# sc15i2gp/daily-ray-trace

Hardware: NVIDIA B200
Metric: camera_paths_per_sec (higher is better)
Workload: dtype f32

## Files before the change

### daily-ray-trace_b200/csrc/drt_capi.cu

```cuda
#include <cuda_runtime.h>
#include <math.h>
#include <stdarg.h>
#include <stdio.h>
#include <stdlib.h>
#include <string.h>
#include <vector>
#include "drt_context.cuh"

static thread_local char g_err[512];

int drt_fail(int code, const char *fmt, ...)
{
    va_list ap;
    va_start(ap, fmt);
    vsnprintf(g_err, sizeof(g_err), fmt, ap);
    va_end(ap);
    return code;
}

extern "C" const char *drt_cuda_last_error(void) { return g_err; }

extern "C" int drt_cuda_device_count(void)
{
    int n = 0;
// ... 170 lines not shown
    if(nmirror + ncond + ndiel == mm->num_lobes && (nmirror != 0) + (ncond != 0) + (ndiel != 0) == 1)
    {
        if(basis_out) *basis_out = nmirror ? 0 : ndiel ? 1 : 2;
        return (nmirror || (base_n && own_n)) ? DRT_CLASS_SPECULAR : DRT_CLASS_GENERAL;
    }
    return DRT_CLASS_GENERAL;
}

static int scene_kernel_mode(const drt_scene *scene)
{
    int nlights = 0;
    for(int i = 0; i < scene->num_surfaces; i += 1) nlights += scene->materials[scene->surfaces[i].material].is_emissive ? 1 : 0;
    bool all_fast = nlights == 1 && !scene->materials[scene->escape_material].is_emissive, classed = all_fast;
    for(int i = 0; i < scene->num_surfaces; i += 1)
    {
        const int m = scene->surfaces[i].material;
        if(scene->materials[m].is_black_body || scene->surfaces[i].type == DRT_GEO_POINT || scene->surfaces[i].type == DRT_GEO_NONE) continue;
        const int cls = classify_material(scene, m, nullptr, nullptr, nullptr);
        if(cls != DRT_CLASS_PLASTIC) all_fast = false;
        if(cls == DRT_CLASS_GENERAL) classed = false;
    }
    if(getenv("DRT_NO_CLASSED")) classed = all_fast;
    return all_fast ? 1 : classed ? 2 : 0;
}

template <typename R>
static void fill_geom(GeomT<R> *g, const drt_scene *s, const drt_camera *c);

extern "C" int drt_cuda_plan_scene(const drt_scene *scene, const drt_camera *camera, int32_t *kernel_mode_out, int32_t *material_class, float *specular_constants)
{
    if(!scene || !camera || !kernel_mode_out) return fail(DRT_CUDA_E_ARG, "NULL argument");
    int rc = drt_cuda_validate_scene(scene);
    if(rc != DRT_CUDA_OK) return rc;
    *kernel_mode_out = scene_kernel_mode(scene);
    if(material_class || specular_constants)
    {
        GeomT<float> *g = new GeomT<float>();
        fill_geom(g, scene, camera);
        for(int m = 0; m < scene->num_materials; m += 1)
        {
            if(material_class) material_class[m] = g->mclass[m];
            if(specular_constants) memcpy(specular_constants + (size_t)m * 6, g->spec_c[m], 6 * sizeof(float));
        }
        delete g;
    }
    return DRT_CUDA_OK;
}

template <typename R>
static void fill_geom(GeomT<R> *g, const drt_scene *s, const drt_camera *c)
{
    memset(g, 0, sizeof(*g));
    g->nsurf = s->num_surfaces; g->nmat = s->num_materials; g->n = s->num_wavelengths;
    g->base_mat = s->base_material; g->escape_mat = s->escape_material;
    uint32_t i0 = (uint32_t)((DRT_TRANS_WL - s->min_wl) / s->wl_interval);
    double w0 = s->min_wl + i0 * s->wl_interval, w1 = s->min_wl + (i0 + 1) * s->wl_interval;
    g->trans_num = (R)(DRT_TRANS_WL - w0);
    g->trans_den = (R)(w1 - w0);
    int nl = 0;
    for(int i = 0; i < s->num_surfaces; i += 1)
    {
        const drt_surface *f = &s->surfaces[i];
        g->type[i] = f->type; g->mat[i] = f->material;
        g->px[i] = (R)f->position[0]; g->py[i] = (R)f->position[1]; g->pz[i] = (R)f->position[2];
        g->rad[i] = (R)f->radius;
        g->nx[i] = (R)f->normal[0]; g->ny[i] = (R)f->normal[1]; g->nz[i] = (R)f->normal[2];
        g->ux[i] = (R)f->u[0]; g->uy[i] = (R)f->u[1]; g->uz[i] = (R)f->u[2];
        g->vx[i] = (R)f->v[0]; g->vy[i] = (R)f->v[1]; g->vz[i] = (R)f->v[2];
        double pdf = 1.0;
        if(f->type == DRT_GEO_PLANE)
        {
            double ul = sqrt(f->u[0] * f->u[0] + f->u[1] * f->u[1] + f->u[2] * f->u[2]);
            double vl = sqrt(f->v[0] * f->v[0] + f->v[1] * f->v[1] + f->v[2] * f->v[2]);
            g->ulen[i] = (R)ul; g->vlen[i] = (R)vl;
            g->unx[i] = (R)(f->u[0] / ul); g->uny[i] = (R)(f->u[1] / ul); g->unz[i] = (R)(f->u[2] / ul);
            g->vnx[i] = (R)(f->v[0] / vl); g->vny[i] = (R)(f->v[1] / vl); g->vnz[i] = (R)(f->v[2] / vl);
            double cx = f->u[1] * f->v[2] - f->u[2] * f->v[1], cy = f->u[2] * f->v[0] - f->u[0] * f->v[2], cz = f->u[0] * f->v[1] - f->u[1] * f->v[0];
            pdf = sqrt(cx * cx + cy * cy + cz * cz);
        }
        else if(f->type == DRT_GEO_SPHERE) pdf = (double)(4.0 * 3.1415926535897932385L * f->radius * f->radius);
        g->light_pdf[i] = (R)pdf;
        if(s->materials[f->material].is_emissive) g->light_surf[nl++] = i;
    }
    g->nlights = nl;
    auto plane_axis = [&](const drt_surface *f) -> int {
        auto single = [](const double *v) -> int {
            int axis = -1;
            for(int k = 0; k < 3; k += 1) if(v[k] != 0.0) { if(axis >= 0) return -1; axis = k; }
            return axis;
        };
        int a = single(f->normal), b = single(f->u), c = single(f->v);
        if(a < 0 || b < 0 || c < 0 || a == b || a == c || b == c) return -1;
        if(f->normal[a] != 1.0 && f->normal[a] != -1.0) return -1;
        return a;
    };
    int slot = 0;
    for(int pass = 0; pass < 9; pass += 1)
        for(int i = 0; i < s->num_surfaces; i += 1)
        {
            const drt_surface *f = &s->surfaces[i];
            const int group = pass / 2;
            if(pass < 8)
            {
                if(f->type != DRT_GEO_PLANE || plane_axis(f) != (group < 3 ? group : -1)) continue;
                if(surface_is_boundary(s, i) != ((pass & 1) == 0)) continue;
                if((pass & 1) == 0) g->nax_b[group] += 1;
            }
            else if(f->type != DRT_GEO_SPHERE) continue;
            g->sid[slot] = i;
            g->N4[slot] = R4<R>{ g->nx[i], g->ny[i], g->nz[i], (R)0 };
            g->P4[slot] = R4<R>{ g->px[i], g->py[i], g->pz[i], g->rad[i] };
            g->U4[slot] = R4<R>{ g->unx[i], g->uny[i], g->unz[i], g->ulen[i] };
            g->V4[slot] = R4<R>{ g->vnx[i], g->vny[i], g->vnz[i], g->vlen[i] };
            if(group < 3)
            {
                const int a = group, b = (a == 0) ? 1 : 0, c = (a == 2) ? 1 : 2;
                double lo[2], hi[2];
                const int bc[2] = { b, c };
                for(int k = 0; k < 2; k += 1)
                {
                    double p0 = f->position[bc[k]], p1 = p0 + f->u[bc[k]] + f->v[bc[k]];
                    lo[k] = p0 < p1 ? p0 : p1; hi[k] = p0 < p1 ? p1 : p0;
                }
                g->AX4[slot] = R4<R>{ (R)f->position[a], (R)(0.5 * (lo[0] + hi[0])), (R)(0.5 * (hi[0] - lo[0])), (R)(0.5 * (lo[1] + hi[1])) };
                g->AXH[slot] = R2<R>{ (R)(0.5 * (hi[1] - lo[1])), (R)i };
                g->nax[a] += 1;
            }
            slot += 1;
            if(pass < 8) g->nplanes += 1; else g->nspheres += 1;
        }
    for(int m = 0; m < s->num_materials; m += 1)
    {
        const drt_material *mm = &s->materials[m];
        g->mflags[m] = (mm->is_black_body ? 1 : 0) | (mm->is_emissive ? 2 : 0);
        g->nlobes[m] = mm->num_lobes; g->dirf[m] = mm->dir_func;
        for(int k = 0; k < mm->num_lobes && k < DRT_MAX_LOBES; k += 1) g->lobes[m][k] = (unsigned char)mm->lobes[k];
        g->shin[m] = (R)mm->shininess; g->rough[m] = (R)mm->roughness;
        int mask = 0;
        for(int k = 0; k < mm->num_lobes && k < DRT_MAX_LOBES; k += 1)
            switch(mm->lobes[k])
            {
                case DRT_LOBE_BP_DIFFUSE: mask |= 1 << BK_DIFFUSE; break;
                case DRT_LOBE_BP_GLOSSY: mask |= 1 << BK_GLOSSY; break;
                case DRT_LOBE_MIRROR: mask |= 1 << BK_MIRROR; break;
                case DRT_LOBE_FS_CONDUCTOR: mask |= 1 << BK_COND_ON; break;
                case DRT_LOBE_FS_DIELECTRIC_REFLECTANCE: mask |= 1 << BK_DIEL_R; break;
                case DRT_LOBE_FS_DIELECTRIC_TRANSMITTANCE: mask |= (1 << BK_DIEL_R) | (1 << BK_CONST); break;
                case DRT_LOBE_CT_CONDUCTOR: mask |= 1 << BK_COND_MN; break;
                default: break;
            }
        g->bmask[m] = mask;
        g->mclass[m] = classify_material(s, m, nullptr, nullptr, nullptr);
        if(g->mclass[m] == DRT_CLASS_SPECULAR)
            for(int match = 0; match < 3; match += 1)
            {
                const bool refl = match == 1, trans = match == 2;
                double cur_c = 0.0, cur_x = 0.0, acc_c = 0.0, acc_x = 0.0;
                for(int k = 0; k < mm->num_lobes; k += 1)
                {
                    bool wrote = false; double val = 0.0, val_c = 0.0;
                    switch(mm->lobes[k])
                    {
                        case DRT_LOBE_MIRROR: wrote = true; val = refl ? 1.0 : 0.0; break;
                        case DRT_LOBE_FS_CONDUCTOR: case DRT_LOBE_FS_DIELECTRIC_REFLECTANCE: wrote = refl; val = 1.0; break;
                        case DRT_LOBE_FS_DIELECTRIC_TRANSMITTANCE: wrote = trans; val = -1.0; val_c = 1.0; break;
                        default: break;
                    }
                    if(wrote) { cur_x = val; cur_c = val_c; }
                    acc_c += cur_c; acc_x += cur_x;
                }
                g->spec_c[m][match][0] = (float)acc_c; g->spec_c[m][match][1] = (float)acc_x;
            }
        int nct = 0;
        for(int k = 0; k < mm->num_lobes && k < DRT_MAX_LOBES; k += 1) nct += mm->lobes[k] == DRT_LOBE_CT_CONDUCTOR;
        g->ct_mult[m] = (float)nct;
        int words = __builtin_popcount((unsigned)mask) + ((mask >> BK_COND_MN) & 1);
        if(!mm->is_black_body && words > g->eval_words) g->eval_words = words;
        if(mm->spd_mask & (1 << DRT_SPD_REFRACT))
        {
            g->n630[m] = (R)value_at_wl(s, mm->spd[DRT_SPD_REFRACT], DRT_TRANS_WL);
            g->refr_a[m] = (R)mm->spd[DRT_SPD_REFRACT][i0];
            g->refr_b[m] = (R)mm->spd[DRT_SPD_REFRACT][i0 + 1];
        }
    }
    for(int k = 0; k < 3; k += 1)
    {
        g->fwd[k] = (R)c->forward[k]; g->right[k] = (R)c->right[k]; g->up[k] = (R)c->up[k];
        g->ap_pos[k] = (R)c->aperture_position[k]; g->film_bl[k] = (R)c->film_bottom_left[k];
    }
    g->ap_radius = (R)c->aperture_radius; g->focal_depth = (R)c->focal_depth;
    g->pixel_w = (R)c->pixel_width; g->pixel_h = (R)c->pixel_height;
    for(int k = 0; k < 9; k += 1) g->lens_rot[k] = (R)c->lens_rotation[k];
}

extern "C" int drt_cuda_validate_scene(const drt_scene *scene)
{
    if(!scene) return fail(DRT_CUDA_E_ARG, "NULL argument");
    int n = scene->num_wavelengths;
    if(n < 2 || n > DRT_MAX_WAVELENGTHS) return fail(DRT_CUDA_E_ARG, "%d wavelengths (need 2..%d)", n, DRT_MAX_WAVELENGTHS);
    if(scene->num_surfaces < 0 || scene->num_surfaces > DRT_MAX_SURFACES || scene->num_materials < 1 || scene->num_materials > DRT_MAX_MATERIALS)
        return fail(DRT_CUDA_E_ARG, "%d surfaces / %d materials out of range", scene->num_surfaces, scene->num_materials);
    if(scene->base_material < 0 || scene->escape_material < 0) return fail(DRT_CUDA_E_UNSUPPORTED, "scene needs a base_material and an escape_material");
    if(scene->base_material >= scene->num_materials || scene->escape_material >= scene->num_materials)
        return fail(DRT_CUDA_E_ARG, "base_material %d / escape_material %d out of range (%d materials)", scene->base_material, scene->escape_material, scene->num_materials);
    if(!(scene->wl_interval > 0.0)) return fail(DRT_CUDA_E_ARG, "wl_interval must be positive");
    uint32_t i0 = (uint32_t)((DRT_TRANS_WL - scene->min_wl) / scene->wl_interval);
    if(DRT_TRANS_WL < scene->min_wl || (int)i0 + 1 >= n) return fail(DRT_CUDA_E_UNSUPPORTED, "630 nm (trans_wl, daily_ray_trace.c:381) lies outside the wavelength grid");
    for(int i = 0; i < scene->num_surfaces; i += 1)
    {
        if(scene->surfaces[i].material < 0 || scene->surfaces[i].material >= scene->num_materials) return fail(DRT_CUDA_E_ARG, "surface %d: bad material index", i);
        if(scene->surfaces[i].type < DRT_GEO_NONE || scene->surfaces[i].type > DRT_GEO_PLANE) return fail(DRT_CUDA_E_ARG, "surface %d: bad type %d", i, scene->surfaces[i].type);
    }
    for(int m = 0; m < scene->num_materials; m += 1)
    {
        const drt_material *mm = &scene->materials[m];
        if(mm->num_lobes < 0 || mm->num_lobes > DRT_MAX_LOBES) return fail(DRT_CUDA_E_ARG, "material %d: %d lobes (0..%d)", m, mm->num_lobes, DRT_MAX_LOBES);
        if(mm->dir_func < DRT_DIR_NONE || mm->dir_func >= DRT_DIR_COUNT) return fail(DRT_CUDA_E_ARG, "material %d: bad dir_func %d", m, mm->dir_func);
        for(int k = 0; k < mm->num_lobes; k += 1)
            if(mm->lobes[k] < -1 || mm->lobes[k] >= DRT_LOBE_COUNT) return fail(DRT_CUDA_E_ARG, "material %d: bad lobe id %d", m, mm->lobes[k]);
    }
    for(int i = 0; i < scene->num_surfaces; i += 1)
    {
        const drt_material *mm = &scene->materials[scene->surfaces[i].material];
        if(scene->surfaces[i].type != DRT_GEO_POINT && scene->surfaces[i].type != DRT_GEO_NONE && !mm->is_black_body && mm->dir_func == DRT_DIR_NONE)
            return fail(DRT_CUDA_E_ARG, "surface %d: its material has no dir_func", i);
    }
    return DRT_CUDA_OK;
}

extern "C" int drt_cuda_upload_scene(drt_cuda_context *ctx, const drt_scene *scene, const drt_camera *camera, const drt_tables *tables)
{
    if(!ctx || !scene || !camera || !tables) return fail(DRT_CUDA_E_ARG, "NULL argument");
    int vrc = drt_cuda_validate_scene(scene);
    if(vrc != DRT_CUDA_OK) return vrc;
    CU(cudaSetDevice(ctx->device));
    const int n = scene->num_wavelengths;
    const uint32_t i0 = (uint32_t)((DRT_TRANS_WL - scene->min_wl) / scene->wl_interval);
    (void)i0;

    GeomT<float> *g32 = new GeomT<float>();
    GeomT<double> *g64 = new GeomT<double>();
    fill_geom(g32, scene, camera);
    fill_geom(g64, scene, camera);

    ctx->hit_bound = scene_hit_bound(scene, camera, &ctx->hit_u0, &ctx->hit_u1, &ctx->hit_v0, &ctx->hit_v1);

    SpdIndex index;
    memset(&index, 0, sizeof(index));
    int half_slots = (n + 15) / 16;
    half_slots = half_slots <= 2 ? 2 : half_slots <= 3 ? 3 : half_slots <= 5 ? 5 : 8;
    index.n = n; index.nslots = half_slots; index.npad = ((n + 31) / 32) * 32;
    if(index.npad < half_slots * 16) index.npad = half_slots * 16;
    std::vector<float> pool((size_t)index.npad, 0.f);
    int rows = 1;
    for(int m = 0; m < scene->num_materials; m += 1)
        for(int k = 0; k < DRT_SPD_COUNT; k += 1)
        {
            if(!(scene->materials[m].spd_mask & (1 << k))) continue;
            index.row[m][k] = (rows++) * index.npad;
            size_t at = pool.size();
            pool.resize(at + (size_t)index.npad, 0.f);
            for(int i = 0; i < n; i += 1) pool[at + (size_t)i] = (float)scene->materials[m].spd[k][i];
        }
    index.nrows = rows;
    if(g32->nlights == 1)
    {
        const double *emission = scene->materials[scene->surfaces[g32->light_surf[0]].material].spd[DRT_SPD_EMISSION];
        const bool have_e = (scene->materials[scene->surfaces[g32->light_surf[0]].material].spd_mask & (1 << DRT_SPD_EMISSION)) != 0;
        for(int m = 0; m < scene->num_materials; m += 1)
        {
            const drt_material *mm = &scene->materials[m];
            if(mm->is_black_body || mm->num_lobes != 2 || g32->bmask[m] != ((1 << BK_DIFFUSE) | (1 << BK_GLOSSY))) continue;
            size_t at = (pool.size() + 3) & ~(size_t)3;
            pool.resize(at + (size_t)half_slots * 64, 0.f);
            index.plastic[m] = (int)at;
            auto val = [&](int k, int slot, int lane) -> float {
                int wl = lane + slot * 16;
                return (wl < n && (mm->spd_mask & (1 << k))) ? (float)mm->spd[k][wl] : 0.f;
            };
            auto emi = [&](int slot, int lane) -> float {
                int wl = lane + slot * 16;
                return (wl < n && have_e) ? (float)emission[wl] : 0.f;
            };
            const int np = half_slots / 2;
            for(int lane = 0; lane < 16; lane += 1)
            {
                for(int pr = 0; pr < np; pr += 1)
                    for(int j = 0; j < 2; j += 1)
                    {
                        int slot = 2 * pr + j;
                        float d = val(DRT_SPD_DIFFUSE, slot, lane), gl = val(DRT_SPD_GLOSSY, slot, lane), e = emi(slot, lane);
                        float *c0 = &pool[at + ((size_t)(2 * pr) * 16 + lane) * 4], *c1 = &pool[at + ((size_t)(2 * pr + 1) * 16 + lane) * 4];
                        c0[j] = d; c0[2 + j] = gl; c1[j] = d * e; c1[2 + j] = gl * e;
                    }
                if(half_slots & 1)
                {
                    int slot = half_slots - 1;
                    float d = val(DRT_SPD_DIFFUSE, slot, lane), gl = val(DRT_SPD_GLOSSY, slot, lane), e = emi(slot, lane);
                    float *c = &pool[at + ((size_t)(half_slots - 1) * 16 + lane) * 4];
                    c[0] = d; c[1] = gl; c[2] = d * e; c[3] = gl * e;
                }
            }
        }
        for(int m = 0; m < scene->num_materials; m += 1)
        {
            const drt_material *mm = &scene->materials[m];
            int nd = 0, ng = 0;
            if(mm->is_black_body || classify_material(scene, m, &nd, &ng, nullptr) != DRT_CLASS_PLASTIC) continue;
            auto val = [&](int k, int mult, int slot, int lane) -> float {
                int wl = lane + slot * 16;
                return (wl < n && (mm->spd_mask & (1 << k))) ? (float)((double)mult * mm->spd[k][wl]) : 0.f;
            };
            const int nchunks = (half_slots + 1) / 2;
            size_t at2 = (pool.size() + 3) & ~(size_t)3;
            pool.resize(at2 + (size_t)nchunks * 64, 0.f);
            index.plastic2[m] = (int)at2;
            for(int lane = 0; lane < 16; lane += 1)
                for(int ch = 0; ch < nchunks; ch += 1)
                {
                    float *c = &pool[at2 + ((size_t)ch * 16 + lane) * 4];
                    if(2 * ch + 1 < half_slots)
                    {
                        c[0] = val(DRT_SPD_DIFFUSE, nd, 2 * ch, lane); c[1] = val(DRT_SPD_DIFFUSE, nd, 2 * ch + 1, lane);
                        c[2] = val(DRT_SPD_GLOSSY, ng, 2 * ch, lane);  c[3] = val(DRT_SPD_GLOSSY, ng, 2 * ch + 1, lane);
                    }
                    else { c[0] = val(DRT_SPD_DIFFUSE, nd, 2 * ch, lane); c[1] = val(DRT_SPD_GLOSSY, ng, 2 * ch, lane); }
                }
        }
        const int nchunks = (half_slots + 1) / 2;
        size_t ate = (pool.size() + 3) & ~(size_t)3;
        pool.resize(ate + (size_t)nchunks * 32, 0.f);
        index.light_pairs = (int)ate;
        for(int lane = 0; lane < 16; lane += 1)
            for(int ch = 0; ch < nchunks; ch += 1)
            {
                float *c = &pool[ate + ((size_t)ch * 16 + lane) * 2];
                int w0 = lane + (2 * ch) * 16, w1 = lane + (2 * ch + 1) * 16;
                c[0] = (w0 < n && have_e) ? (float)emission[w0] : 0.f;
                c[1] = (2 * ch + 1 < half_slots && w1 < n && have_e) ? (float)emission[w1] : 0.f;
            }
    }

    if(scene->materials[scene->base_material].spd_mask & (1 << DRT_SPD_REFRACT))
    {
        const drt_material *bm = &scene->materials[scene->base_material];
        const bool base_k = (bm->spd_mask & (1 << DRT_SPD_EXTINCT)) != 0;
        for(int m = 0; m < scene->num_materials; m += 1)
        {
            const drt_material *mm = &scene->materials[m];
            if(m == scene->base_material || mm->is_black_body || !(mm->spd_mask & (1 << DRT_SPD_REFRACT))) continue;
            const bool own_k = (mm->spd_mask & (1 << DRT_SPD_EXTINCT)) != 0;
            for(int side = 0; side < 2; side += 1)
                for(int k = 0; k < 3; k += 1)
                {
                    size_t at = pool.size();
                    pool.resize(at + (size_t)index.npad, 0.f);
                    index.fres[m][side][k] = (int)at;
                    for(int i = 0; i < n; i += 1)
                    {
                        const double ir = side ? mm->spd[DRT_SPD_REFRACT][i] : bm->spd[DRT_SPD_REFRACT][i];
                        const double tr = side ? bm->spd[DRT_SPD_REFRACT][i] : mm->spd[DRT_SPD_REFRACT][i];
                        const double te = side ? (base_k ? bm->spd[DRT_SPD_EXTINCT][i] : 0.0) : (own_k ? mm->spd[DRT_SPD_EXTINCT][i] : 0.0);
                        const double eta = tr / ir, kap = te / ir;
                        pool[at + (size_t)i] = (float)(k == 0 ? ir / tr : k == 1 ? eta * eta - kap * kap : 4.0 * eta * eta * kap * kap);
                    }
                }
        }
    }

    std::vector<unsigned char> rgbt(drt_rgb_tables_bytes());
    drt_fill_rgb_tables(rgbt.data(), tables);

    ctx->have_scene = false;
    cudaError_t e = cudaSuccess;
    if(e == cudaSuccess && !ctx->d_geom32) e = cudaMalloc(&ctx->d_geom32, sizeof(GeomT<float>));
    if(e == cudaSuccess && !ctx->d_geom64) e = cudaMalloc(&ctx->d_geom64, sizeof(GeomT<double>));
    if(e == cudaSuccess && !ctx->d_index) e = cudaMalloc(&ctx->d_index, sizeof(SpdIndex));
    if(e == cudaSuccess && !ctx->d_rgb_tables) e = cudaMalloc(&ctx->d_rgb_tables, rgbt.size());
    if(e == cudaSuccess && ctx->pool_capacity < pool.size() * 4)
    {
        cudaFree(ctx->d_pool); ctx->d_pool = nullptr; ctx->pool_capacity = 0;
        e = cudaMalloc(&ctx->d_pool, pool.size() * 4);
        if(e == cudaSuccess) ctx->pool_capacity = pool.size() * 4;
    }
    if(e == cudaSuccess) e = cudaMemcpy(ctx->d_geom32, g32, sizeof(GeomT<float>), cudaMemcpyHostToDevice);
    if(e == cudaSuccess) e = cudaMemcpy(ctx->d_geom64, g64, sizeof(GeomT<double>), cudaMemcpyHostToDevice);
    if(e == cudaSuccess) e = cudaMemcpy(ctx->d_index, &index, sizeof(index), cudaMemcpyHostToDevice);
    if(e == cudaSuccess) e = cudaMemcpy(ctx->d_pool, pool.data(), pool.size() * 4, cudaMemcpyHostToDevice);
    if(e == cudaSuccess) e = cudaMemcpy(ctx->d_rgb_tables, rgbt.data(), rgbt.size(), cudaMemcpyHostToDevice);
    int nlights = g32->nlights;
    int mode = scene_kernel_mode(scene);
    bool all_fast = mode == 1, classed = mode != 0;
    if(pool.size() > 65535) all_fast = classed = false;
    int eval_words = g32->eval_words > 0 ? g32->eval_words : 1;
    delete g32; delete g64;
    if(e != cudaSuccess) return fail(DRT_CUDA_E_CUDA, "scene upload: %s", cudaGetErrorString(e));
    ctx->n = n; ctx->nslots = index.nslots; ctx->nlights = nlights; ctx->eval_words = eval_words; ctx->all_fast = all_fast; ctx->classed = classed && !all_fast; ctx->pool_words = (uint32_t)pool.size();
    ctx->upload_bytes = sizeof(GeomT<float>) + sizeof(GeomT<double>) + sizeof(SpdIndex) + pool.size() * 4 + rgbt.size();
    ctx->have_scene = true;
    return DRT_CUDA_OK;
}

extern "C" int drt_cuda_scene_upload_bytes(const drt_cuda_context *ctx, size_t *bytes)
{
    if(!ctx || !bytes) return fail(DRT_CUDA_E_ARG, "NULL argument");
    *bytes = ctx->upload_bytes;
    return DRT_CUDA_OK;
}

extern "C" int drt_cuda_set_geometry_precision(drt_cuda_context *ctx, int precision)
{
    if(!ctx || (precision != DRT_GEOMETRY_F32 && precision != DRT_GEOMETRY_F64)) return fail(DRT_CUDA_E_ARG, "bad precision");
    ctx->f64_geometry = precision == DRT_GEOMETRY_F64;
    return DRT_CUDA_OK;
}

extern "C" int drt_cuda_film_sizes(const drt_cuda_context *ctx, uint32_t width, uint32_t height, size_t *spectral, size_t *filter)
{
    if(!ctx || !ctx->have_scene) return fail(DRT_CUDA_E_STATE, "upload a scene first");
    if(spectral) *spectral = (size_t)width * height * (size_t)ctx->n * 4;
    if(filter) *filter = (size_t)width * height * 4;
    return DRT_CUDA_OK;
}

static int kernel_mode(const drt_cuda_context *ctx) { return ctx->f64_geometry ? 0 : ctx->all_fast ? 1 : ctx->classed ? 2 : 0; }

static void record_layout(const drt_cuda_context *ctx, uint32_t max_depth, uint32_t smem_depth, RenderLaunch &L)
{
    L.eval_words = (uint32_t)ctx->eval_words;
    const bool compact = kernel_mode(ctx) != 0;
    L.bounce_words = (2 + (uint32_t)ctx->nlights * (L.eval_words + 1) + L.eval_words + 3u) & ~3u;
    if(L.bounce_words < 8) L.bounce_words = 8;
    L.head_words = 4;
    if(smem_depth > max_depth) smem_depth = max_depth;
    if(compact) { L.bounce_words = 4; L.head_words = (2 + (smem_depth + 1) / 2 + 3u) & ~3u; }
    L.smem_depth = smem_depth;
    L.path_words = L.head_words + smem_depth * L.bounce_words;
    L.path_stride = ((L.path_words / 4) & 1u) ? L.path_words : L.path_words + 4;
    const uint32_t over = max_depth - smem_depth;
    L.deep_hdr_off = over * L.bounce_words;
    L.deep_stride = over ? ((L.deep_hdr_off + (compact ? (over + 1) / 2 : 0u) + 4u + 3u) & ~3u) : 0u;
}

static bool launch_shape(const drt_cuda_context *ctx, uint32_t max_depth, bool whole, RenderLaunch &L, int *warps_out, int *ctas_out, size_t *smem_out)
{
    const int mode = kernel_mode(ctx);
    const int full_warps = drt_render_cta_warps(ctx->f64_geometry, mode), want_ctas = drt_render_min_ctas(ctx->f64_geometry, mode);
    auto bytes = [&](uint32_t depth, int warps) { record_layout(ctx, max_depth, depth, L); return drt_render_smem_bytes(L, ctx->f64_geometry, warps, ctx->nslots); };
    int warps = full_warps;
    uint32_t depth = max_depth;
    const size_t per_cta = (size_t)(227 * 1024) / (size_t)want_ctas - 1024;
    if(!whole && max_depth > 1 && bytes(max_depth, warps) > per_cta)
    {
        uint32_t lo = 1, hi = max_depth;
        while(lo < hi) { uint32_t mid = (lo + hi + 1) / 2; if(bytes(mid, warps) <= per_cta) lo = mid; else hi = mid - 1; }
        depth = lo;
    }
    size_t smem = bytes(depth, warps);
    while(smem > ctx->smem_optin && warps > 1) { warps /= 2; smem = bytes(depth, warps); }
    *warps_out = warps; *smem_out = smem;
    if(smem > ctx->smem_optin) return false;
    int ctas_per_sm = (int)((size_t)(227 * 1024) / (smem + 1024));
    int by_threads = (want_ctas * full_warps) / warps;
    if(ctas_per_sm > by_threads) ctas_per_sm = by_threads;
    if(ctas_per_sm < 1) ctas_per_sm = 1;
    *ctas_out = ctas_per_sm;
    return true;
}

extern "C" int drt_cuda_render_kernel_info(drt_cuda_context *ctx, const drt_render_params *params, char *name, size_t name_len, int *warps_per_cta, int *ctas_per_sm)
{
    if(!ctx || !params || params->sample_end <= params->sample_begin) return fail(DRT_CUDA_E_ARG, "bad argument");
    const uint32_t max_depth = params->max_depth;
    if(!ctx->have_scene) return fail(DRT_CUDA_E_STATE, "upload a scene first");
    RenderLaunch L;
    memset(&L, 0, sizeof(L));
    L.pool_words = ctx->pool_words;
    int warps = 0, ctas = 0;
    size_t smem = 0;
    if(!launch_shape(ctx, max_depth, false, L, &warps, &ctas, &smem)) return fail(DRT_CUDA_E_UNSUPPORTED, "one bounce record of this scene does not fit in shared memory");
    if(name && name_len)
        snprintf(name, name_len, "drt::render_kernel<%s,%d,%d,%s,%s>", ctx->f64_geometry ? "double" : "float", ctx->nslots,
                 kernel_mode(ctx), (params->sample_end - params->sample_begin >= 32) ? "true" : "false", L.deep_stride ? "true" : "false");
    if(warps_per_cta) *warps_per_cta = warps;
    if(ctas_per_sm) *ctas_per_sm = ctas;
    return DRT_CUDA_OK;
}

static int launch(drt_cuda_context *ctx, const drt_render_params *p, uint32_t x0, uint32_t y0, uint32_t x1, uint32_t y1,
                  FilmPtrs film, float *dump, int accumulate, cudaStream_t stream, float *record_dump = nullptr, uint32_t *path_words_out = nullptr,
                  const drt_film *scatter = nullptr, int scatter_count = 0, int scatter_rank = 0, uint64_t scatter_slice = 0, bool keep_stats = false,
                  uint64_t band_begin = 0, uint64_t band_end = 0, const drt_adaptive *adaptive = nullptr)
{
    if(!ctx->have_scene) return fail(DRT_CUDA_E_STATE, "upload a scene first");
    if(p->width == 0 || p->height == 0 || x1 > p->width || y1 > p->height || x0 >= x1 || y0 >= y1) return fail(DRT_CUDA_E_ARG, "bad image rectangle");
    if(p->sample_end < p->sample_begin) return fail(DRT_CUDA_E_ARG, "bad sample range [%u,%u)", p->sample_begin, p->sample_end);
    CU(cudaSetDevice(ctx->device));
    if(p->sample_end == p->sample_begin)
    {
        if(path_words_out) *path_words_out = 0;
        if(!keep_stats)
        {
            ctx->d_stats = ctx->d_stats_ring + (ctx->stats_calls++ % DRT_RING);
            CU(cudaMemsetAsync(ctx->d_stats, 0, sizeof(DeviceStats), stream));
        }
        ctx->last_launches = 0;
        if(film.sum && !accumulate && scatter_count == 0)
        {
            const size_t n = (size_t)ctx->n, w = p->width;
            if(x0 != 0 || x1 != p->width) return fail(DRT_CUDA_E_ARG, "empty sample range on a partial-width rectangle");
            const size_t at = (size_t)y0 * w, cnt = (size_t)(y1 - y0) * w;
            CU(cudaMemsetAsync(film.sum + at * n, 0, cnt * n * 4, stream)); CU(cudaMemsetAsync(film.mean + at * n, 0, cnt * n * 4, stream));
            CU(cudaMemsetAsync(film.m2 + at * n, 0, cnt * n * 4, stream));  CU(cudaMemsetAsync(film.filter + at, 0, cnt * 4, stream));
        }
        return DRT_CUDA_OK;
    }
    RenderLaunch L;
    memset(&L, 0, sizeof(L));
    L.geom = ctx->f64_geometry ? ctx->d_geom64 : ctx->d_geom32;
    L.spd_index = ctx->d_index; L.pool = ctx->d_pool; L.pool_words = ctx->pool_words;
    L.film = film; L.path_dump = dump; L.record_dump = record_dump;
    L.width = p->width; L.height = p->height; L.x0 = x0; L.y0 = y0; L.x1 = x1; L.y1 = y1;
    L.sample_begin = p->sample_begin; L.sample_end = p->sample_end; L.max_depth = p->max_depth;
    L.pixel_scheme = p->pixel_scheme; L.seed = p->seed; L.accumulate = accumulate; L.nlights = ctx->nlights;
    uint32_t spp = p->sample_end - p->sample_begin;
    L.pixels_per_task = spp >= 32 ? 1 : 32 / spp;
    for(int i = 0; i < scatter_count; i += 1) L.scatter[i] = FilmPtrs{ scatter[i].sum, scatter[i].filter, scatter[i].mean, scatter[i].m2 };
    L.scatter_count = (uint32_t)scatter_count; L.scatter_rank = (uint32_t)scatter_rank; L.scatter_slice = (uint32_t)scatter_slice;
    uint32_t rect[4];
    hit_rect(ctx->hit_bound && p->max_depth > 0, ctx->hit_u0, ctx->hit_u1, ctx->hit_v0, ctx->hit_v1, p->width, p->height, rect);
    L.hit_x0 = rect[0]; L.hit_y0 = rect[1]; L.hit_x1 = rect[2]; L.hit_y1 = rect[3];
    if(adaptive)
    {
        L.adaptive = 1; L.rel_error = adaptive->rel_error; L.min_samples = adaptive->min_samples;
        L.luminance_w = reinterpret_cast<const float *>(static_cast<const unsigned char *>(ctx->d_rgb_tables) + drt_rgb_tables_yw_offset());
    }
    const bool whole = record_dump != nullptr || (path_words_out != nullptr && !dump && !film.sum);
    int warps, ctas_per_sm;
    size_t smem;
    if(!launch_shape(ctx, p->max_depth, whole, L, &warps, &ctas_per_sm, &smem))
        return fail(DRT_CUDA_E_UNSUPPORTED, "%s: max_cast_depth %u with %d lights needs %zu bytes of shared memory per warp (limit %zu)",
                    whole ? "record dump" : "render", p->max_depth, ctx->nlights, smem, ctx->smem_optin);
    if(path_words_out) { *path_words_out = L.path_words; if(!record_dump && !dump && !film.sum) return DRT_CUDA_OK; }
    uint64_t npix = (uint64_t)(x1 - x0) * (y1 - y0);
    const bool band = band_end > band_begin;
    if(band)
    {
        if(L.pixels_per_task != 1 || scatter_count < 1 || band_end > scatter_slice || x0 != 0 || y0 != 0 || x1 != p->width || y1 != p->height)
            return fail(DRT_CUDA_E_ARG, "a band needs a scattered whole-frame render with at least 32 samples per pixel");
        L.band_chunk = (uint32_t)(band_end - band_begin); L.band_period = (uint32_t)scatter_slice; L.band_base = (uint32_t)band_begin;
    }
    uint64_t ntasks = band ? (uint64_t)L.band_chunk * scatter_count : (npix + L.pixels_per_task - 1) / L.pixels_per_task;
    if(scatter_count > 1)
        L.task_rotate = band ? (uint32_t)(((uint64_t)scatter_rank * L.band_chunk) % ntasks)
                             : (uint32_t)((((uint64_t)scatter_rank * scatter_slice) / L.pixels_per_task) % ntasks);
    uint64_t grid = (uint64_t)ctx->num_sms * ctas_per_sm;
    uint64_t need = (ntasks + warps - 1) / warps;
    if(grid > need) grid = need;
    if(L.deep_stride)
    {
        const size_t need_bytes = (size_t)grid * (size_t)warps * DRT_WARP * L.deep_stride * 4;
        int rc = drt_ensure_buffer(&ctx->d_deep, &ctx->deep_bytes, need_bytes);
        if(rc != DRT_CUDA_OK) return rc;
        L.deep = ctx->d_deep;
    }
    if(!keep_stats)
    {
        ctx->d_stats = ctx->d_stats_ring + (ctx->stats_calls++ % DRT_RING);
        CU(cudaMemsetAsync(ctx->d_stats, 0, sizeof(DeviceStats), stream));
    }
    L.stats = ctx->d_stats;
    L.task_counter = ctx->d_counter_ring + (ctx->counter_launches++ % DRT_RING);
    CU(cudaMemsetAsync(L.task_counter, 0, sizeof(unsigned int), stream));
    cudaError_t e = drt_launch_render(L, ctx->f64_geometry, kernel_mode(ctx), ctx->nslots, (int)grid, warps, smem, stream);
    if(e != cudaSuccess) return fail(DRT_CUDA_E_CUDA, "render kernel launch: %s", cudaGetErrorString(e));
    ctx->launches += 1;
    ctx->last_launches = 1;
    return DRT_CUDA_OK;
}

extern "C" int drt_cuda_render_device(drt_cuda_context *ctx, const drt_render_params *params, const drt_film *film, int accumulate, void *stream)
{
    if(!ctx || !params || !film || !film->sum || !film->filter || !film->mean || !film->m2) return fail(DRT_CUDA_E_ARG, "NULL argument");
    FilmPtrs f = { film->sum, film->filter, film->mean, film->m2 };
    return launch(ctx, params, 0, 0, params->width, params->height, f, nullptr, accumulate, (cudaStream_t)stream);
}

extern "C" int drt_cuda_render_device_scatter(drt_cuda_context *ctx, const drt_render_params *params, const drt_film *staging, int count, int rank,
                                              uint64_t slice_pixels, void *stream)
{
    if(!ctx || !params || !staging || count < 1 || count > DRT_MAX_PEERS || rank < 0 || rank >= count) return fail(DRT_CUDA_E_ARG, "bad argument (1..%d staging films)", DRT_MAX_PEERS);
    uint64_t npix = (uint64_t)params->width * params->height;
    if(slice_pixels == 0 || slice_pixels * (uint64_t)count < npix || slice_pixels > 0xffffffffull) return fail(DRT_CUDA_E_ARG, "slices of %llu pixels do not cover the image", (unsigned long long)slice_pixels);
    for(int i = 0; i < count; i += 1)
        if(!staging[i].sum || !staging[i].filter || !staging[i].mean || !staging[i].m2) return fail(DRT_CUDA_E_ARG, "NULL staging film %d", i);
    FilmPtrs f = { staging[0].sum, staging[0].filter, staging[0].mean, staging[0].m2 };
    return launch(ctx, params, 0, 0, params->width, params->height, f, nullptr, 0, (cudaStream_t)stream, nullptr, nullptr, staging, count, rank, slice_pixels);
}

extern "C" int drt_cuda_render_device_scatter_band(drt_cuda_context *ctx, const drt_render_params *params, const drt_film *staging, int count, int rank,
                                                   uint64_t slice_pixels, uint64_t band_begin, uint64_t band_end, int keep_stats, void *stream)
{
    if(!ctx || !params || !staging || count < 1 || count > DRT_MAX_PEERS || rank < 0 || rank >= count) return fail(DRT_CUDA_E_ARG, "bad argument (1..%d staging films)", DRT_MAX_PEERS);
    uint64_t npix = (uint64_t)params->width * params->height;
    if(slice_pixels == 0 || slice_pixels * (uint64_t)count < npix || slice_pixels > 0xffffffffull) return fail(DRT_CUDA_E_ARG, "slices of %llu pixels do not cover the image", (unsigned long long)slice_pixels);
    if(band_begin >= band_end || band_end > slice_pixels) return fail(DRT_CUDA_E_ARG, "bad band [%llu, %llu) of a slice of %llu pixels", (unsigned long long)band_begin, (unsigned long long)band_end, (unsigned long long)slice_pixels);
    for(int i = 0; i < count; i += 1)
        if(!staging[i].sum || !staging[i].filter || !staging[i].mean || !staging[i].m2) return fail(DRT_CUDA_E_ARG, "NULL staging film %d", i);
    FilmPtrs f = { staging[0].sum, staging[0].filter, staging[0].mean, staging[0].m2 };
    return launch(ctx, params, 0, 0, params->width, params->height, f, nullptr, 0, (cudaStream_t)stream, nullptr, nullptr, staging, count, rank, slice_pixels,
                  keep_stats != 0, band_begin, band_end);
}

int drt_ensure_buffer(float **buf, size_t *have, size_t need)
{
    if(*have >= need) return DRT_CUDA_OK;
    cudaFree(*buf); *buf = nullptr; *have = 0;
    CU(cudaMalloc(buf, need));
    *have = need;
    return DRT_CUDA_OK;
}

static int adaptive_args(const drt_cuda_context *ctx, const drt_render_params *p, const drt_adaptive *a)
{
    if(!ctx->have_scene) return fail(DRT_CUDA_E_STATE, "upload a scene first");
    if(p->sample_end < p->sample_begin) return fail(DRT_CUDA_E_ARG, "bad sample range [%u,%u)", p->sample_begin, p->sample_end);
    const uint32_t range = p->sample_end - p->sample_begin;
    if(!(a->rel_error > 0.f) || !isfinite(a->rel_error))
        return fail(DRT_CUDA_E_ARG, "adaptive sampling: rel_error must be a finite number > 0 (got %g)", (double)a->rel_error);
    if(a->min_samples < 32u || a->min_samples > range)
        return fail(DRT_CUDA_E_ARG, "adaptive sampling: min_samples must lie in [32, %u], the call's sample range [%u,%u) (got %u); "
                    "a pixel is checked after each batch of 32 samples, so the range needs at least 32", range, p->sample_begin, p->sample_end, a->min_samples);
    if(ctx->f64_geometry)
        return fail(DRT_CUDA_E_UNSUPPORTED, "adaptive sampling runs with f32 geometry only: f64 geometry is the branch-flip diagnostic and has no adaptive kernel");
    return DRT_CUDA_OK;
}

extern "C" int drt_cuda_render_device_adaptive(drt_cuda_context *ctx, const drt_render_params *params, const drt_adaptive *adaptive,
                                               const drt_film *film, int accumulate, void *stream)
{
    if(!ctx || !params || !adaptive || !film || !film->sum || !film->filter || !film->mean || !film->m2) return fail(DRT_CUDA_E_ARG, "NULL argument");
    int rc = adaptive_args(ctx, params, adaptive);
    if(rc != DRT_CUDA_OK) return rc;
    FilmPtrs f = { film->sum, film->filter, film->mean, film->m2 };
    return launch(ctx, params, 0, 0, params->width, params->height, f, nullptr, accumulate, (cudaStream_t)stream, nullptr, nullptr, nullptr, 0, 0, 0, false, 0, 0, adaptive);
}

static int render_host(drt_cuda_context *ctx, const drt_render_params *params, const drt_adaptive *adaptive, const drt_film *out)
{
    if(!ctx || !params || !out || !out->sum || !out->filter || !out->mean || !out->m2) return fail(DRT_CUDA_E_ARG, "NULL argument");
    if(!ctx->have_scene) return fail(DRT_CUDA_E_STATE, "upload a scene first");
    CU(cudaSetDevice(ctx->device));
    size_t npix = (size_t)params->width * params->height, plane = npix * (size_t)ctx->n * 4, fplane = npix * 4;
    int rc = drt_ensure_buffer(&ctx->d_film, &ctx->film_bytes, 3 * plane + fplane);
    if(rc != DRT_CUDA_OK) return rc;
    float *base = ctx->d_film;
    FilmPtrs f = { base, base + 3 * (plane / 4), base + plane / 4, base + 2 * (plane / 4) };
    const uint64_t paths = (uint64_t)npix * (params->sample_end - params->sample_begin);
    static const int cut[] = { 0, 4, 8, 12, 14, 15, 16 };
    int bands = (paths >= (1ull << 26) && params->height >= 64) ? 6 : 1;
    if(bands > 1 && !ctx->band_render)
    {
        CU(cudaStreamCreateWithFlags(&ctx->band_render, cudaStreamNonBlocking));
        CU(cudaStreamCreateWithFlags(&ctx->band_copy, cudaStreamNonBlocking));
        for(int i = 0; i < 16; i += 1) CU(cudaEventCreateWithFlags(&ctx->band_done[i], cudaEventDisableTiming));
    }
    cudaStream_t sr = bands > 1 ? ctx->band_render : 0, sc = bands > 1 ? ctx->band_copy : 0;
    if(bands > 1) CU(cudaDeviceSynchronize());
    const size_t n = (size_t)ctx->n, w = params->width;
    for(int b = 0; b < bands; b += 1)
    {
        const uint32_t y0 = bands > 1 ? (uint32_t)((uint64_t)params->height * cut[b] / 16) : 0u;
        const uint32_t y1 = bands > 1 ? (uint32_t)((uint64_t)params->height * cut[b + 1] / 16) : params->height;
        rc = launch(ctx, params, 0, y0, params->width, y1, f, nullptr, 0, sr, nullptr, nullptr, nullptr, 0, 0, 0, b > 0, 0, 0, adaptive);
        if(rc != DRT_CUDA_OK) return rc;
        if(bands > 1) { CU(cudaEventRecord(ctx->band_done[b], sr)); CU(cudaStreamWaitEvent(sc, ctx->band_done[b], 0)); }
        const size_t at = (size_t)y0 * w * n, cnt = (size_t)(y1 - y0) * w * n * 4;
        CU(cudaMemcpyAsync(out->sum + at, f.sum + at, cnt, cudaMemcpyDeviceToHost, sc));
        CU(cudaMemcpyAsync(out->mean + at, f.mean + at, cnt, cudaMemcpyDeviceToHost, sc));
        CU(cudaMemcpyAsync(out->m2 + at, f.m2 + at, cnt, cudaMemcpyDeviceToHost, sc));
        CU(cudaMemcpyAsync(out->filter + (size_t)y0 * w, f.filter + (size_t)y0 * w, (size_t)(y1 - y0) * w * 4, cudaMemcpyDeviceToHost, sc));
    }
    ctx->last_launches = (uint64_t)bands;
    if(bands > 1) { CU(cudaStreamSynchronize(sr)); CU(cudaStreamSynchronize(sc)); }
    CU(cudaStreamSynchronize(0));
    return DRT_CUDA_OK;
}

extern "C" int drt_cuda_render_host(drt_cuda_context *ctx, const drt_render_params *params, const drt_film *out)
{
    return render_host(ctx, params, nullptr, out);
}

extern "C" int drt_cuda_render_host_adaptive(drt_cuda_context *ctx, const drt_render_params *params, const drt_adaptive *adaptive, const drt_film *out)
{
    if(!ctx || !params || !adaptive) return fail(DRT_CUDA_E_ARG, "NULL argument");
    int rc = adaptive_args(ctx, params, adaptive);
    if(rc != DRT_CUDA_OK) return rc;
    return render_host(ctx, params, adaptive, out);
}

extern "C" int drt_cuda_get_stats(drt_cuda_context *ctx, drt_cuda_stats *out)
{
    if(!ctx || !out) return fail(DRT_CUDA_E_ARG, "NULL argument");
    CU(cudaSetDevice(ctx->device));
    CU(cudaDeviceSynchronize());
    DeviceStats s;
    CU(cudaMemcpy(&s, ctx->d_stats, sizeof(s), cudaMemcpyDeviceToHost));
    memset(out, 0, sizeof(*out));
    out->paths = s.paths; out->closest_rays = s.closest_rays; out->shadow_rays = s.shadow_rays;
    out->shaded_bounces = s.shaded_bounces; out->rng_draws = s.rng_draws;
    for(int i = 0; i < 8; i += 1) out->terminated_at_depth[i] = s.terminated_at_depth[i];
    out->reached_depth_cap = s.reached_depth_cap;
    out->kernel_launches = ctx->last_launches;
    return DRT_CUDA_OK;
}

#ifdef DRT_PHASE_CLOCKS
extern "C" int drt_cuda_phase_clocks(drt_cuda_context *ctx, uint64_t out[4])
{
    if(!ctx || !out) return fail(DRT_CUDA_E_ARG, "NULL argument");
    CU(cudaSetDevice(ctx->device));
    CU(cudaDeviceSynchronize());
    DeviceStats s;
    CU(cudaMemcpy(&s, ctx->d_stats, sizeof(s), cudaMemcpyDeviceToHost));
    for(int i = 0; i < 4; i += 1) out[i] = s.phase_clocks[i];
    return DRT_CUDA_OK;
}
#endif

extern "C" int drt_cuda_sample_paths(drt_cuda_context *ctx, const drt_render_params *params,
                                     uint32_t x0, uint32_t y0, uint32_t x1, uint32_t y1, float *out_host)
{
    if(!ctx || !params || !out_host) return fail(DRT_CUDA_E_ARG, "NULL argument");
    if(!ctx->have_scene) return fail(DRT_CUDA_E_STATE, "upload a scene first");
    if(x1 <= x0 || y1 <= y0 || params->sample_end <= params->sample_begin) return fail(DRT_CUDA_E_ARG, "empty rectangle or sample range");
    CU(cudaSetDevice(ctx->device));
    size_t bytes = (size_t)(x1 - x0) * (y1 - y0) * (params->sample_end - params->sample_begin) * (size_t)ctx->n * 4;
    int rc = drt_ensure_buffer(&ctx->d_dump, &ctx->dump_bytes, bytes);
    if(rc != DRT_CUDA_OK) return rc;
    FilmPtrs none = { nullptr, nullptr, nullptr, nullptr };
    rc = launch(ctx, params, x0, y0, x1, y1, none, ctx->d_dump, 0, 0);
    if(rc != DRT_CUDA_OK) return rc;
    CU(cudaMemcpy(out_host, ctx->d_dump, bytes, cudaMemcpyDeviceToHost));
    return DRT_CUDA_OK;
}

extern "C" int drt_cuda_debug_records(drt_cuda_context *ctx, const drt_render_params *params, uint32_t x0, uint32_t y0, uint32_t x1, uint32_t y1,
                                      float *out_host, size_t out_capacity_words, uint32_t *words_per_path)
{
    if(!ctx || !params || !words_per_path) return fail(DRT_CUDA_E_ARG, "NULL argument");
    if(!ctx->have_scene) return fail(DRT_CUDA_E_STATE, "upload a scene first");
    if(x1 <= x0 || y1 <= y0 || params->sample_end <= params->sample_begin) return fail(DRT_CUDA_E_ARG, "empty rectangle or sample range");
    CU(cudaSetDevice(ctx->device));
    FilmPtrs none = { nullptr, nullptr, nullptr, nullptr };
    int rc = launch(ctx, params, x0, y0, x1, y1, none, nullptr, 0, 0, nullptr, words_per_path);
    if(rc != DRT_CUDA_OK || !out_host) return rc;
    size_t words = (size_t)(x1 - x0) * (y1 - y0) * (params->sample_end - params->sample_begin) * (size_t)*words_per_path;
    if(words > out_capacity_words) return fail(DRT_CUDA_E_ARG, "record buffer too small: need %zu words", words);
    rc = drt_ensure_buffer(&ctx->d_dump, &ctx->dump_bytes, words * 4);
    if(rc != DRT_CUDA_OK) return rc;
    rc = launch(ctx, params, x0, y0, x1, y1, none, nullptr, 0, 0, ctx->d_dump, nullptr);
    if(rc != DRT_CUDA_OK) return rc;
    CU(cudaMemcpy(out_host, ctx->d_dump, words * 4, cudaMemcpyDeviceToHost));
    return DRT_CUDA_OK;
}

extern "C" int drt_cuda_film_to_rgb(drt_cuda_context *ctx, const drt_film *film, uint32_t width, uint32_t height, int which,
                                    float *rgb_device, uint32_t *bgra_device, void *stream)
{
    if(!ctx || !film || which < 0 || which > 2) return fail(DRT_CUDA_E_ARG, "bad argument");
    if(!ctx->have_scene) return fail(DRT_CUDA_E_STATE, "upload a scene first");
    CU(cudaSetDevice(ctx->device));
    const float *plane = which == 0 ? film->sum : which == 1 ? film->mean : film->m2;
    const float *filter = which == 0 ? film->filter : nullptr;
    if(!plane || (which == 0 && !filter)) return fail(DRT_CUDA_E_ARG, "film plane is NULL");
    const uint64_t npix64 = (uint64_t)width * height;
    if(npix64 == 0 || npix64 > 0xffffffffull) return fail(DRT_CUDA_E_ARG, "%u x %u pixels out of range", width, height);
    uint32_t npix = (uint32_t)npix64;
    int grid = ctx->num_sms * 8;
    drt_launch_film_to_rgb(ctx->d_rgb_tables, plane, filter, which == 2, npix, rgb_device, bgra_device, grid, (cudaStream_t)stream);
    CU(cudaGetLastError());
    ctx->launches += 1;
    return DRT_CUDA_OK;
}

extern "C" int drt_cuda_film_merge(drt_cuda_context *ctx, const drt_film *dst, const drt_film *src, uint32_t width, uint32_t height, void *stream)
{
    if(!ctx || !dst || !src) return fail(DRT_CUDA_E_ARG, "NULL argument");
    if(!ctx->have_scene) return fail(DRT_CUDA_E_STATE, "upload a scene first");
    CU(cudaSetDevice(ctx->device));
    FilmPtrs d = { dst->sum, dst->filter, dst->mean, dst->m2 }, s = { src->sum, src->filter, src->mean, src->m2 };
    drt_launch_film_merge(d, s, (uint32_t)ctx->n, (size_t)width * height, ctx->num_sms * 8, (cudaStream_t)stream);
    CU(cudaGetLastError());
    ctx->launches += 2;
    return DRT_CUDA_OK;
}

extern "C" int drt_cuda_film_alloc(drt_cuda_context *ctx, uint32_t width, uint32_t height, drt_film *out)
{
    if(!ctx || !out) return fail(DRT_CUDA_E_ARG, "NULL argument");
    if(!ctx->have_scene) return fail(DRT_CUDA_E_STATE, "upload a scene first");
    CU(cudaSetDevice(ctx->device));
    size_t npix = (size_t)width * height, plane = npix * (size_t)ctx->n * 4;
    memset(out, 0, sizeof(*out));
    cudaError_t e = cudaMalloc(&out->sum, plane);
    if(e == cudaSuccess) e = cudaMalloc(&out->mean, plane);
    if(e == cudaSuccess) e = cudaMalloc(&out->m2, plane);
    if(e == cudaSuccess) e = cudaMalloc(&out->filter, npix * 4);
    if(e == cudaSuccess) e = cudaMemset(out->sum, 0, plane);
    if(e == cudaSuccess) e = cudaMemset(out->mean, 0, plane);
    if(e == cudaSuccess) e = cudaMemset(out->m2, 0, plane);
    if(e == cudaSuccess) e = cudaMemset(out->filter, 0, npix * 4);
    if(e != cudaSuccess)
    {
        cudaFree(out->sum); cudaFree(out->mean); cudaFree(out->m2); cudaFree(out->filter);
        memset(out, 0, sizeof(*out));
        return fail(DRT_CUDA_E_CUDA, "film_alloc %ux%u: %s", width, height, cudaGetErrorString(e));
    }
    return DRT_CUDA_OK;
}

extern "C" int drt_cuda_film_free(drt_cuda_context *ctx, drt_film *film)
{
    if(!ctx || !film) return fail(DRT_CUDA_E_ARG, "NULL argument");
    CU(cudaSetDevice(ctx->device));
    cudaFree(film->sum); cudaFree(film->mean); cudaFree(film->m2); cudaFree(film->filter);
    memset(film, 0, sizeof(*film));
    return DRT_CUDA_OK;
}

extern "C" int drt_cuda_film_ipc_export(drt_cuda_context *ctx, const drt_film *film, unsigned char handles[4][64])
{
    if(!ctx || !film || !handles) return fail(DRT_CUDA_E_ARG, "NULL argument");
    CU(cudaSetDevice(ctx->device));
    static_assert(sizeof(cudaIpcMemHandle_t) == 64, "CUDA IPC handle size");
    float *ptrs[4] = { film->sum, film->filter, film->mean, film->m2 };
    for(int i = 0; i < 4; i += 1)
    {
        cudaIpcMemHandle_t h;
        CU(cudaIpcGetMemHandle(&h, ptrs[i]));
        memcpy(handles[i], &h, 64);
    }
    return DRT_CUDA_OK;
}

extern "C" int drt_cuda_film_ipc_open(drt_cuda_context *ctx, const unsigned char handles[4][64], drt_film *out)
{
    if(!ctx || !handles || !out) return fail(DRT_CUDA_E_ARG, "NULL argument");
    CU(cudaSetDevice(ctx->device));
    void *ptrs[4] = { nullptr, nullptr, nullptr, nullptr };
    for(int i = 0; i < 4; i += 1)
    {
        cudaIpcMemHandle_t h;
        memcpy(&h, handles[i], 64);
        CU(cudaIpcOpenMemHandle(&ptrs[i], h, cudaIpcMemLazyEnablePeerAccess));
    }
    out->sum = (float *)ptrs[0]; out->filter = (float *)ptrs[1]; out->mean = (float *)ptrs[2]; out->m2 = (float *)ptrs[3];
    return DRT_CUDA_OK;
}

extern "C" int drt_cuda_film_ipc_close(drt_cuda_context *ctx, drt_film *mapped)
{
    if(!ctx || !mapped) return fail(DRT_CUDA_E_ARG, "NULL argument");
    CU(cudaSetDevice(ctx->device));
    cudaIpcCloseMemHandle(mapped->sum); cudaIpcCloseMemHandle(mapped->filter); cudaIpcCloseMemHandle(mapped->mean); cudaIpcCloseMemHandle(mapped->m2);
    memset(mapped, 0, sizeof(*mapped));
    return DRT_CUDA_OK;
}

extern "C" int drt_cuda_buffer_alloc(drt_cuda_context *ctx, size_t bytes, void **out)
{
    if(!ctx || !out || bytes == 0) return fail(DRT_CUDA_E_ARG, "bad argument");
    CU(cudaSetDevice(ctx->device));
    CU(cudaMalloc(out, bytes));
    CU(cudaMemset(*out, 0, bytes));
    return DRT_CUDA_OK;
// ... 127 lines not shown
```

### daily-ray-trace_b200/csrc/drt_context.cuh

```cuda
#pragma once
#include <cuda_runtime.h>
#include <stdarg.h>
#include <stdint.h>
#include <stdio.h>
#include "drt_cuda.h"
#include "drt_device.cuh"

cudaError_t drt_launch_render(const RenderLaunch &L, bool f64_geometry, int mode, int nslots, int grid, int warps, size_t smem, cudaStream_t stream);
int         drt_render_cta_warps(bool f64_geometry, int mode);
int         drt_render_min_ctas(bool f64_geometry, int mode);
size_t      drt_render_smem_bytes(const RenderLaunch &L, bool f64_geometry, int warps, int nslots);
void        drt_launch_film_to_rgb(const void *tables, const float *plane, const float *filter, int normalise_by_max, uint32_t npix,
                                   float *rgb, uint32_t *bgra, int grid, cudaStream_t stream);
void        drt_launch_film_merge(FilmPtrs dst, FilmPtrs src, uint32_t n, size_t npix, int grid, cudaStream_t stream);
void        drt_launch_fma_peak(int packed, float *out, int iters, int grid, cudaStream_t stream);
void        drt_launch_film_gather_merge(const void *tables, int count, const FilmPtrs *films, FilmPtrs dst, uint32_t pixel_begin, uint32_t pixel_end, uint32_t src_base, uint32_t dst_base,
                                         uint32_t *bgra_sum, uint32_t *bgra_mean, uint32_t *bgra_var, int grid, cudaStream_t stream);
size_t      drt_rgb_tables_bytes(void);
size_t      drt_rgb_tables_yw_offset(void);
void        drt_fill_rgb_tables(void *dst_host, const drt_tables *t);

int drt_fail(int code, const char *fmt, ...);
#define fail drt_fail

#define CU(call) do { cudaError_t e_ = (call); if(e_ != cudaSuccess) return fail(DRT_CUDA_E_CUDA, "%s: %s", #call, cudaGetErrorString(e_)); } while(0)

#define DRT_RING 64

struct drt_cuda_context
{
    int    device = 0;
    int    num_sms = 0;
    size_t smem_optin = 0;
    bool   have_scene = false;
    bool   f64_geometry = false;
    int    n = 0, nslots = 0, nlights = 0, eval_words = 1;
    bool   hit_bound = false;
    double hit_u0 = 0, hit_u1 = 0, hit_v0 = 0, hit_v1 = 0;
    bool   classed = false;
    bool   all_fast = false;
    void  *d_geom32 = nullptr, *d_geom64 = nullptr;
    SpdIndex *d_index = nullptr;
    float *d_pool = nullptr;
    uint32_t pool_words = 0;
    size_t pool_capacity = 0;
    void  *d_rgb_tables = nullptr;
    DeviceStats *d_stats_ring = nullptr;
    unsigned int *d_counter_ring = nullptr;
    uint64_t stats_calls = 0, counter_launches = 0;
    DeviceStats *d_stats = nullptr;
    float *d_film = nullptr; size_t film_bytes = 0;
    float *d_dump = nullptr; size_t dump_bytes = 0;
    float *d_deep = nullptr; size_t deep_bytes = 0;
    float *d_slice = nullptr; size_t slice_bytes = 0;
    uint64_t launches = 0;
    size_t upload_bytes = 0;
    uint64_t last_launches = 0;
    cudaStream_t band_render = nullptr, band_copy = nullptr;
    cudaEvent_t  band_done[16] = {};
    unsigned int *d_wait_timeouts = nullptr;
    struct drt_multi_state *multi = nullptr;
};


void drt_exchange_release(drt_cuda_context *ctx);
int drt_ensure_buffer(float **buf, size_t *have, size_t need);
```

### daily-ray-trace_b200/csrc/drt_device.cuh

```cuda
#pragma once
#include <stdint.h>
#include "drt_scene.h"

#define DRT_WARP 32
#define DRT_MAX_SLOTS 4
#define DRT_HALF 16
#define DRT_MAX_HALF_SLOTS 8
#ifndef DRT_CTA_WARPS
#define DRT_CTA_WARPS 8
#endif
#ifndef DRT_FAST_WARPS
#define DRT_FAST_WARPS 14
#endif
#ifndef DRT_CLASSED_WARPS
#define DRT_CLASSED_WARPS 16
#endif
#ifndef DRT_CLASSED_CTAS
#define DRT_CLASSED_CTAS 2
#endif
#ifndef DRT_GENERAL_CTAS
#define DRT_GENERAL_CTAS 2
#endif
#ifndef DRT_LOCKSTEP
#define DRT_LOCKSTEP 2
#endif
#ifndef DRT_GATE_PATIENCE_CYCLES
#define DRT_GATE_PATIENCE_CYCLES 20000000ll
#endif
#ifndef DRT_GATE_SUSPEND_NS
#define DRT_GATE_SUSPEND_NS 20000u
#endif
#define DRT_CTA_THREADS (DRT_CTA_WARPS * DRT_WARP)
#ifndef DRT_MIN_CTAS
#define DRT_MIN_CTAS 2
#endif

enum { DRT_CLASS_PLASTIC = 0, DRT_CLASS_SPECULAR = 1, DRT_CLASS_ROUGH = 2, DRT_CLASS_GENERAL = 3 };
enum { BK_CONST = 0, BK_DIFFUSE, BK_GLOSSY, BK_MIRROR, BK_DIEL_R, BK_COND_ON, BK_COND_MN, BK_COUNT };

template <typename R> struct alignas(16) R4 { R x, y, z, w; };
template <typename R> struct alignas(8) R2 { R x, y; };

template <typename R>
struct GeomT
{
    int   nplanes, nspheres, pad2, pad3;
    int   nax[4];
    int   nax_b[4];
    R4<R> AX4[DRT_MAX_SURFACES];
    R2<R> AXH[DRT_MAX_SURFACES];
    int   sid[DRT_MAX_SURFACES];
    R4<R> N4[DRT_MAX_SURFACES];
    R4<R> P4[DRT_MAX_SURFACES];
    R4<R> U4[DRT_MAX_SURFACES];
    R4<R> V4[DRT_MAX_SURFACES];
    int nsurf, nlights, base_mat, escape_mat, nmat, n, eval_words, pad1;
    R   trans_num, trans_den;
    int type[DRT_MAX_SURFACES], mat[DRT_MAX_SURFACES], light_surf[DRT_MAX_SURFACES];
    R   px[DRT_MAX_SURFACES], py[DRT_MAX_SURFACES], pz[DRT_MAX_SURFACES], rad[DRT_MAX_SURFACES];
    R   nx[DRT_MAX_SURFACES], ny[DRT_MAX_SURFACES], nz[DRT_MAX_SURFACES];
    R   unx[DRT_MAX_SURFACES], uny[DRT_MAX_SURFACES], unz[DRT_MAX_SURFACES], ulen[DRT_MAX_SURFACES];
    R   vnx[DRT_MAX_SURFACES], vny[DRT_MAX_SURFACES], vnz[DRT_MAX_SURFACES], vlen[DRT_MAX_SURFACES];
    R   ux[DRT_MAX_SURFACES], uy[DRT_MAX_SURFACES], uz[DRT_MAX_SURFACES];
    R   vx[DRT_MAX_SURFACES], vy[DRT_MAX_SURFACES], vz[DRT_MAX_SURFACES];
    R   light_pdf[DRT_MAX_SURFACES];
    int mflags[DRT_MAX_MATERIALS];
    int mclass[DRT_MAX_MATERIALS];
    float spec_c[DRT_MAX_MATERIALS][3][2];
    float ct_mult[DRT_MAX_MATERIALS];
    int bmask[DRT_MAX_MATERIALS];
    int nlobes[DRT_MAX_MATERIALS], dirf[DRT_MAX_MATERIALS];
    unsigned char lobes[DRT_MAX_MATERIALS][DRT_MAX_LOBES];
    R   shin[DRT_MAX_MATERIALS], rough[DRT_MAX_MATERIALS];
    R   n630[DRT_MAX_MATERIALS];
    R   refr_a[DRT_MAX_MATERIALS], refr_b[DRT_MAX_MATERIALS];
    R   fwd[3], right[3], up[3], ap_pos[3], film_bl[3];
    R   ap_radius, focal_depth, pixel_w, pixel_h;
    R   lens_rot[9];
};

struct SpdIndex
{
    int n, nslots, npad, nrows;
    int row[DRT_MAX_MATERIALS][DRT_SPD_COUNT];
    int plastic[DRT_MAX_MATERIALS];
    int plastic2[DRT_MAX_MATERIALS];
    int light_pairs, pad[3];
    int fres[DRT_MAX_MATERIALS][2][3];
};

struct FilmPtrs { float *sum, *filter, *mean, *m2; };
#define DRT_MAX_PEERS 16

struct DeviceStats
{
    unsigned long long paths, closest_rays, shadow_rays, shaded_bounces, rng_draws;
    unsigned long long terminated_at_depth[8];
    unsigned long long reached_depth_cap;
#ifdef DRT_PHASE_CLOCKS
    unsigned long long phase_clocks[4];
#endif
};

struct RenderLaunch
{
    const void     *geom;
    const SpdIndex *spd_index;
    const float    *pool;
    FilmPtrs        film;
    float          *path_dump;
    float          *record_dump;
    DeviceStats    *stats;
    unsigned int   *task_counter;
    uint32_t width, height;
    uint32_t x0, y0, x1, y1;
    uint32_t sample_begin, sample_end;
    uint32_t max_depth;
    int32_t  pixel_scheme;
    uint64_t seed;
    int32_t  accumulate;
    int32_t  nlights;
    uint32_t pixels_per_task;
    uint32_t eval_words;
    uint32_t bounce_words;
    uint32_t head_words;
    uint32_t path_words;
    uint32_t path_stride;
    uint32_t geom_bytes, pool_words;
    uint32_t smem_depth, deep_stride, deep_hdr_off;
    float   *deep;
    uint32_t hit_x0, hit_y0, hit_x1, hit_y1;
    uint32_t scatter_count, scatter_rank, scatter_slice;
    uint32_t band_chunk, band_period, band_base;
    uint32_t task_rotate;
    FilmPtrs scatter[DRT_MAX_PEERS];
    const float *luminance_w;
    float    rel_error;
    uint32_t min_samples;
    uint32_t adaptive;
};
```

### daily-ray-trace_b200/csrc/drt_render.cuh

```cuda
#pragma once
#include <cuda_runtime.h>
#include <math_constants.h>
#include "drt_device.cuh"
#include "drt_rng.h"

namespace drt {


template <typename R> struct V3 { R x, y, z; };

template <typename R> __device__ __forceinline__ V3<R> mk(R x, R y, R z) { V3<R> v; v.x = x; v.y = y; v.z = z; return v; }
template <typename R> __device__ __forceinline__ V3<R> operator+(V3<R> a, V3<R> b) { return mk<R>(a.x + b.x, a.y + b.y, a.z + b.z); }
template <typename R> __device__ __forceinline__ V3<R> operator-(V3<R> a, V3<R> b) { return mk<R>(a.x - b.x, a.y - b.y, a.z - b.z); }
template <typename R> __device__ __forceinline__ V3<R> operator*(V3<R> a, R f) { return mk<R>(f * a.x, f * a.y, f * a.z); }
template <typename R> __device__ __forceinline__ V3<R> neg(V3<R> a) { return mk<R>(-a.x, -a.y, -a.z); }
template <typename R> __device__ __forceinline__ R dot(V3<R> a, V3<R> b) { return a.x * b.x + a.y * b.y + a.z * b.z; }
template <typename R> __device__ __forceinline__ V3<R> cross(V3<R> a, V3<R> b)
{
    return mk<R>(a.y * b.z - a.z * b.y, a.z * b.x - a.x * b.z, a.x * b.y - a.y * b.x);
}

__device__ __forceinline__ float r_rcp_fast(float x) { float r; asm("rcp.approx.ftz.f32 %0, %1;" : "=f"(r) : "f"(x)); return r; }
__device__ __forceinline__ float  r_sqrt(float x)  { float r; asm("sqrt.approx.ftz.f32 %0, %1;" : "=f"(r) : "f"(x)); return r; }
__device__ __forceinline__ double r_sqrt(double x) { return sqrt(x); }
// ... 235 lines not shown
    int sm = g.mat[found];
    h.surf_mat = sm; h.trans_mat = sm; h.inc_mat = g.base_mat;
    if(h.on_dot < R(0))
    {
        if(!is_plane) { h.trans_mat = g.base_mat; h.inc_mat = sm; }
        n = neg(n);
        h.on_dot = dot(n, h.out);
    }
    h.nrm = n;
    return true;
}

template <typename R> __device__ __forceinline__ bool visible(const GeomT<R> &g, V3<R> p0, V3<R> p1, int skip, V3<R> &dir)
{
    dir = normalise(p1 - p0);
    V3<R> o = p0 + dir * Num<R>::fudge();
    V3<R> po = p1 - o;
    R vis_dist = r_sqrt(dot(po, po)) - Num<R>::fudge();
    R t;
    if(g.nax_b[0] + g.nax_b[1] + g.nax_b[2] + g.nax_b[3] == g.nplanes && g.nspheres == 0) return true;
    return nearest_surface<R>(g, o, dir, vis_dist, skip, true, &t) < 0;
}

#define BMASK_PLASTIC ((1 << BK_DIFFUSE) | (1 << BK_GLOSSY))

template <typename R>
static __device__ __noinline__ void eval_weights_general(const GeomT<R> &g, int m, V3<R> nrm, V3<R> out, R on_dot, V3<R> in, int match, float scale,
                                                  float *rec, uint32_t at)
{
    const bool is_reflection = match & 1, is_transmission = match & 2;
    float cur[BK_COUNT], acc[BK_COUNT];
#pragma unroll
    for(int k = 0; k < BK_COUNT; k += 1) { cur[k] = 0.f; acc[k] = 0.f; }
    float mn_cos = 0.f;
    int nl = g.nlobes[m];
    for(int li = 0; li < nl; li += 1)
    {
        int lobe = g.lobes[m][li];
        bool wrote = true;
        int kind = BK_CONST;
        float val = 0.f, val_const = 0.f;
        switch(lobe)
        {
            case DRT_LOBE_BP_DIFFUSE:
                kind = BK_DIFFUSE; val = (float)((R(1) / Num<R>::pi()) * r_abs(dot(nrm, in)));
                break;
            case DRT_LOBE_BP_GLOSSY:
            {
                V3<R> bis = normalise(out + in);
                R nb = dot(nrm, bis);
                R coef = r_pow((R(0) > nb) ? R(0) : nb, g.shin[m]);
                kind = BK_GLOSSY; val = (float)(coef * r_abs(dot(nrm, in)));
                break;
            }
            case DRT_LOBE_MIRROR:
                kind = BK_MIRROR; val = is_reflection ? 1.f : 0.f;
                break;
            case DRT_LOBE_FS_CONDUCTOR:
                kind = BK_COND_ON; val = 1.f; wrote = is_reflection;
                break;
            case DRT_LOBE_FS_DIELECTRIC_REFLECTANCE:
                kind = BK_DIEL_R; val = 1.f; wrote = is_reflection;
                break;
            case DRT_LOBE_FS_DIELECTRIC_TRANSMITTANCE:
                kind = BK_DIEL_R; val = -1.f; val_const = 1.f; wrote = is_transmission;
                break;
            case DRT_LOBE_CT_CONDUCTOR:
            {
                V3<R> mn = normalise(out + in);
                R mn_dot = r_abs(dot(nrm, mn));
                R rough = g.rough[m], r2 = rough * rough;
                R d = dot(nrm, mn), gg = R(0);
                if(d > R(0))
                {
                    R d2 = d * d, d4 = d2 * d2, tan_sq = r_div(R(1), d2) - R(1);
                    gg = r_div(r2, Num<R>::pi() * d4 * (r2 + tan_sq) * (r2 + tan_sq));
                }
                R v_mn = dot(out, mn), v_sn = dot(out, nrm);
                R quot = r_abs(r_div(v_mn, v_sn)), att = R(0);
                if(!(quot <= R(0)))
                {
                    R tan_sq = r_div(R(1), v_sn * v_sn) - R(1);
                    att = r_div(R(2), R(1) + r_sqrt(R(1) + r2 * tan_sq));
                }
                kind = BK_COND_MN; val = (float)((gg * att) * r_div(R(1), R(4) * on_dot));
                mn_cos = (float)mn_dot;
                break;
            }
            default: wrote = false; break;
        }
        if(wrote)
        {
#pragma unroll
            for(int k = 0; k < BK_COUNT; k += 1) cur[k] = (k == kind) ? val : 0.f;
            cur[BK_CONST] += val_const;
        }
#pragma unroll
        for(int k = 0; k < BK_COUNT; k += 1) acc[k] += cur[k];
    }
    const int mask = g.bmask[m];
#pragma unroll
    for(int k = 0; k < BK_COUNT; k += 1)
        if(mask & (1 << k)) { rec[at] = acc[k] * scale; at += 1; }
    if(mask & (1 << BK_COND_MN)) rec[at] = mn_cos;
}

template <typename R>
__device__ __forceinline__ void plastic_weights(const GeomT<R> &g, int m, V3<R> nrm, V3<R> out, V3<R> in, float scale, float &wd, float &wg)
{
    R cos_in = r_abs(dot(nrm, in));
    V3<R> bis = normalise(out + in);
    R nb = dot(nrm, bis);
    R coef = r_pow((R(0) > nb) ? R(0) : nb, g.shin[m]);
    wd = (float)((R(1) / Num<R>::pi()) * cos_in) * scale;
    wg = (float)(coef * cos_in) * scale;
}
template <typename R>
static __device__ __noinline__ float2 ct_weight(const GeomT<R> &g, int m, V3<R> nrm, V3<R> out, R on_dot, V3<R> in)
{
    V3<R> mn = normalise(out + in);
    R d = dot(nrm, mn), gg = R(0);
    R rough = g.rough[m], r2 = rough * rough;
    if(d > R(0))
    {
        R d2 = d * d, d4 = d2 * d2, tan_sq = r_div(R(1), d2) - R(1);
        gg = r_div(r2, Num<R>::pi() * d4 * (r2 + tan_sq) * (r2 + tan_sq));
    }
    R v_mn = dot(out, mn), v_sn = dot(out, nrm);
    R quot = r_abs(r_div(v_mn, v_sn)), att = R(0);
    if(!(quot <= R(0)))
    {
        R tan_sq = r_div(R(1), v_sn * v_sn) - R(1);
        att = r_div(R(2), R(1) + r_sqrt(R(1) + r2 * tan_sq));
    }
    return make_float2((float)((gg * att) * r_div(R(1), R(4) * on_dot)) * g.ct_mult[m], (float)r_abs(d));
}

template <typename T> __device__ __forceinline__ T fresnel_dielectric(T ir, T tr, T inc_cos)
{
    T inc_sin_sq = T(1) - inc_cos * inc_cos;
    T rel = r_div(ir, tr);
    T ts_sin_sq = rel * rel * inc_sin_sq;
    if(ts_sin_sq >= T(1)) return T(1);
    T ts_cos = r_sqrt_fast(T(1) - ts_sin_sq * ts_sin_sq);
    T tr_on = tr * inc_cos, tr_ts = tr * ts_cos, ir_on = ir * inc_cos, ir_ts = ir * ts_cos;
    T par = r_div(tr_on - ir_ts, tr_on + ir_ts);
    T per = r_div(ir_on - tr_ts, ir_on + tr_ts);
    return T(0.5) * (par * par + per * per);
}


__device__ __forceinline__ void sincospi_quarter(float u, float &s, float &c)
{
    const float v = u * u;
    const float ps = fmaf(fmaf(-0x1.330cc6p-1f, v, 0x1.46805cp+1f), v, -0x1.4abc24p+2f);
    s = fmaf(u, 0x1.921fb6p+1f, (u * v) * ps);
    const float pc = fmaf(fmaf(fmaf(0x1.d9f7bcp-3f, v, -0x1.55c664p+0f), v, 0x1.03c1dep+2f), v, -0x1.3bd3ccp+2f);
    c = fmaf(v, pc, 1.f);
}

__device__ __forceinline__ void disc_sincos(float q, bool steep, float &s, float &c)
{
    float a, b;
    sincospi_quarter(0.25f * q, a, b);
    s = steep ? b : a; c = steep ? a : b;
}
__device__ __forceinline__ void disc_sincos(double q, bool steep, double &s, double &c) { r_sincospi(steep ? 0.5 - 0.25 * q : 0.25 * q, &s, &c); }

template <typename R> __device__ __forceinline__ V3<R> sample_disc(Rng &rng)
{
    R rx = rng.unit<R>();
    R ry = rng.unit<R>();
    R ox = R(2) * rx - R(1), oy = R(2) * ry - R(1);
    if(ox == R(0) && oy == R(0)) return mk<R>(R(0), R(0), R(0));
    R r, q;
    const bool steep = !(r_abs(ox) > r_abs(oy));
    if(!steep) { r = ox; q = r_div(oy, ox); }
    else       { r = oy; q = r_div(ox, oy); }
    R s, c;
    disc_sincos(q, steep, s, c);
    return mk<R>(r * c, r * s, R(0));
}

template <typename R> struct DirSample { V3<R> in; R inv_pdf; int match; Rng rng; };

template <typename R>
static __device__ __noinline__ DirSample<R> sample_direction_general(const GeomT<R> &g, Hit<R> h, Rng rng)
{
    DirSample<R> out;
    V3<R> in = mk<R>(R(0), R(0), R(0));
    R inv_pdf = R(0);
    int match = 0;
    int m = h.surf_mat;
    switch(g.dirf[m])
    {
        case DRT_DIR_UNIFORM_HEMISPHERE:
        {
            R u = rng.unit<R>();
            R v = rng.unit<R>();
            R r = r_sqrt(R(1) - u * u);
            R s, c;
            r_sincospi(R(2) * v, &s, &c);
            in = rotate_from_z<R>(h.nrm, mk<R>(r * c, r * s, u));
            inv_pdf = R(2) * Num<R>::pi();
            break;
        }
        case DRT_DIR_SPECULAR:
            in = reflect<R>(neg(h.out), h.nrm);
            inv_pdf = R(1);
            match = 1;
            break;
        case DRT_DIR_TRANSMIT:
            in = transmit<R>(neg(h.out), h.nrm, g.n630[h.inc_mat], g.n630[h.trans_mat]);
            inv_pdf = R(1);
            match = ((in.x == in.x) && (in.y == in.y) && (in.z == in.z)) ? 2 : 0;
            break;
        case DRT_DIR_REFLECT_OR_TRANSMIT:
        {
            R ra = fresnel_dielectric<R>(g.refr_a[h.inc_mat], g.refr_a[h.trans_mat], h.on_dot);
            R rb = fresnel_dielectric<R>(g.refr_b[h.inc_mat], g.refr_b[h.trans_mat], h.on_dot);
            R rd = ra + (g.trans_num * r_div(rb - ra, g.trans_den));
            R f = rng.unit<R>();
            if(f < rd)
            {
                in = reflect<R>(neg(h.out), h.nrm);
                inv_pdf = r_div(R(1), rd);
                match = 1;
            }
            else
            {
                in = transmit<R>(neg(h.out), h.nrm, g.n630[h.inc_mat], g.n630[h.trans_mat]);
                inv_pdf = r_div(R(1), R(1) - rd);
                match = ((in.x == in.x) && (in.y == in.y) && (in.z == in.z)) ? 2 : 0;
            }
            break;
        }
        case DRT_DIR_CT:
        {
            R rough = g.rough[m];
            do
            {
                R f = rng.unit<R>();
                R gq = rng.unit<R>();
                R tan_mn = r_div(rough * r_sqrt(f), r_sqrt(R(1) - f));
                R cos_mn = r_rsqrt(R(1) + tan_mn * tan_mn);
                R cm2 = cos_mn * cos_mn;
                R sin_mn = r_sqrt((cm2 < R(1)) ? R(1) - cm2 : R(0));
                R s, c;
                r_sincospi(R(2) * gq, &s, &c);
                V3<R> mn = rotate_from_z<R>(h.nrm, mk<R>(sin_mn * c, sin_mn * s, cos_mn));
                R sn_mn = dot(h.nrm, mn);
                if(sn_mn < R(0)) { mn = neg(mn); sn_mn = -sn_mn; }
                R o_mn = dot(h.out, mn);
                in = reflect<R>(neg(h.out), mn);
                R d = R(0);
                if(sn_mn > R(0))
                {
                    R r2 = rough * rough, d2 = sn_mn * sn_mn, d4 = d2 * d2, tan_sq = r_div(R(1), d2) - R(1);
                    d = r_div(r2, Num<R>::pi() * d4 * (r2 + tan_sq) * (r2 + tan_sq));
                }
                d = d * sn_mn;
                inv_pdf = r_div(R(4) * o_mn, d);
            }
            while(dot(in, h.nrm) < R(0));
            break;
        }
        default: break;
    }
    out.in = in; out.inv_pdf = inv_pdf; out.match = match; out.rng = rng;
    return out;
}

template <typename R>
__device__ __forceinline__ void sample_direction(const GeomT<R> &g, const Hit<R> &h, Rng &rng, V3<R> &in, R &inv_pdf, int &match)
{
    if(g.dirf[h.surf_mat] == DRT_DIR_COS_WEIGHTED_HEMISPHERE)
    {
        V3<R> q;
        for(;;)
        {
            q = sample_disc<R>(rng);
            if(dot(q, q) < R(1)) break;
        }
        q.z = r_sqrt(R(1) - dot(q, q));
        in = rotate_from_z<R>(h.nrm, q);
        inv_pdf = r_div(Num<R>::pi(), dot(h.nrm, in));
        match = 0;
        return;
    }
    DirSample<R> s = sample_direction_general<R>(g, h, rng);
    in = s.in; inv_pdf = s.inv_pdf; match = s.match; rng = s.rng;
}


#define REC_NB   0
#define REC_VIG  1
#define REC_HDR16 2
#define REC_HEAD 4
#define KIND_SHADE 1u
#define KIND_EMIT  2u
#define HDR_FAST 4u


template <typename R, int MODE, bool DEEP>
__device__ __forceinline__ uint32_t trace_path(const GeomT<R> &g, const SpdIndex &ix, const RenderLaunch &L, float *rec, float *deep,
                                               uint32_t x, uint32_t y, uint32_t sample, uint32_t (&tally)[4])
{
    constexpr bool ALLFAST = MODE != 0;
    constexpr bool CLASSED = MODE == 2;
    Rng rng;
    rng.begin(L.seed, y * L.width + x, sample);

    R px = R(0), py = R(0);
    if(L.pixel_scheme == DRT_PIXEL_CENTER) { px = R(0.5); py = R(0.5); }
    else if(L.pixel_scheme == DRT_PIXEL_RANDOM) { px = rng.unit<R>(); py = rng.unit<R>(); }
    R film_x = (R(x) + px) * g.pixel_w;
    R film_y = (R(y) + py) * g.pixel_h;
    V3<R> fwd = mk<R>(g.fwd[0], g.fwd[1], g.fwd[2]);
    V3<R> ap = mk<R>(g.ap_pos[0], g.ap_pos[1], g.ap_pos[2]);
    V3<R> point = (mk<R>(g.right[0], g.right[1], g.right[2]) * film_x + mk<R>(g.up[0], g.up[1], g.up[2]) * film_y)
                  + mk<R>(g.film_bl[0], g.film_bl[1], g.film_bl[2]);
    V3<R> o, d;
    if(g.ap_radius > R(0))
    {
        V3<R> focus_dir = normalise(ap - point);
        focus_dir = focus_dir * r_div(g.focal_depth, dot(focus_dir, fwd));
        V3<R> focus_point = point + focus_dir;
        V3<R> disc = sample_disc<R>(rng) * g.ap_radius;
        V3<R> lens = mk<R>(g.lens_rot[0] * disc.x + g.lens_rot[3] * disc.y + g.lens_rot[6] * disc.z,
                           g.lens_rot[1] * disc.x + g.lens_rot[4] * disc.y + g.lens_rot[7] * disc.z,
                           g.lens_rot[2] * disc.x + g.lens_rot[5] * disc.y + g.lens_rot[8] * disc.z);
        o = ap + lens;
        d = normalise(focus_point - o);
    }
    else
    {
        o = point;
        d = normalise(ap - o);
    }
    rec[REC_VIG] = (float)dot(d, fwd);

    uint32_t nb = 0, closest = 0, shadow = 0, shaded = 0, end_depth = L.max_depth, general = 0, emitter = 0;
    int skip = -1;
    const uint32_t bw = L.bounce_words, ew = L.eval_words;
    for(uint32_t depth = 0; depth < L.max_depth; depth += 1)
    {
        Hit<R> h;
        closest += 1;
        bool found = closest_hit<R>(g, o, d, skip, h);
        int m = found ? h.surf_mat : g.escape_mat;
        int flags = g.mflags[m];
        const bool in_smem = !DEEP || nb < L.smem_depth;
        float *rb = in_smem ? rec + REC_HEAD + nb * bw : deep + (nb - L.smem_depth) * bw;
        if(flags & 1)
        {
            if(flags & 2)
            {
                if(ALLFAST) emitter = (uint32_t)(m + 1) << 16;
                else { rb[0] = __uint_as_float(KIND_EMIT | ((uint32_t)m << 3)); nb += 1; }
            }
            end_depth = depth;
            break;
        }
        shaded += 1;
        const int sm = h.surf_mat;
        const int cls = CLASSED ? g.mclass[sm] : DRT_CLASS_PLASTIC;
        const bool plastic = ALLFAST ? (cls == DRT_CLASS_PLASTIC) : (g.bmask[sm] == BMASK_PLASTIC && g.nlobes[sm] == 2);
        const bool fast = ALLFAST || (plastic && ix.plastic[sm] != 0);
        const int nlights = ALLFAST ? 1 : g.nlights;
        float *recw = in_smem ? rec + L.head_words + 4u * nb : deep + 4u * (nb - L.smem_depth);
        if(CLASSED && cls == DRT_CLASS_ROUGH) { recw[0] = 0.f; recw[1] = 1.f; }
        uint32_t vis_mask = 0;
        float wd_n = 0.f, wg_n = 0.f;
        for(int j = 0; j < nlights; j += 1)
        {
            int ls = g.light_surf[j];
            int lt = g.type[ls];
            V3<R> lp = mk<R>(g.px[ls], g.py[ls], g.pz[ls]);
            R k;
            if(lt == DRT_GEO_POINT)
            {
                V3<R> to = lp - h.pos;
                R dist = r_sqrt(dot(to, to));
                k = (R(4) * Num<R>::pi() * dist * dist) * g.light_pdf[ls];
            }
            else if(lt == DRT_GEO_SPHERE)
            {
                R u = rng.unit<R>();
                R v = rng.unit<R>();
                R r = r_sqrt(R(1) - u * u);
                R s, c;
                r_sincospi(R(2) * v, &s, &c);
                lp = lp + mk<R>(r * c, r * s, u) * g.rad[ls];
                k = g.light_pdf[ls];
            }
            else
            {
                R u = rng.unit<R>();
                R v = rng.unit<R>();
                lp = (lp + mk<R>(g.ux[ls], g.uy[ls], g.uz[ls]) * u) + mk<R>(g.vx[ls], g.vy[ls], g.vz[ls]) * v;
                k = g.light_pdf[ls];
            }
            shadow += 1;
            V3<R> ldir;
            if(visible<R>(g, h.pos, lp, h.plane_slot, ldir))
            {
                const uint32_t e = 2 + (ew + 1) * (uint32_t)j;
                if(plastic)
                {
                    plastic_weights<R>(g, sm, h.nrm, h.out, ldir, fast ? (float)k : 1.f, wd_n, wg_n);
                    if(!fast) { rb[e] = wd_n; rb[e + 1] = wg_n; }
                }
                else if(CLASSED)
                {
                    if(cls == DRT_CLASS_ROUGH)
                    {
                        const float2 wc = ct_weight<R>(g, sm, h.nrm, h.out, h.on_dot, ldir);
                        recw[0] = wc.x * (float)k; recw[1] = wc.y;
                    }
                }
                else eval_weights_general<R>(g, sm, h.nrm, h.out, h.on_dot, ldir, 0, 1.f, rb, e);
                if(!fast) rb[e + ew] = (float)k;
                vis_mask |= 1u << j;
            }
        }
        V3<R> in; R inv_pdf; int match;
        const uint32_t es = 2 + (ew + 1) * (uint32_t)nlights;
        float wd_s = 0.f, wg_s = 0.f;
        if(ALLFAST && plastic && depth + 1 == L.max_depth && g.dirf[sm] == DRT_DIR_COS_WEIGHTED_HEMISPHERE)
        {
            rng.draws += 2;
            in = h.nrm;
        }
        else
        {
            sample_direction<R>(g, h, rng, in, inv_pdf, match);
            if(plastic) plastic_weights<R>(g, sm, h.nrm, h.out, in, (float)inv_pdf, wd_s, wg_s);
            else if(!CLASSED) eval_weights_general<R>(g, sm, h.nrm, h.out, h.on_dot, in, match, (float)inv_pdf, rb, es);
        }
        if(ALLFAST)
        {
            uint32_t hdr16;
            if(plastic)
            {
                *reinterpret_cast<float4 *>(recw) = make_float4(wd_n, wg_n, wd_s, wg_s);
                hdr16 = (uint32_t)ix.plastic2[sm];
            }
            else
            {
                general = 1;
                const uint32_t inside = (h.inc_mat != g.base_mat) ? 1u : 0u;
                if(cls == DRT_CLASS_ROUGH)
                {
                    const float2 wc = ct_weight<R>(g, sm, h.nrm, h.out, h.on_dot, in);
                    recw[2] = wc.x * (float)inv_pdf; recw[3] = wc.y;
                    hdr16 = (uint32_t)DRT_CLASS_ROUGH | (inside << 4) | ((uint32_t)sm << 5);
                }
                else
                {
                    const int mask = g.bmask[sm], mt = match & 3;
                    recw[0] = g.spec_c[sm][mt < 3 ? mt : 0][0] * (float)inv_pdf;
                    recw[1] = g.spec_c[sm][mt < 3 ? mt : 0][1] * (float)inv_pdf;
                    recw[2] = (float)h.on_dot;
                    const uint32_t basis = (mask & (1 << BK_MIRROR)) ? 0u : (mask & (1 << BK_DIEL_R)) ? 1u : 2u;
                    hdr16 = (uint32_t)DRT_CLASS_SPECULAR | (basis << 2) | (inside << 4) | ((uint32_t)sm << 5);
                }
            }
            if(nb == 0u)
            {
                const float vig = rec[REC_VIG];
                const uint32_t c = hdr16 & 3u;
                recw[0] *= vig;
                if(c != (uint32_t)DRT_CLASS_ROUGH) recw[1] *= vig;
                if(c != (uint32_t)DRT_CLASS_SPECULAR) recw[2] *= vig;
                if(c == (uint32_t)DRT_CLASS_PLASTIC) recw[3] *= vig;
            }
            if(in_smem) reinterpret_cast<uint16_t *>(rec + REC_HDR16)[nb] = (uint16_t)hdr16;
            else reinterpret_cast<uint16_t *>(deep + L.deep_hdr_off)[nb - L.smem_depth] = (uint16_t)hdr16;
        }
        else if(fast)
        {
            float4 *r4 = reinterpret_cast<float4 *>(rb);
            r4[0] = make_float4(__uint_as_float(KIND_SHADE | HDR_FAST | ((uint32_t)ix.plastic[sm] << 2)), wd_n, wg_n, 0.f);
            r4[1] = make_float4(wd_s, wg_s, 0.f, 0.f);
        }
        else
        {
            general = 1;
            if(plastic) { rb[es] = wd_s; rb[es + 1] = wg_s; }
            uint32_t swapped = (h.inc_mat != g.base_mat) ? 1u : 0u;
            rb[0] = __uint_as_float(KIND_SHADE | ((uint32_t)sm << 3) | (swapped << 8) | (vis_mask << 16));
            rb[1] = (float)h.on_dot;
        }
        nb += 1;
        d = in;
        o = h.pos;
        skip = h.plane_slot;
    }
    rec[REC_NB] = __uint_as_float(nb | emitter);
    tally[0] += closest; tally[1] += shadow; tally[2] += shaded; tally[3] += rng.draws;
    return ((end_depth < L.max_depth) ? (end_depth < 7 ? end_depth : 7) : 8) | (general << 8);
}

__device__ __forceinline__ unsigned long long pk2(float a, float b) { unsigned long long r; asm("mov.b64 %0, {%1, %2};" : "=l"(r) : "f"(a), "f"(b)); return r; }
__device__ __forceinline__ void upk2(unsigned long long v, float &a, float &b) { asm("mov.b64 {%0, %1}, %2;" : "=f"(a), "=f"(b) : "l"(v)); }
__device__ __forceinline__ unsigned long long fma2(unsigned long long a, unsigned long long b, unsigned long long c)
{ unsigned long long r; asm("fma.rn.f32x2 %0, %1, %2, %3;" : "=l"(r) : "l"(a), "l"(b), "l"(c)); return r; }
__device__ __forceinline__ unsigned long long mul2(unsigned long long a, unsigned long long b)
{ unsigned long long r; asm("mul.rn.f32x2 %0, %1, %2;" : "=l"(r) : "l"(a), "l"(b)); return r; }
__device__ __forceinline__ void fma2_acc(unsigned long long &acc, unsigned long long a, unsigned long long b)
{ asm("fma.rn.f32x2 %0, %1, %2, %0;" : "+l"(acc) : "l"(a), "l"(b)); }
__device__ __forceinline__ void mul2_by(unsigned long long &x, unsigned long long t)
{ asm("mul.rn.f32x2 %0, %0, %1;" : "+l"(x) : "l"(t)); }
__device__ __forceinline__ void add2_acc(unsigned long long &acc, unsigned long long x)
{ asm("add.rn.f32x2 %0, %0, %1;" : "+l"(acc) : "l"(x)); }
__device__ __forceinline__ unsigned long long add2(unsigned long long a, unsigned long long b)
{ unsigned long long r; asm("add.rn.f32x2 %0, %1, %2;" : "=l"(r) : "l"(a), "l"(b)); return r; }

template <int NS> __device__ __forceinline__ void v_fma(float (&o)[NS], const float (&a)[NS], const float (&b)[NS], const float (&c)[NS])
{
#pragma unroll
    for(int k = 0; k + 1 < NS; k += 2) upk2(fma2(pk2(a[k], a[k + 1]), pk2(b[k], b[k + 1]), pk2(c[k], c[k + 1])), o[k], o[k + 1]);
    if(NS & 1) o[NS - 1] = fmaf(a[NS - 1], b[NS - 1], c[NS - 1]);
}
template <int NS> __device__ __forceinline__ void v_fma_s(float (&o)[NS], float s, const float (&b)[NS], const float (&c)[NS])
{
#pragma unroll
    for(int k = 0; k + 1 < NS; k += 2) upk2(fma2(pk2(s, s), pk2(b[k], b[k + 1]), pk2(c[k], c[k + 1])), o[k], o[k + 1]);
    if(NS & 1) o[NS - 1] = fmaf(s, b[NS - 1], c[NS - 1]);
}
template <int NS> __device__ __forceinline__ void v_mul(float (&o)[NS], const float (&a)[NS], const float (&b)[NS])
{
#pragma unroll
    for(int k = 0; k + 1 < NS; k += 2) upk2(mul2(pk2(a[k], a[k + 1]), pk2(b[k], b[k + 1])), o[k], o[k + 1]);
    if(NS & 1) o[NS - 1] = a[NS - 1] * b[NS - 1];
}
template <int NS> __device__ __forceinline__ void v_mul_s(float (&o)[NS], float s, const float (&b)[NS])
{
#pragma unroll
    for(int k = 0; k + 1 < NS; k += 2) upk2(mul2(pk2(s, s), pk2(b[k], b[k + 1])), o[k], o[k + 1]);
    if(NS & 1) o[NS - 1] = s * b[NS - 1];
}
template <int NS> __device__ __forceinline__ void v_add(float (&o)[NS], const float (&a)[NS], const float (&b)[NS])
{
#pragma unroll
    for(int k = 0; k + 1 < NS; k += 2) upk2(add2(pk2(a[k], a[k + 1]), pk2(b[k], b[k + 1])), o[k], o[k + 1]);
    if(NS & 1) o[NS - 1] = a[NS - 1] + b[NS - 1];
}
template <int NS> __device__ __forceinline__ void v_sub(float (&o)[NS], const float (&a)[NS], const float (&b)[NS])
{
    const unsigned long long m1 = pk2(-1.f, -1.f);
#pragma unroll
    for(int k = 0; k + 1 < NS; k += 2) upk2(fma2(pk2(b[k], b[k + 1]), m1, pk2(a[k], a[k + 1])), o[k], o[k + 1]);
    if(NS & 1) o[NS - 1] = a[NS - 1] - b[NS - 1];
}


template <int NS> struct Spec { float v[NS]; };
template <int NS> struct ShadeState { Spec<NS> thr, dst; };

static __device__ __noinline__ float fresnel_dielectric_rel(float rel, float inc_cos)
{
    const float inc_sin_sq = 1.f - inc_cos * inc_cos;
    const float ts_sin_sq = rel * rel * inc_sin_sq;
    if(ts_sin_sq >= 1.f) return 1.f;
    const float ts_cos = r_sqrt_fast(1.f - ts_sin_sq * ts_sin_sq);
    const float a = rel * ts_cos, b = rel * inc_cos;
    const float par = r_div(inc_cos - a, inc_cos + a);
    const float per = r_div(b - ts_cos, b + ts_cos);
    return 0.5f * (par * par + per * per);
}
static __device__ __noinline__ float fresnel_conductor_ab(float A, float B, float inc_cos)
{
    const float cos_sq = inc_cos * inc_cos, sin_sq = 1.f - cos_sq;
    const float r = A - sin_sq;
    const float apb_sq = r_sqrt_fast(fmaf(r, r, B));
    const float a = r_sqrt_fast(fmaxf(0.5f * (apb_sq + r), 0.f));
    const float s = apb_sq + cos_sq;
    const float t = 2.f * a * inc_cos;
    const float u = fmaf(cos_sq, apb_sq, sin_sq * sin_sq);
    const float v = t * sin_sq;
    const float par = r_div(s - t, s + t);
    const float per = r_div(par * (u - v), u + v);
    return 0.5f * (par + per);
}

static __device__ __noinline__ unsigned long long fresnel_conductor_ab2(unsigned long long A2, unsigned long long B2, float inc_cos)
{
    const float cos_sq = inc_cos * inc_cos, sin_sq = 1.f - cos_sq;
    const unsigned long long m1 = pk2(-1.f, -1.f), cs2 = pk2(cos_sq, cos_sq);
    const unsigned long long r2 = add2(A2, pk2(-sin_sq, -sin_sq));
    float q0, q1;
    upk2(fma2(r2, r2, B2), q0, q1);
    const unsigned long long apb2 = pk2(r_sqrt_fast(q0), r_sqrt_fast(q1));
    upk2(mul2(add2(apb2, r2), pk2(0.5f, 0.5f)), q0, q1);
    const unsigned long long a2 = pk2(r_sqrt_fast(fmaxf(q0, 0.f)), r_sqrt_fast(fmaxf(q1, 0.f)));
    const unsigned long long s2 = add2(apb2, cs2);
    const unsigned long long t2 = mul2(a2, pk2(2.f * inc_cos, 2.f * inc_cos));
    const unsigned long long u2 = fma2(apb2, cs2, pk2(sin_sq * sin_sq, sin_sq * sin_sq));
    const unsigned long long v2 = mul2(t2, pk2(sin_sq, sin_sq));
    upk2(add2(s2, t2), q0, q1);
    const unsigned long long par2 = mul2(fma2(t2, m1, s2), pk2(r_rcp_fast(q0), r_rcp_fast(q1)));
    upk2(add2(u2, v2), q0, q1);
    const unsigned long long per2 = mul2(mul2(par2, fma2(v2, m1, u2)), pk2(r_rcp_fast(q0), r_rcp_fast(q1)));
    return mul2(add2(par2, per2), pk2(0.5f, 0.5f));
}
static __device__ __noinline__ unsigned long long fresnel_dielectric_rel2(unsigned long long rel2, float inc_cos)
{
    const float inc_sin_sq = 1.f - inc_cos * inc_cos;
    const unsigned long long m1 = pk2(-1.f, -1.f), c2 = pk2(inc_cos, inc_cos);
    const unsigned long long ts2 = mul2(mul2(rel2, rel2), pk2(inc_sin_sq, inc_sin_sq));
    float t0, t1, q0, q1;
    upk2(ts2, t0, t1);
    upk2(fma2(mul2(ts2, m1), ts2, pk2(1.f, 1.f)), q0, q1);
    const unsigned long long tc2 = pk2(r_sqrt_fast(fmaxf(q0, 0.f)), r_sqrt_fast(fmaxf(q1, 0.f)));
    const unsigned long long a2 = mul2(rel2, tc2), b2 = mul2(rel2, c2);
    upk2(add2(c2, a2), q0, q1);
    const unsigned long long par2 = mul2(fma2(a2, m1, c2), pk2(r_rcp_fast(q0), r_rcp_fast(q1)));
    upk2(add2(b2, tc2), q0, q1);
    const unsigned long long per2 = mul2(fma2(tc2, m1, b2), pk2(r_rcp_fast(q0), r_rcp_fast(q1)));
    float f0, f1;
    upk2(mul2(fma2(per2, per2, mul2(par2, par2)), pk2(0.5f, 0.5f)), f0, f1);
    return pk2(t0 >= 1.f ? 1.f : f0, t1 >= 1.f ? 1.f : f1);
}

template <int NS>
__device__ __forceinline__ Spec<NS> eval_spectrum_general(const float *col, uint32_t at, int mask, const SpdIndex &ix, const float *pool_lane,
                                                          int surf_mat, int inside, float on_dot)
{
    float w_const = 0.f, w_d = 0.f, w_g = 0.f, w_m = 0.f, w_r = 0.f, w_a = 0.f, w_b = 0.f, c_b = 0.f;
    if(mask & (1 << BK_CONST))   { w_const = col[at]; at += 1; }
    if(mask & (1 << BK_DIFFUSE)) { w_d = col[at]; at += 1; }
    if(mask & (1 << BK_GLOSSY))  { w_g = col[at]; at += 1; }
    if(mask & (1 << BK_MIRROR))  { w_m = col[at]; at += 1; }
    if(mask & (1 << BK_DIEL_R))  { w_r = col[at]; at += 1; }
    if(mask & (1 << BK_COND_ON)) { w_a = col[at]; at += 1; }
    if(mask & (1 << BK_COND_MN)) { w_b = col[at]; c_b = col[at + 1]; }
    const float *dr = pool_lane + ix.row[surf_mat][DRT_SPD_DIFFUSE];
    const float *gr = pool_lane + ix.row[surf_mat][DRT_SPD_GLOSSY];
    const float *mr = pool_lane + ix.row[surf_mat][DRT_SPD_MIRROR];
    Spec<NS> f;
#pragma unroll
    for(int k = 0; k < NS; k += 1)
        f.v[k] = fmaf(w_m, mr[k * DRT_HALF], fmaf(w_g, gr[k * DRT_HALF], fmaf(w_d, dr[k * DRT_HALF], w_const)));
    if(w_r != 0.f)
    {
        const float *rel = pool_lane + ix.fres[surf_mat][inside][0];
#pragma unroll
        for(int k = 0; k + 1 < NS; k += 2)
        {
            float r0, r1;
            upk2(fresnel_dielectric_rel2(pk2(rel[k * DRT_HALF], rel[(k + 1) * DRT_HALF]), on_dot), r0, r1);
            f.v[k] = fmaf(w_r, r0, f.v[k]); f.v[k + 1] = fmaf(w_r, r1, f.v[k + 1]);
        }
        if(NS & 1) f.v[NS - 1] = fmaf(w_r, fresnel_dielectric_rel(rel[(NS - 1) * DRT_HALF], on_dot), f.v[NS - 1]);
    }
    if(w_a != 0.f || w_b != 0.f)
    {
        const float *ra = pool_lane + ix.fres[surf_mat][inside][1], *rb = pool_lane + ix.fres[surf_mat][inside][2];
#pragma unroll 1
        for(int t = 0; t < 2; t += 1)
        {
            const float w = t ? w_b : w_a, cs = t ? c_b : on_dot;
            if(w == 0.f) continue;
#pragma unroll
            for(int k = 0; k + 1 < NS; k += 2)
            {
                float r0, r1;
                upk2(fresnel_conductor_ab2(pk2(ra[k * DRT_HALF], ra[(k + 1) * DRT_HALF]), pk2(rb[k * DRT_HALF], rb[(k + 1) * DRT_HALF]), cs), r0, r1);
                f.v[k] = fmaf(w, r0, f.v[k]); f.v[k + 1] = fmaf(w, r1, f.v[k + 1]);
            }
            if(NS & 1) f.v[NS - 1] = fmaf(w, fresnel_conductor_ab(ra[(NS - 1) * DRT_HALF], rb[(NS - 1) * DRT_HALF], cs), f.v[NS - 1]);
        }
    }
    return f;
}

template <int NS, typename G>
static __device__ __noinline__ ShadeState<NS> shade_bounce_general(const float *col, uint32_t base, uint32_t hdr, const G &g, const SpdIndex &ix,
                                                            const float *pool_lane, uint32_t ew, int nlights, ShadeState<NS> st)
{
    const int surf_mat = (hdr >> 3) & 31;
    const int mask = g.bmask[surf_mat];
    const bool swapped = (hdr >> 8) & 1u;
    const int inside = swapped ? 1 : 0;
    const uint32_t vis = hdr >> 16;
    const float on_dot = col[base + 1];
    float contrib[NS];
#pragma unroll
    for(int k = 0; k < NS; k += 1) contrib[k] = 0.f;
#pragma unroll 1
    for(int j = 0; j < nlights; j += 1)
    {
        if(!((vis >> j) & 1u)) continue;
        uint32_t e = base + 2 + (ew + 1) * (uint32_t)j;
        Spec<NS> f = eval_spectrum_general<NS>(col, e, mask, ix, pool_lane, surf_mat, inside, on_dot);
        float kk = col[e + ew];
        const float *erow = pool_lane + ix.row[g.mat[g.light_surf[j]]][DRT_SPD_EMISSION];
#pragma unroll
        for(int k = 0; k < NS; k += 1) contrib[k] = ((contrib[k] + f.v[k]) * erow[k * DRT_HALF]) * kk;
    }
#pragma unroll
    for(int k = 0; k < NS; k += 1) st.dst.v[k] = fmaf(st.thr.v[k], contrib[k], st.dst.v[k]);
    Spec<NS> f = eval_spectrum_general<NS>(col, base + 2 + (ew + 1) * (uint32_t)nlights, mask, ix, pool_lane, surf_mat, inside, on_dot);
#pragma unroll
    for(int k = 0; k < NS; k += 1) st.thr.v[k] *= f.v[k];
    return st;
}

template <int NS>
__device__ __forceinline__ void shade_special(uint32_t hdr, float4 w, const float *pool_lane, const SpdIndex &ix,
                                              unsigned long long (&r2)[NS / 2 > 0 ? NS / 2 : 1], float &r1)
{
    constexpr int NP = NS / 2;
    const int cls = (int)(hdr & 3u), inside = (int)((hdr >> 4) & 1u), mat = (int)((hdr >> 5) & 31u);
    if(cls == DRT_CLASS_SPECULAR)
    {
        const uint32_t basis = (hdr >> 2) & 3u;
        const float *x0 = pool_lane + (basis == 0u ? ix.row[mat][DRT_SPD_MIRROR] : basis == 1u ? ix.fres[mat][inside][0] : ix.fres[mat][inside][1]);
        const float *x1 = pool_lane + ix.fres[mat][inside][2];
        const unsigned long long c0 = pk2(w.x, w.x), c1 = pk2(w.y, w.y);
#pragma unroll
        for(int k = 0; k < NP; k += 1)
        {
            unsigned long long x = pk2(x0[(2 * k) * DRT_HALF], x0[(2 * k + 1) * DRT_HALF]);
            if(basis == 1u) x = fresnel_dielectric_rel2(x, w.z);
            else if(basis == 2u) x = fresnel_conductor_ab2(x, pk2(x1[(2 * k) * DRT_HALF], x1[(2 * k + 1) * DRT_HALF]), w.z);
            mul2_by(r2[k], fma2(c1, x, c0));
        }
        if(NS & 1)
        {
            float x = x0[(NS - 1) * DRT_HALF];
            if(basis == 1u) x = fresnel_dielectric_rel(x, w.z);
            else if(basis == 2u) x = fresnel_conductor_ab(x, x1[(NS - 1) * DRT_HALF], w.z);
            r1 *= fmaf(w.y, x, w.x);
        }
    }
    else
    {
        const float *ra = pool_lane + ix.fres[mat][inside][1], *rb = pool_lane + ix.fres[mat][inside][2];
        auto rows2 = [&](int k, unsigned long long &a2, unsigned long long &b2)
        {
            a2 = pk2(ra[(2 * k) * DRT_HALF], ra[(2 * k + 1) * DRT_HALF]); b2 = pk2(rb[(2 * k) * DRT_HALF], rb[(2 * k + 1) * DRT_HALF]);
        };
        const float a1 = (NS & 1) ? ra[(NS - 1) * DRT_HALF] : 0.f, b1 = (NS & 1) ? rb[(NS - 1) * DRT_HALF] : 0.f;
        const unsigned long long ws = pk2(w.z, w.z);
#pragma unroll
        for(int k = 0; k < NP; k += 1) { unsigned long long a2, b2; rows2(k, a2, b2); mul2_by(r2[k], mul2(ws, fresnel_conductor_ab2(a2, b2, w.w))); }
        if(NS & 1) r1 *= w.z * fresnel_conductor_ab(a1, b1, w.w);
        if(w.x != 0.f)
        {
            const unsigned long long wn = pk2(w.x, w.x);
#pragma unroll
            for(int k = 0; k < NP; k += 1) { unsigned long long a2, b2; rows2(k, a2, b2); fma2_acc(r2[k], wn, fresnel_conductor_ab2(a2, b2, w.y)); }
            if(NS & 1) r1 = fmaf(w.x, fresnel_conductor_ab(a1, b1, w.y), r1);
        }
    }
}

template <bool DEEP> __device__ __forceinline__ uint32_t load_hdr16(const uint16_t *p)
{
    if constexpr(DEEP) return *p;
    uint32_t v;
    asm volatile("ld.shared.u16 %0, [%1];" : "=r"(v) : "r"((uint32_t)__cvta_generic_to_shared(p)));
    return v;
}

template <int NS, int MODE, bool DEEP>
__device__ __forceinline__ void replay_compact(const float *col, const float *deep, uint32_t nb, const SpdIndex &ix, const float *pool, const float *pool_lane,
                                               uint32_t lane16, const RenderLaunch &L, unsigned long long (&r2)[NS / 2 > 0 ? NS / 2 : 1], float &r1)
{
    constexpr bool CLASSED = MODE == 2;
    constexpr int NP = NS / 2;
    const uint32_t nshade = nb & 0xffffu;
    if(nshade == 0u)
    {
        const float v = col[REC_VIG];
#pragma unroll
        for(int k = 0; k < NP; k += 1) r2[k] = pk2(v, v);
        r1 = v;
        return;
    }
    int b = (int)nshade - 1;
    int rest = 0;
    const uint16_t *hp = reinterpret_cast<const uint16_t *>(col + REC_HDR16) + b;
    const float4 *wp = reinterpret_cast<const float4 *>(col + L.head_words) + b;
    if(DEEP && nshade > L.smem_depth)
    {
        rest = (int)L.smem_depth;
        b = (int)(nshade - L.smem_depth) - 1;
        hp = reinterpret_cast<const uint16_t *>(deep + L.deep_hdr_off) + b;
        wp = reinterpret_cast<const float4 *>(deep) + b;
    }
    auto step_back = [&]() { const int s = (!DEEP || b > 0) ? 1 : 0; hp -= s; wp -= s; };
    uint32_t hdr = load_hdr16<DEEP>(hp);
    const float e = (nb >> 16) ? 1.f : 0.f;
    if(!CLASSED || (hdr & 3u) == 0u)
    {
        const float4 w = *wp;
        const float4 *blk = reinterpret_cast<const float4 *>(pool + hdr) + lane16;
        const float wd = fmaf(w.z, e, w.x), wg = fmaf(w.w, e, w.y);
        const unsigned long long wd2 = pk2(wd, wd), wg2 = pk2(wg, wg);
        step_back();
        hdr = load_hdr16<DEEP>(hp);
        b -= 1;
#pragma unroll
        for(int k = 0; k < NP; k += 1)
        {
            const float4 dg = blk[k * DRT_HALF];
            r2[k] = fma2(wg2, pk2(dg.z, dg.w), mul2(wd2, pk2(dg.x, dg.y)));
        }
        if(NS & 1)
        {
            const float2 q = *reinterpret_cast<const float2 *>(blk + NP * DRT_HALF);
            r1 = fmaf(wg, q.y, wd * q.x);
        }
    }
    else
    {
#pragma unroll
        for(int k = 0; k < NP; k += 1) r2[k] = pk2(e, e);
        r1 = e;
    }
#pragma unroll 1
    for(;;)
    {
#pragma unroll 1
        for(; b >= 0; b -= 1)
        {
            const float4 w = *wp;
            if constexpr(CLASSED)
            {
                if(hdr & 3u)
                {
                    shade_special<NS>(hdr, w, pool_lane, ix, r2, r1);
                    step_back();
                    hdr = load_hdr16<DEEP>(hp);
                    continue;
                }
            }
            const float4 *blk = reinterpret_cast<const float4 *>(pool + hdr) + lane16;
            const unsigned long long wdn = pk2(w.x, w.x), wgn = pk2(w.y, w.y), wds = pk2(w.z, w.z), wgs = pk2(w.w, w.w);
            step_back();
            hdr = load_hdr16<DEEP>(hp);
#pragma unroll
            for(int k = 0; k < NP; k += 1)
            {
                const float4 dg = blk[k * DRT_HALF];
                r2[k] = fma2(pk2(dg.z, dg.w), fma2(wgs, r2[k], wgn), mul2(pk2(dg.x, dg.y), fma2(wds, r2[k], wdn)));
            }
            if(NS & 1)
            {
                const float2 q = *reinterpret_cast<const float2 *>(blk + NP * DRT_HALF);
                r1 = fmaf(q.y, fmaf(w.w, r1, w.y), q.x * fmaf(w.z, r1, w.x));
            }
        }
        if(!DEEP || rest == 0) break;
        b = rest - 1;
        rest = 0;
        hp = reinterpret_cast<const uint16_t *>(col + REC_HDR16) + b;
        wp = reinterpret_cast<const float4 *>(col + L.head_words) + b;
        hdr = load_hdr16<DEEP>(hp);
    }
}

template <int NS, bool DEEP, typename G>
__device__ __forceinline__ void replay_path(const float *col, const float *deep, uint32_t nb, const G &g, const SpdIndex &ix, const float *pool, const float *pool_lane,
                                            uint32_t lane16, const RenderLaunch &L, float (&c)[NS])
{
    constexpr int NP = NS / 2;
    unsigned long long thr2[NP > 0 ? NP : 1], dst2[NP > 0 ? NP : 1];
    float thr1 = 1.f, dst1 = 0.f;
#pragma unroll
    for(int k = 0; k < NP; k += 1) { thr2[k] = pk2(1.f, 1.f); dst2[k] = pk2(0.f, 0.f); }
    const uint32_t bw = L.bounce_words, ew = L.eval_words;
    const float *p = (!DEEP || L.smem_depth) ? col + REC_HEAD : deep;
    float4 a_next = *reinterpret_cast<const float4 *>(p);
    for(uint32_t b = 0; b < nb; b += 1)
    {
        const float4 a = a_next;
        const float *pc = p;
        p = (DEEP && b + 1 == L.smem_depth) ? deep : p + bw;
        if(b + 1 < nb) a_next = *reinterpret_cast<const float4 *>(p);
        const uint32_t hdr = __float_as_uint(a.x);
        if((hdr & HDR_FAST) != 0u)
        {
            const float4 s4 = *reinterpret_cast<const float4 *>(pc + 4);
            const float4 *blk = reinterpret_cast<const float4 *>(pool) + (hdr >> 4) + lane16;
            const unsigned long long wdn = pk2(a.y, a.y), wgn = pk2(a.z, a.z), wds = pk2(s4.x, s4.x), wgs = pk2(s4.y, s4.y);
#pragma unroll
            for(int k = 0; k < NP; k += 1)
            {
                const float4 dg = blk[(2 * k) * DRT_HALF], ee = blk[(2 * k + 1) * DRT_HALF];
                unsigned long long f = fma2(wgn, pk2(ee.z, ee.w), mul2(wdn, pk2(ee.x, ee.y)));
                dst2[k] = fma2(thr2[k], f, dst2[k]);
                unsigned long long t = fma2(wgs, pk2(dg.z, dg.w), mul2(wds, pk2(dg.x, dg.y)));
                thr2[k] = mul2(thr2[k], t);
            }
            if(NS & 1)
            {
                const float4 q = blk[(NS - 1) * DRT_HALF];
                dst1 = fmaf(thr1, fmaf(a.z, q.w, a.y * q.z), dst1);
                thr1 *= fmaf(s4.y, q.y, s4.x * q.x);
            }
            continue;
        }
        if((hdr & 3u) == KIND_EMIT)
        {
            const float *row = pool_lane + ix.row[(hdr >> 3) & 31][DRT_SPD_EMISSION];
#pragma unroll
            for(int k = 0; k < NP; k += 1) dst2[k] = fma2(thr2[k], pk2(row[(2 * k) * DRT_HALF], row[(2 * k + 1) * DRT_HALF]), dst2[k]);
            if(NS & 1) dst1 = fmaf(thr1, row[(NS - 1) * DRT_HALF], dst1);
            break;
        }
        ShadeState<NS> st;
#pragma unroll
        for(int k = 0; k < NP; k += 1) { upk2(thr2[k], st.thr.v[2 * k], st.thr.v[2 * k + 1]); upk2(dst2[k], st.dst.v[2 * k], st.dst.v[2 * k + 1]); }
        if(NS & 1) { st.thr.v[NS - 1] = thr1; st.dst.v[NS - 1] = dst1; }
        st = shade_bounce_general<NS, G>(pc, 0u, hdr, g, ix, pool_lane, ew, L.nlights, st);
#pragma unroll
        for(int k = 0; k < NP; k += 1) { thr2[k] = pk2(st.thr.v[2 * k], st.thr.v[2 * k + 1]); dst2[k] = pk2(st.dst.v[2 * k], st.dst.v[2 * k + 1]); }
        if(NS & 1) { thr1 = st.thr.v[NS - 1]; dst1 = st.dst.v[NS - 1]; }
    }
    const float vig = col[REC_VIG];
    const unsigned long long vig2 = pk2(vig, vig);
#pragma unroll
    for(int k = 0; k < NP; k += 1) upk2(mul2(dst2[k], vig2), c[2 * k], c[2 * k + 1]);
    if(NS & 1) c[NS - 1] = dst1 * vig;
}

template <int NS> struct BatchStats
{
    static constexpr int NP = NS / 2, NP1 = NP > 0 ? NP : 1;
    unsigned long long s2[NP1], q2[NP1], k2[NP1];
    float s1, q1, k1;
    uint32_t cnt;
    __device__ __forceinline__ void clear()
    {
        cnt = 0u; s1 = 0.f; q1 = 0.f; k1 = 0.f;
#pragma unroll
        for(int k = 0; k < NP; k += 1) { s2[k] = pk2(0.f, 0.f); q2[k] = pk2(0.f, 0.f); k2[k] = pk2(0.f, 0.f); }
    }
    __device__ __forceinline__ void add(const unsigned long long (&r2)[NP1], float r1, bool first)
    {
        const unsigned long long m1 = pk2(-1.f, -1.f);
        if(first)
        {
#pragma unroll
            for(int k = 0; k < NP; k += 1) k2[k] = r2[k];
            k1 = r1;
        }
        cnt += 1u;
#pragma unroll
        for(int k = 0; k < NP; k += 1)
        {
            add2_acc(s2[k], r2[k]);
            const unsigned long long d = fma2(k2[k], m1, r2[k]);
            q2[k] = fma2(d, d, q2[k]);
        }
        if(NS & 1)
        {
            s1 += r1;
            const float d = r1 - k1;
            q1 = fmaf(d, d, q1);
        }
    }
};

template <int NS> struct PixelFilm
{
    float sum[NS], mean[NS], m2[NS], cnt;
    bool  lit;
    __device__ __forceinline__ void clear()
    {
        cnt = 0.f; lit = false;
#pragma unroll
        for(int k = 0; k < NS; k += 1) { sum[k] = 0.f; mean[k] = 0.f; m2[k] = 0.f; }
    }
    __device__ __forceinline__ void park(float *s) const
    {
        s[0] = cnt; s[DRT_WARP] = lit ? 1.f : 0.f;
#pragma unroll
        for(int k = 0; k < NS; k += 1) { s[(2 + k) * DRT_WARP] = sum[k]; s[(2 + NS + k) * DRT_WARP] = mean[k]; s[(2 + 2 * NS + k) * DRT_WARP] = m2[k]; }
    }
    __device__ __forceinline__ void unpark(const float *s)
    {
        cnt = s[0]; lit = s[DRT_WARP] != 0.f;
#pragma unroll
        for(int k = 0; k < NS; k += 1) { sum[k] = s[(2 + k) * DRT_WARP]; mean[k] = s[(2 + NS + k) * DRT_WARP]; m2[k] = s[(2 + 2 * NS + k) * DRT_WARP]; }
    }
    __device__ __forceinline__ void add(const float (&c)[NS])
    {
        cnt += 1.f; lit = true;
        float inv = r_rcp_fast(cnt);
        float delta[NS], rest[NS];
        v_add<NS>(sum, sum, c);
        v_sub<NS>(delta, c, mean);
        v_fma_s<NS>(mean, inv, delta, mean);
        v_sub<NS>(rest, c, mean);
        v_fma<NS>(m2, delta, rest, m2);
    }
    __device__ __forceinline__ void add_zeros(uint32_t k)
    {
        const float n0 = cnt;
        cnt += (float)k;
        if(!lit || k == 0u) return;
        const float w = (float)k * r_rcp_fast(cnt);
        const float s = n0 * w;
#pragma unroll
        for(int j = 0; j < NS; j += 1)
        {
            m2[j] = fmaf(mean[j] * mean[j], s, m2[j]);
            mean[j] = fmaf(-mean[j], w, mean[j]);
        }
    }
    __device__ __forceinline__ void add_batch(uint32_t nz, const BatchStats<NS> &bs, const float *e, uint32_t lane16)
    {
        if(bs.cnt == 0u) { add_zeros(nz); return; }
        const float nb = (float)(bs.cnt + nz), n0 = cnt, zf = (float)nz;
        cnt += nb; lit = true;
        const float inv_nb = r_rcp_fast(nb);
        const float w = nb * r_rcp_fast(cnt);
        const float s = n0 * w;
#pragma unroll
        for(int j = 0; j < NS; j += 1)
        {
            float S, Q, K, t;
            if(j + 1 < NS || !(NS & 1))
            {
                if(j & 1) { upk2(bs.s2[j >> 1], t, S); upk2(bs.q2[j >> 1], t, Q); upk2(bs.k2[j >> 1], t, K); }
                else      { upk2(bs.s2[j >> 1], S, t); upk2(bs.q2[j >> 1], Q, t); upk2(bs.k2[j >> 1], K, t); }
            }
            else { S = bs.s1; Q = bs.q1; K = bs.k1; }
            const float E = e[2 * ((j >> 1) * DRT_HALF + lane16) + (j & 1)];
            const float m = S * inv_nb, dk = m - K;
            const float m2b = fmaxf(fmaf(-nb * dk, dk, fmaf(zf * K, K, Q)), 0.f);
            const float delta = fmaf(E, m, -mean[j]);
            sum[j] = fmaf(E, S, sum[j]);
            m2[j] = fmaf(delta * delta, s, fmaf(E * E, m2b, m2[j]));
            mean[j] = fmaf(delta, w, mean[j]);
        }
    }
    __device__ __forceinline__ void merge_halves()
    {
        float nb = __shfl_xor_sync(0xffffffffu, cnt, DRT_HALF);
        bool  lb = __shfl_xor_sync(0xffffffffu, (int)lit, DRT_HALF) != 0;
        float nab = cnt + nb;
        float wb = (nab > 0.f) ? nb / nab : 0.f;
#pragma unroll
        for(int k = 0; k < NS; k += 1)
        {
            float mb = __shfl_xor_sync(0xffffffffu, mean[k], DRT_HALF);
            float vb = __shfl_xor_sync(0xffffffffu, m2[k], DRT_HALF);
            float sb = __shfl_xor_sync(0xffffffffu, sum[k], DRT_HALF);
            float delta = mb - mean[k];
            m2[k] = m2[k] + vb + delta * delta * cnt * wb;
            mean[k] = fmaf(delta, wb, mean[k]);
            sum[k] += sb;
        }
        cnt = nab; lit = lit || lb;
    }
};

template <int NS>
static __device__ __forceinline__ bool pixel_converged(const PixelFilm<NS> &f, const RenderLaunch &L, uint32_t n, uint32_t lane16)
{
    const float nb = __shfl_xor_sync(0xffffffffu, f.cnt, DRT_HALF);
    const float nab = f.cnt + nb;
    const float wb = (nab > 0.f) ? nb / nab : 0.f;
    const float inv = 1.f / (nab * (nab - 1.f));
    float y = 0.f, e = 0.f;
#pragma unroll
    for(int k = 0; k < NS; k += 1)
    {
        const float mb = __shfl_xor_sync(0xffffffffu, f.mean[k], DRT_HALF);
        const float vb = __shfl_xor_sync(0xffffffffu, f.m2[k], DRT_HALF);
        const float delta = mb - f.mean[k];
        const float m2 = f.m2[k] + vb + delta * delta * f.cnt * wb;
        const float mean = fmaf(delta, wb, f.mean[k]);
        const uint32_t wl = lane16 + k * DRT_HALF;
        if(wl < n)
        {
            const float w = __ldg(L.luminance_w + wl);
            y = fmaf(w, mean, y);
            e = fmaf(w, sqrtf(fmaxf(m2, 0.f) * inv), e);
        }
    }
#pragma unroll
    for(int o = DRT_HALF / 2; o > 0; o >>= 1) { y += __shfl_xor_sync(0xffffffffu, y, o); e += __shfl_xor_sync(0xffffffffu, e, o); }
    const bool stop = nab >= (float)L.min_samples && e <= L.rel_error * y;
    return __shfl_sync(0xffffffffu, stop ? 1 : 0, 0) != 0;
}

template <int NS>
static __device__ __noinline__ PixelFilm<NS> film_load(FilmPtrs film, uint32_t gpix, uint32_t n, uint32_t lane)
{
    PixelFilm<NS> f;
    f.clear();
    if(lane >= DRT_HALF) return f;
    f.cnt = film.filter[gpix]; f.lit = true;
#pragma unroll
    for(int k = 0; k < NS; k += 1)
    {
        uint32_t wl = lane + k * DRT_HALF;
        size_t at = (size_t)gpix * n + wl;
        f.sum[k] = (wl < n) ? film.sum[at] : 0.f; f.mean[k] = (wl < n) ? film.mean[at] : 0.f; f.m2[k] = (wl < n) ? film.m2[at] : 0.f;
    }
    return f;
}

template <int NS>
static __device__ __noinline__ void film_store(FilmPtrs film, uint32_t gpix, uint32_t n, uint32_t lane, PixelFilm<NS> f)
{
    if(lane >= DRT_HALF) return;
#pragma unroll
    for(int k = 0; k < NS; k += 1)
    {
        uint32_t wl = lane + k * DRT_HALF;
        if(wl < n)
        {
            size_t at = (size_t)gpix * n + wl;
            film.sum[at] = f.sum[k]; film.mean[at] = f.mean[k]; film.m2[at] = f.m2[k];
        }
    }
    if(lane == 0) film.filter[gpix] = f.cnt;
}


template <int NS>
static __device__ __noinline__ void dump_path(float *record_dump, float *path_dump, uint32_t path_words, const float *rec_slot, const float *c,
                                       const float *e, size_t path_index, uint32_t n, uint32_t lane16)
{
    if(record_dump)
        for(uint32_t wd = lane16; wd < path_words; wd += DRT_HALF) record_dump[path_index * path_words + wd] = rec_slot[wd];
    if(path_dump)
#pragma unroll
        for(int k = 0; k < NS; k += 1)
        {
            uint32_t wl = lane16 + k * DRT_HALF;
            const float ek = e ? e[2 * ((k >> 1) * DRT_HALF + lane16) + (k & 1)] : 1.f;
            if(wl < n) path_dump[path_index * n + wl] = c ? ek * c[k] : 0.f;
        }
}

#ifndef DRT_PARK_GENERAL
#define DRT_PARK_GENERAL 0
#endif
#define DRT_PHASE_TRACE  0
#define DRT_PHASE_BOOK   1
#define DRT_PHASE_REPLAY 2
#define DRT_PHASE_OTHER  3
#ifdef DRT_PHASE_CLOCKS
#define DRT_PHASE_CUT(k) do { uint32_t t_; asm volatile("mov.u32 %0, %%clock;" : "=r"(t_) :: "memory"); \
                              if(lane == 0) atomicAdd(&s_phase[k], (unsigned long long)(t_ - phase_t)); phase_t = t_; } while(0)
#else
#define DRT_PHASE_CUT(k) do {} while(0)
#endif
#define DRT_RENDER_BOUNDS(MODE) __launch_bounds__((MODE == 1 ? DRT_FAST_WARPS : MODE == 2 ? DRT_CLASSED_WARPS : DRT_CTA_WARPS) * DRT_WARP, \
                                                  MODE == 1 ? DRT_MIN_CTAS : MODE == 2 ? DRT_CLASSED_CTAS : DRT_GENERAL_CTAS)
template <typename R, int NS, int MODE, bool PAIRED, bool DEEP>
__global__ void DRT_RENDER_BOUNDS(MODE) render_kernel(const RenderLaunch L)
{
    constexpr bool ADAPTIVE = false;
#include "drt_render_body.cuh"
}

template <typename R, int NS, int MODE, bool DEEP>
__global__ void DRT_RENDER_BOUNDS(MODE) render_kernel_adaptive(const RenderLaunch L)
{
    constexpr bool PAIRED = true, ADAPTIVE = true;
#include "drt_render_body.cuh"
}

}


template <typename K>
static cudaError_t drt_launch_one(K kernel, const RenderLaunch &L, int grid, int warps, size_t smem, cudaStream_t stream)
{
    cudaError_t e = cudaFuncSetAttribute(kernel, cudaFuncAttributeMaxDynamicSharedMemorySize, (int)smem);
    if(e != cudaSuccess) return e;
    e = cudaFuncSetAttribute(kernel, cudaFuncAttributePreferredSharedMemoryCarveout, 100);
    if(e != cudaSuccess) return e;
    kernel<<<grid, warps * DRT_WARP, smem, stream>>>(L);
    return cudaGetLastError();
}

template <typename R, int MODE, bool PAIRED, bool DEEP>
static cudaError_t drt_launch_render_ns(const RenderLaunch &L, int nslots, int grid, int warps, size_t smem, cudaStream_t stream)
{
    switch(nslots)
    {
        case 2: return drt_launch_one(drt::render_kernel<R, 2, MODE, PAIRED, DEEP>, L, grid, warps, smem, stream);
        case 3: return drt_launch_one(drt::render_kernel<R, 3, MODE, PAIRED, DEEP>, L, grid, warps, smem, stream);
        case 5: return drt_launch_one(drt::render_kernel<R, 5, MODE, PAIRED, DEEP>, L, grid, warps, smem, stream);
        default: return drt_launch_one(drt::render_kernel<R, 8, MODE, PAIRED, DEEP>, L, grid, warps, smem, stream);
    }
}

template <int MODE, bool DEEP>
static cudaError_t drt_launch_adaptive_ns(const RenderLaunch &L, int nslots, int grid, int warps, size_t smem, cudaStream_t stream)
{
    switch(nslots)
    {
        case 2: return drt_launch_one(drt::render_kernel_adaptive<float, 2, MODE, DEEP>, L, grid, warps, smem, stream);
        case 3: return drt_launch_one(drt::render_kernel_adaptive<float, 3, MODE, DEEP>, L, grid, warps, smem, stream);
        case 5: return drt_launch_one(drt::render_kernel_adaptive<float, 5, MODE, DEEP>, L, grid, warps, smem, stream);
        default: return drt_launch_one(drt::render_kernel_adaptive<float, 8, MODE, DEEP>, L, grid, warps, smem, stream);
    }
}

#define DRT_DEFINE_ADAPTIVE_LAUNCHERS(NAME, MODE) \
    cudaError_t NAME(const RenderLaunch &L, int nslots, int grid, int warps, size_t smem, cudaStream_t stream) \
    { \
        return drt_launch_adaptive_ns<MODE, false>(L, nslots, grid, warps, smem, stream); \
    } \
    cudaError_t NAME##_deep(const RenderLaunch &L, int nslots, int grid, int warps, size_t smem, cudaStream_t stream) \
    { \
        return drt_launch_adaptive_ns<MODE, true>(L, nslots, grid, warps, smem, stream); \
    }

#define DRT_DEFINE_LAUNCHER(NAME, R, MODE, DEEP) \
    cudaError_t NAME(const RenderLaunch &L, bool paired, int nslots, int grid, int warps, size_t smem, cudaStream_t stream) \
    { \
        return paired ? drt_launch_render_ns<R, MODE, true, DEEP>(L, nslots, grid, warps, smem, stream) \
                      : drt_launch_render_ns<R, MODE, false, DEEP>(L, nslots, grid, warps, smem, stream); \
    }
```

### daily-ray-trace_b200/csrc/drt_render_body.cuh

```cuda
    constexpr bool ALLFAST = MODE != 0;
    constexpr bool LOCKSTEP = MODE == 2 ? ((DRT_LOCKSTEP & 2) != 0) : MODE == 0 ? ((DRT_LOCKSTEP & 1) != 0) : ((DRT_LOCKSTEP & 4) != 0);
    __shared__ unsigned long long phase_bar;
    __shared__ uint32_t gates_off;
#ifdef DRT_PHASE_CLOCKS
    __shared__ unsigned long long s_phase[4];
    uint32_t phase_t = 0;
    if(threadIdx.x < 4) s_phase[threadIdx.x] = 0ull;
#endif
    const uint32_t bar_addr = (uint32_t)__cvta_generic_to_shared(&phase_bar);
    if(LOCKSTEP && threadIdx.x == 0)
    {
        asm volatile("mbarrier.init.shared::cta.b64 [%0], %1;" :: "r"(bar_addr), "r"(blockDim.x >> 5) : "memory");
        gates_off = L.scatter_count > 1 ? 1u : 0u;
    }
    extern __shared__ __align__(16) unsigned char smem_raw[];
    GeomT<R> *sg = reinterpret_cast<GeomT<R> *>(smem_raw);
    size_t off = (sizeof(GeomT<R>) + 15) & ~size_t(15);
    SpdIndex *six = reinterpret_cast<SpdIndex *>(smem_raw + off);
    off += (sizeof(SpdIndex) + 15) & ~size_t(15);
    float *spool = reinterpret_cast<float *>(smem_raw + off);
    off += (size_t)L.pool_words * 4;
    unsigned long long *s_stats = reinterpret_cast<unsigned long long *>(smem_raw + off);
    off += 16 * 8;
    off = (off + 15) & ~size_t(15);
    float *srec = reinterpret_cast<float *>(smem_raw + off);
    float *spark = srec + (size_t)(blockDim.x >> 5) * L.path_stride * DRT_WARP;

    {
        const uint32_t *src = reinterpret_cast<const uint32_t *>(L.geom);
        uint32_t *dst = reinterpret_cast<uint32_t *>(sg);
#pragma unroll 1
        for(uint32_t i = threadIdx.x; i < sizeof(GeomT<R>) / 4; i += blockDim.x) dst[i] = src[i];
        src = reinterpret_cast<const uint32_t *>(L.spd_index);
        dst = reinterpret_cast<uint32_t *>(six);
#pragma unroll 1
        for(uint32_t i = threadIdx.x; i < sizeof(SpdIndex) / 4; i += blockDim.x) dst[i] = src[i];
#pragma unroll 1
        for(uint32_t i = threadIdx.x; i < L.pool_words; i += blockDim.x) spool[i] = L.pool[i];
        if(threadIdx.x < 16) s_stats[threadIdx.x] = 0ull;
    }
    __syncthreads();
    const GeomT<R> &g = *sg;
    const SpdIndex &ix = *six;

    const uint32_t lane = threadIdx.x & 31u, warp = threadIdx.x >> 5;
    const uint32_t lane16 = lane & (DRT_HALF - 1), half = lane >> 4;
#ifdef DRT_PHASE_CLOCKS
    asm volatile("mov.u32 %0, %%clock;" : "=r"(phase_t) :: "memory");
#endif
    float *rec = srec + (size_t)warp * L.path_stride * DRT_WARP;
    const uint32_t stride = L.path_stride;
    float *park = spark + (size_t)warp * (3 * NS + 2) * DRT_WARP + lane;
    float *deep_w = DEEP ? L.deep + (size_t)(blockIdx.x * (blockDim.x >> 5) + warp) * DRT_WARP * L.deep_stride : nullptr;
    const float *pool_lane = spool + lane16;
    const uint32_t rw = L.x1 - L.x0, npix = rw * (L.y1 - L.y0);
    const uint32_t spp = L.sample_end - L.sample_begin;
    const uint32_t n = (uint32_t)ix.n;
    const uint32_t ntasks = (PAIRED && L.band_chunk) ? L.band_chunk * L.scatter_count : (npix + L.pixels_per_task - 1) / L.pixels_per_task;
    const bool have_film = L.film.sum != nullptr;
    constexpr bool paired = PAIRED;
    auto store_pixel = [&](uint32_t gpix, const PixelFilm<NS> &f)
    {
        FilmPtrs out = L.film;
        uint32_t at = gpix;
        if(L.scatter_count)
        {
            const uint32_t owner = gpix / L.scatter_slice;
            out = L.scatter[owner];
            at = L.scatter_rank * L.scatter_slice + (gpix - owner * L.scatter_slice);
        }
        film_store<NS>(out, at, n, lane, f);
    };
    const bool dumping = L.path_dump || L.record_dump;

    uint32_t tally[4] = { 0u, 0u, 0u, 0u };
    uint32_t traced = 0;
    uint32_t gate_parity = 0;
    auto gate = [&]()
    {
        if constexpr(LOCKSTEP)
        {
            if(*reinterpret_cast<volatile uint32_t *>(&gates_off)) return;
            if(lane == 0) asm volatile("mbarrier.arrive.shared::cta.b64 _, [%0];" :: "r"(bar_addr) : "memory");
            __syncwarp();
            uint32_t ok = 0;
            const long long t0 = clock64();
            while(!ok)
            {
                asm volatile("{ .reg .pred p; mbarrier.try_wait.parity.shared::cta.b64 p, [%1], %2, %3; selp.u32 %0, 1, 0, p; }"
                             : "=r"(ok) : "r"(bar_addr), "r"(gate_parity), "r"(DRT_GATE_SUSPEND_NS) : "memory");
                if(!ok && (clock64() - t0 > DRT_GATE_PATIENCE_CYCLES || *reinterpret_cast<volatile uint32_t *>(&gates_off)))
                {
                    gates_off = 1u;
                    break;
                }
            }
            gate_parity ^= 1u;
        }
    };
    for(;;)
    {
        uint32_t task = 0;
        if(lane == 0) task = atomicAdd(L.task_counter, 1u);
        task = __shfl_sync(0xffffffffu, task, 0);
        if(task >= ntasks)
        {
            if(LOCKSTEP && lane == 0) asm volatile("mbarrier.arrive_drop.shared::cta.b64 _, [%0];" :: "r"(bar_addr) : "memory");
            break;
        }
        task += L.task_rotate;
        if(task >= ntasks) task -= ntasks;
        uint32_t p_begin = task * L.pixels_per_task;
        if(paired && L.band_chunk)
        {
            p_begin = (p_begin / L.band_chunk) * L.band_period + L.band_base + p_begin % L.band_chunk;
            if(p_begin >= L.width * L.height) continue;
        }
        const uint32_t p_end = paired ? p_begin + 1u : min(p_begin + L.pixels_per_task, npix);
        const uint32_t total = (p_end - p_begin) * spp;
        traced += total;

        PixelFilm<NS> film;
        film.clear();
        const uint32_t task_x = L.x0 + p_begin % rw, task_y = L.y0 + p_begin / rw;
        if(paired && L.accumulate && have_film) film = film_load<NS>(L.film, task_y * L.width + task_x, n, lane);

        if(paired && !dumping && (task_x < L.hit_x0 || task_x >= L.hit_x1 || task_y < L.hit_y0 || task_y >= L.hit_y1))
        {
            uint32_t taken = total;
            if constexpr(ADAPTIVE)
            {
                for(uint32_t q0 = 0; q0 < total; q0 += DRT_WARP)
                {
                    const uint32_t count = min((uint32_t)DRT_WARP, total - q0);
                    if(half == 0) film.add_zeros(count);
                    if(pixel_converged<NS>(film, L, n, lane16)) { taken = q0 + count; break; }
                }
                traced -= total - taken;
            }
            else if(half == 0) film.add_zeros(total);
            if(lane == 0)
            {
                atomicAdd(&s_stats[1], (unsigned long long)taken);
                atomicAdd(&s_stats[4], (unsigned long long)((L.pixel_scheme == DRT_PIXEL_RANDOM) ? 2u * taken : 0u));
                atomicAdd(&s_stats[5], (unsigned long long)taken);
            }
            film.merge_halves();
            if(have_film) store_pixel(task_y * L.width + task_x, film);
            continue;
        }
        for(uint32_t q0 = 0; q0 < total; q0 += DRT_WARP)
        {
            DRT_PHASE_CUT(DRT_PHASE_OTHER);
            gate();
            if((ALLFAST || DRT_PARK_GENERAL) && paired) film.park(park);
            const uint32_t q = q0 + lane;
            uint32_t bin = 9, general = 0;
            uint32_t my_px = 0, my_s = q;
            if(!paired) { my_px = q / spp; my_s = q - my_px * spp; }
            if(q < total)
            {
                uint32_t x = task_x, y = task_y;
                if(!paired) { const uint32_t lp = p_begin + my_px; x = L.x0 + lp % rw; y = L.y0 + lp / rw; }
                if(x < L.hit_x0 || x >= L.hit_x1 || y < L.hit_y0 || y >= L.hit_y1)
                {
                    rec[lane * stride + REC_NB] = 0.f;
                    tally[0] += 1; tally[3] += (L.pixel_scheme == DRT_PIXEL_RANDOM) ? 2u : 0u;
                    bin = 0;
                }
                else
                {
                    uint32_t r = trace_path<R, MODE, DEEP>(g, ix, L, rec + lane * stride, deep_w + (size_t)lane * L.deep_stride, x, y, L.sample_begin + my_s, tally);
                    bin = r & 255u; general = r >> 8;
                }
            }
            __syncwarp();
            DRT_PHASE_CUT(DRT_PHASE_TRACE);
            gate();
            if(!ALLFAST && DRT_PARK_GENERAL && paired) film.unpark(park);
            {
                const uint32_t peers = __match_any_sync(0xffffffffu, bin);
                if(bin < 9u && lane == (uint32_t)__ffs(peers) - 1u) atomicAdd(&s_stats[5 + bin], (unsigned long long)__popc(peers));
            }
            const uint32_t count = min((uint32_t)DRT_WARP, total - q0);
            const uint32_t my_nb = __float_as_uint(rec[lane * stride + REC_NB]);
            if(paired && !dumping && !__any_sync(0xffffffffu, lane < count && my_nb != 0u))
            {
                if(ALLFAST) film.unpark(park);
                if(half == 0) film.add_zeros(count);
                __syncwarp();
                DRT_PHASE_CUT(DRT_PHASE_BOOK);
                if constexpr(ADAPTIVE)
                    if(pixel_converged<NS>(film, L, n, lane16)) { traced -= total - (q0 + count); break; }
                continue;
            }
            const uint32_t cls = (my_nb == 0u) ? 0u : min((my_nb & 0xffffu) + (my_nb >> 16 ? 1u : 0u), 15u) + (general ? 16u : 0u);
            uint32_t v = (lane >= count) ? 0xffffffffu : (((my_px << 5) | cls) << 5) | lane;
#pragma unroll
            for(uint32_t k = 2; k <= 32; k <<= 1)
#pragma unroll
                for(uint32_t j = k >> 1; j > 0; j >>= 1)
                {
                    uint32_t other = __shfl_xor_sync(0xffffffffu, v, j);
                    bool keep_min = ((lane & k) == 0) == ((lane & j) == 0);
                    v = keep_min ? min(v, other) : max(v, other);
                }
            const uint32_t per_px = paired ? count : spp;
            const uint32_t npx = paired ? 1u : count / spp;
#pragma unroll 1
            for(uint32_t px = 0; px < npx; px += 1)
            {
                const uint32_t lp = p_begin + px;
                uint32_t gpix = 0;
                auto start_film = [&]()
                {
                    if(!paired)
                    {
                        gpix = (L.y0 + lp / rw) * L.width + L.x0 + lp % rw;
                        film.clear();
                        if(L.accumulate && have_film) film = film_load<NS>(L.film, gpix, n, lane);
                    }
                };
                if(!ALLFAST) start_film();
                const uint32_t lo = px * per_px;
                const uint32_t nzero = __popc(__ballot_sync(0xffffffffu, lane < count && my_px == px && my_nb == 0u));
                if(!ALLFAST && half == 0) film.add_zeros(nzero);
                if(dumping)
                    for(uint32_t i = lo; i < lo + nzero; i += 1)
                    {
                        const uint32_t slot = __shfl_sync(0xffffffffu, v, i) & 31u;
                        const uint32_t s_in = paired ? q0 + slot : slot - px * spp;
                        if(half == 0) dump_path<NS>(L.record_dump, L.path_dump, L.path_words, rec + slot * stride, nullptr, nullptr, (size_t)lp * spp + s_in, n, lane16);
                    }
                BatchStats<NS> bs;
                if(ALLFAST) bs.clear();
                DRT_PHASE_CUT(DRT_PHASE_BOOK);
                for(uint32_t i = lo + nzero; i < lo + per_px; i += 2)
                {
                    const uint32_t pos = i + half;
                    const uint32_t slot = __shfl_sync(0xffffffffu, v, pos & 31u) & 31u;
                    const uint32_t nb = __shfl_sync(0xffffffffu, my_nb, slot);
                    if(pos < lo + per_px)
                    {
                        float c[NS];
                        if constexpr(ALLFAST)
                        {
                            unsigned long long r2[BatchStats<NS>::NP1];
                            float r1;
                            replay_compact<NS, MODE, DEEP>(rec + slot * stride, deep_w + (size_t)slot * L.deep_stride, nb, ix, spool, pool_lane, lane16, L, r2, r1);
                            bs.add(r2, r1, i == lo + nzero);
                            if(dumping)
                            {
#pragma unroll
                                for(int k = 0; k < NS / 2; k += 1) upk2(r2[k], c[2 * k], c[2 * k + 1]);
                                if(NS & 1) c[NS - 1] = r1;
                            }
                        }
                        else
                        {
                            replay_path<NS, DEEP>(rec + slot * stride, deep_w + (size_t)slot * L.deep_stride, nb, g, ix, spool, pool_lane, lane16, L, c);
                            film.add(c);
                        }
                        if(dumping)
                        {
                            float cc[NS];
#pragma unroll
                            for(int k = 0; k < NS; k += 1) cc[k] = c[k];
                            dump_path<NS>(L.record_dump, L.path_dump, L.path_words, rec + slot * stride, cc, ALLFAST ? spool + ix.light_pairs : nullptr,
                                          (size_t)lp * spp + (paired ? q0 + slot : slot - px * spp), n, lane16);
                        }
                    }
                }
                DRT_PHASE_CUT(DRT_PHASE_REPLAY);
                if constexpr(ALLFAST)
                {
                    if(paired) film.unpark(park);
                    else start_film();
                    film.add_batch(half == 0 ? nzero : 0u, bs, spool + ix.light_pairs, lane16);
                }
                if(!paired)
                {
                    film.merge_halves();
                    if(have_film) store_pixel(gpix, film);
                }
            }
            __syncwarp();
            DRT_PHASE_CUT(DRT_PHASE_BOOK);
            if constexpr(ADAPTIVE)
                if(pixel_converged<NS>(film, L, n, lane16)) { traced -= total - (q0 + count); break; }
        }
        if(paired)
        {
            film.merge_halves();
            if(have_film) store_pixel(task_y * L.width + task_x, film);
        }
    }

    DRT_PHASE_CUT(DRT_PHASE_OTHER);
#pragma unroll
    for(int k = 0; k < 4; k += 1)
    {
        unsigned long long v = tally[k];
#pragma unroll
        for(int o = 16; o > 0; o >>= 1) v += __shfl_xor_sync(0xffffffffu, v, o);
        if(lane == 0) atomicAdd(&s_stats[1 + k], v);
    }
    if(lane == 0) atomicAdd(&s_stats[0], (unsigned long long)traced);
    __syncthreads();
    if(threadIdx.x < 14 && s_stats[threadIdx.x])
        atomicAdd(reinterpret_cast<unsigned long long *>(L.stats) + threadIdx.x, s_stats[threadIdx.x]);
#ifdef DRT_PHASE_CLOCKS
    if(threadIdx.x < 4) atomicAdd(&L.stats->phase_clocks[threadIdx.x], s_phase[threadIdx.x]);
#endif
```

### daily-ray-trace_b200/cuda.py

```python
import ctypes as C
import os

import numpy as np

from . import PACKAGE_DIR
from ._structs import Adaptive, Camera, RenderParams, Scene, Tables

GEOMETRY_F32, GEOMETRY_F64 = 0, 1

EXPORTS = ["drt_cuda_last_error", "drt_cuda_device_count", "drt_cuda_create", "drt_cuda_destroy", "drt_cuda_upload_scene",
           "drt_cuda_scene_upload_bytes", "drt_cuda_set_geometry_precision", "drt_cuda_film_sizes", "drt_cuda_render_device", "drt_cuda_render_host", "drt_cuda_render_host_multi",
           "drt_cuda_get_stats", "drt_cuda_analyse_scene", "drt_cuda_validate_scene", "drt_cuda_render_kernel_info", "drt_cuda_sample_paths", "drt_cuda_film_to_rgb", "drt_cuda_film_merge",
           "drt_cuda_measure_fp32_peak", "drt_cuda_film_alloc", "drt_cuda_film_free", "drt_cuda_film_ipc_export",
           "drt_cuda_film_ipc_open", "drt_cuda_film_ipc_close", "drt_cuda_film_merge_many", "drt_cuda_film_merge_slices", "drt_cuda_render_device_scatter", "drt_cuda_debug_records", "drt_cuda_buffer_alloc", "drt_cuda_buffer_free",
           "drt_cuda_buffer_ipc_export", "drt_cuda_buffer_ipc_open", "drt_cuda_buffer_ipc_close",
           "drt_cuda_film_merge_slices_local", "drt_cuda_film_read_slice", "drt_cuda_flags_signal", "drt_cuda_flags_wait", "drt_cuda_flags_timeouts",
           "drt_cuda_host_alloc", "drt_cuda_host_free", "drt_cuda_render_host_multi_images", "drt_cuda_render_device_scatter_band", "drt_cuda_plan_scene",
           "drt_cuda_render_device_adaptive", "drt_cuda_render_host_adaptive"]


class Film(C.Structure):
    _fields_ = [("sum", C.c_void_p), ("filter", C.c_void_p), ("mean", C.c_void_p), ("m2", C.c_void_p)]


class Stats(C.Structure):
    _fields_ = [("paths", C.c_uint64), ("closest_rays", C.c_uint64), ("shadow_rays", C.c_uint64),
                ("shaded_bounces", C.c_uint64), ("rng_draws", C.c_uint64), ("terminated_at_depth", C.c_uint64 * 8),
                ("reached_depth_cap", C.c_uint64), ("kernel_launches", C.c_uint64)]


class CudaError(RuntimeError):
    def __init__(self, code, message):
        super().__init__(f"drt_cuda error {code}: {message}")
        self.code = code


_lib = None


def library_path():
    return os.environ.get("DRT_CUDA_LIB") or os.path.join(PACKAGE_DIR, "libdrt_cuda.so")


def lib():
    global _lib
    if _lib is None:
        path = library_path()
        if not os.path.exists(path):
            raise ImportError(f"{path} is missing: the CUDA extension must be built (make -C {PACKAGE_DIR}); "
                              "this package has no CPU render path")
        L = C.CDLL(path)
        L.drt_cuda_last_error.restype = C.c_char_p
        L.drt_cuda_create.argtypes = [C.c_int, C.POINTER(C.c_void_p)]
        L.drt_cuda_destroy.argtypes = [C.c_void_p]
        L.drt_cuda_destroy.restype = None
        L.drt_cuda_upload_scene.argtypes = [C.c_void_p, C.POINTER(Scene), C.POINTER(Camera), C.POINTER(Tables)]
        L.drt_cuda_scene_upload_bytes.argtypes = [C.c_void_p, C.POINTER(C.c_size_t)]
        L.drt_cuda_validate_scene.argtypes = [C.POINTER(Scene)]
        L.drt_cuda_plan_scene.argtypes = [C.POINTER(Scene), C.POINTER(Camera), C.POINTER(C.c_int32), C.POINTER(C.c_int32), C.POINTER(C.c_float)]
        L.drt_cuda_analyse_scene.argtypes = [C.POINTER(Scene), C.POINTER(Camera), C.c_uint32, C.c_uint32, C.POINTER(C.c_uint32 * 4), C.POINTER(C.c_int32)]
        L.drt_cuda_render_kernel_info.argtypes = [C.c_void_p, C.POINTER(RenderParams), C.c_char_p, C.c_size_t, C.POINTER(C.c_int), C.POINTER(C.c_int)]
        L.drt_cuda_set_geometry_precision.argtypes = [C.c_void_p, C.c_int]
        L.drt_cuda_film_sizes.argtypes = [C.c_void_p, C.c_uint32, C.c_uint32, C.POINTER(C.c_size_t), C.POINTER(C.c_size_t)]
        L.drt_cuda_render_device.argtypes = [C.c_void_p, C.POINTER(RenderParams), C.POINTER(Film), C.c_int, C.c_void_p]
        L.drt_cuda_render_host_multi.argtypes = [C.POINTER(C.c_void_p), C.c_int, C.POINTER(RenderParams), C.POINTER(Film)]
        L.drt_cuda_render_device_scatter.argtypes = [C.c_void_p, C.POINTER(RenderParams), C.POINTER(Film), C.c_int, C.c_int, C.c_uint64, C.c_void_p]
        L.drt_cuda_film_merge_slices.argtypes = [C.c_void_p, C.POINTER(Film), C.POINTER(Film), C.c_int, C.c_uint64, C.c_uint32, C.c_uint32,
                                                 C.c_uint64, C.c_uint64, C.c_void_p, C.c_void_p, C.c_void_p, C.c_void_p]
        L.drt_cuda_render_host.argtypes = [C.c_void_p, C.POINTER(RenderParams), C.POINTER(Film)]
        L.drt_cuda_render_device_adaptive.argtypes = [C.c_void_p, C.POINTER(RenderParams), C.POINTER(Adaptive), C.POINTER(Film), C.c_int, C.c_void_p]
        L.drt_cuda_render_host_adaptive.argtypes = [C.c_void_p, C.POINTER(RenderParams), C.POINTER(Adaptive), C.POINTER(Film)]
        L.drt_cuda_film_merge_slices_local.argtypes = [C.c_void_p, C.POINTER(Film), C.POINTER(Film), C.c_int, C.c_uint64, C.c_uint32, C.c_uint32,
                                                       C.c_uint64, C.c_uint64, C.c_void_p, C.c_void_p, C.c_void_p, C.c_void_p]
        L.drt_cuda_film_read_slice.argtypes = [C.c_void_p, C.POINTER(Film), C.c_uint64, C.c_uint64, C.c_uint64, C.POINTER(Film), C.c_void_p]
        L.drt_cuda_render_device_scatter_band.argtypes = [C.c_void_p, C.POINTER(RenderParams), C.POINTER(Film), C.c_int, C.c_int, C.c_uint64, C.c_uint64, C.c_uint64, C.c_int, C.c_void_p]
        L.drt_cuda_flags_signal.argtypes = [C.c_void_p, C.POINTER(C.c_void_p), C.c_int, C.c_uint32, C.c_void_p]
        L.drt_cuda_flags_wait.argtypes = [C.c_void_p, C.c_void_p, C.c_int, C.c_uint32, C.c_void_p]
        L.drt_cuda_flags_timeouts.argtypes = [C.c_void_p, C.POINTER(C.c_uint32)]
        L.drt_cuda_host_alloc.argtypes = [C.c_size_t, C.POINTER(C.c_void_p)]
        L.drt_cuda_host_free.argtypes = [C.c_void_p]
        L.drt_cuda_get_stats.argtypes = [C.c_void_p, C.POINTER(Stats)]
        L.drt_cuda_sample_paths.argtypes = [C.c_void_p, C.POINTER(RenderParams)] + [C.c_uint32] * 4 + [C.c_void_p]
        L.drt_cuda_film_to_rgb.argtypes = [C.c_void_p, C.POINTER(Film), C.c_uint32, C.c_uint32, C.c_int, C.c_void_p,
                                           C.c_void_p, C.c_void_p]
        L.drt_cuda_film_merge.argtypes = [C.c_void_p, C.POINTER(Film), C.POINTER(Film), C.c_uint32, C.c_uint32, C.c_void_p]
        L.drt_cuda_debug_records.argtypes = [C.c_void_p, C.POINTER(RenderParams)] + [C.c_uint32] * 4 + [C.c_void_p, C.c_size_t, C.POINTER(C.c_uint32)]
        L.drt_cuda_buffer_alloc.argtypes = [C.c_void_p, C.c_size_t, C.POINTER(C.c_void_p)]
        L.drt_cuda_buffer_free.argtypes = [C.c_void_p, C.c_void_p]
        L.drt_cuda_buffer_ipc_export.argtypes = [C.c_void_p, C.c_void_p, C.c_void_p]
        L.drt_cuda_buffer_ipc_open.argtypes = [C.c_void_p, C.c_void_p, C.POINTER(C.c_void_p)]
        L.drt_cuda_buffer_ipc_close.argtypes = [C.c_void_p, C.c_void_p]
        L.drt_cuda_film_alloc.argtypes = [C.c_void_p, C.c_uint32, C.c_uint32, C.POINTER(Film)]
        L.drt_cuda_film_free.argtypes = [C.c_void_p, C.POINTER(Film)]
        L.drt_cuda_film_ipc_export.argtypes = [C.c_void_p, C.POINTER(Film), C.c_void_p]
        L.drt_cuda_film_ipc_open.argtypes = [C.c_void_p, C.c_void_p, C.POINTER(Film)]
        L.drt_cuda_film_ipc_close.argtypes = [C.c_void_p, C.POINTER(Film)]
        L.drt_cuda_film_merge_many.argtypes = [C.c_void_p, C.POINTER(Film), C.POINTER(Film), C.c_int, C.c_uint32, C.c_uint32,
                                               C.c_uint64, C.c_uint64, C.c_void_p, C.c_void_p, C.c_void_p, C.c_void_p]
        L.drt_cuda_measure_fp32_peak.argtypes = [C.c_void_p, C.c_int, C.POINTER(C.c_double)]
        _lib = L
    return _lib


def _check(rc):
    if rc != 0:
        raise CudaError(rc, lib().drt_cuda_last_error().decode(errors="replace"))


def device_count():
    return lib().drt_cuda_device_count()


class Context:

    def __init__(self, device=0):
        self._h = C.c_void_p()
        _check(lib().drt_cuda_create(device, C.byref(self._h)))
        self.device = device
        self.n = None

    def close(self):
        if self._h:
            lib().drt_cuda_destroy(self._h)
            self._h = C.c_void_p()

    def __del__(self):
        try:
            self.close()
        except Exception:
            pass

    def upload_scene(self, scene, camera, tables):
        _check(lib().drt_cuda_upload_scene(self._h, C.byref(scene), C.byref(camera), C.byref(tables)))
        self.n = scene.num_wavelengths

    def scene_upload_bytes(self):
        v = C.c_size_t()
        _check(lib().drt_cuda_scene_upload_bytes(self._h, C.byref(v)))
        return v.value

    def render_kernel_info(self, params):
        name = C.create_string_buffer(96)
        warps, ctas = C.c_int(), C.c_int()
        _check(lib().drt_cuda_render_kernel_info(self._h, C.byref(params), name, len(name), C.byref(warps), C.byref(ctas)))
        return name.value.decode(), warps.value, ctas.value

    def set_geometry_precision(self, precision):
        _check(lib().drt_cuda_set_geometry_precision(self._h, precision))

    def render_host(self, params):
        npix = max(params.width * params.height, 1)
        n = self.n or 1
        out = {"sum": np.empty((npix, n), np.float32), "filter": np.empty(npix, np.float32),
               "mean": np.empty((npix, n), np.float32), "m2": np.empty((npix, n), np.float32)}
        film = Film(out["sum"].ctypes.data, out["filter"].ctypes.data, out["mean"].ctypes.data, out["m2"].ctypes.data)
        _check(lib().drt_cuda_render_host(self._h, C.byref(params), C.byref(film)))
        return out

    def render_host_adaptive(self, params, rel_error, min_samples):
        npix = max(params.width * params.height, 1)
        n = self.n or 1
        out = {"sum": np.empty((npix, n), np.float32), "filter": np.empty(npix, np.float32),
               "mean": np.empty((npix, n), np.float32), "m2": np.empty((npix, n), np.float32)}
        film = Film(out["sum"].ctypes.data, out["filter"].ctypes.data, out["mean"].ctypes.data, out["m2"].ctypes.data)
        _check(lib().drt_cuda_render_host_adaptive(self._h, C.byref(params), C.byref(Adaptive(rel_error, min_samples)), C.byref(film)))
        return out

    def render_device_adaptive(self, params, rel_error, min_samples, film, accumulate=False, stream=None):
        _check(lib().drt_cuda_render_device_adaptive(self._h, C.byref(params), C.byref(Adaptive(rel_error, min_samples)), C.byref(film),
                                                     int(accumulate), stream))

    def render_host_into(self, params, film):
        _check(lib().drt_cuda_render_host(self._h, C.byref(params), C.byref(film)))

    def render_device(self, params, film, accumulate=False, stream=None):
        _check(lib().drt_cuda_render_device(self._h, C.byref(params), C.byref(film), int(accumulate), stream))

    def sample_paths(self, params, x0, y0, x1, y1):
        spp = params.sample_end - params.sample_begin
        out = np.empty(((y1 - y0) * (x1 - x0), spp, self.n), np.float32)
        _check(lib().drt_cuda_sample_paths(self._h, C.byref(params), x0, y0, x1, y1, out.ctypes.data))
        return out

    def debug_records(self, params, x0, y0, x1, y1):
        words = C.c_uint32()
        _check(lib().drt_cuda_debug_records(self._h, C.byref(params), x0, y0, x1, y1, None, 0, C.byref(words)))
        spp = params.sample_end - params.sample_begin
        out = np.empty(((y1 - y0) * (x1 - x0), spp, words.value), np.uint32)
        _check(lib().drt_cuda_debug_records(self._h, C.byref(params), x0, y0, x1, y1, out.ctypes.data, out.size, C.byref(words)))
        return out

    def stats(self):
        s = Stats()
        _check(lib().drt_cuda_get_stats(self._h, C.byref(s)))
        return s

    def film_to_rgb(self, film, width, height, which, rgb_ptr=None, bgra_ptr=None, stream=None):
        _check(lib().drt_cuda_film_to_rgb(self._h, C.byref(film), width, height, which, rgb_ptr, bgra_ptr, stream))

    def film_merge(self, dst, src, width, height, stream=None):
        _check(lib().drt_cuda_film_merge(self._h, C.byref(dst), C.byref(src), width, height, stream))

    def buffer_alloc(self, nbytes):
        p = C.c_void_p()
        _check(lib().drt_cuda_buffer_alloc(self._h, nbytes, C.byref(p)))
        return p.value

    def buffer_free(self, ptr):
        _check(lib().drt_cuda_buffer_free(self._h, ptr))

    def buffer_ipc_export(self, ptr):
        buf = C.create_string_buffer(64)
        _check(lib().drt_cuda_buffer_ipc_export(self._h, ptr, buf))
        return buf.raw

    def buffer_ipc_open(self, handle):
        p = C.c_void_p()
        _check(lib().drt_cuda_buffer_ipc_open(self._h, C.create_string_buffer(handle, 64), C.byref(p)))
        return p.value

    def buffer_ipc_close(self, ptr):
        _check(lib().drt_cuda_buffer_ipc_close(self._h, ptr))

    def film_alloc(self, width, height):
        f = Film()
        _check(lib().drt_cuda_film_alloc(self._h, width, height, C.byref(f)))
        return f

    def film_free(self, film):
        _check(lib().drt_cuda_film_free(self._h, C.byref(film)))

    def film_ipc_export(self, film):
        buf = C.create_string_buffer(256)
        _check(lib().drt_cuda_film_ipc_export(self._h, C.byref(film), buf))
        return buf.raw

    def film_ipc_open(self, handles):
        f = Film()
        _check(lib().drt_cuda_film_ipc_open(self._h, C.create_string_buffer(handles, 256), C.byref(f)))
        return f

    def film_ipc_close(self, film):
        _check(lib().drt_cuda_film_ipc_close(self._h, C.byref(film)))

    def film_merge_many(self, dst, srcs, width, height, pixel_begin, pixel_end, bgra=None, stream=None):
        arr = (Film * len(srcs))(*srcs)
        b = bgra or (None, None, None)
        _check(lib().drt_cuda_film_merge_many(self._h, C.byref(dst), arr, len(srcs), width, height, pixel_begin, pixel_end,
                                              b[0], b[1], b[2], stream))

    def render_device_scatter(self, params, staging, rank, slice_pixels, stream=None):
        arr = (Film * len(staging))(*staging)
        _check(lib().drt_cuda_render_device_scatter(self._h, C.byref(params), arr, len(staging), rank, slice_pixels, stream))

    def film_merge_slices(self, dst, staging, count, slice_pixels, width, height, pixel_begin, pixel_end, bgra=None, stream=None):
        b = bgra or (None, None, None)
        _check(lib().drt_cuda_film_merge_slices(self._h, C.byref(dst), C.byref(staging), count, slice_pixels, width, height,
                                                pixel_begin, pixel_end, b[0], b[1], b[2], stream))

    def film_merge_slices_local(self, slice_film, staging, count, slice_pixels, width, height, pixel_begin, pixel_end, bgra=None, stream=None):
        b = bgra or (None, None, None)
        _check(lib().drt_cuda_film_merge_slices_local(self._h, C.byref(slice_film), C.byref(staging), count, slice_pixels, width, height,
                                                      pixel_begin, pixel_end, b[0], b[1], b[2], stream))

    def film_read_slice(self, slice_film, slice_begin, pixel_begin, pixel_end, host_film, stream=None):
        _check(lib().drt_cuda_film_read_slice(self._h, C.byref(slice_film), slice_begin, pixel_begin, pixel_end, C.byref(host_film), stream))

    def render_device_scatter_band(self, params, staging, rank, slice_pixels, band_begin, band_end, keep_stats=False, stream=None):
        arr = (Film * len(staging))(*staging)
        _check(lib().drt_cuda_render_device_scatter_band(self._h, C.byref(params), arr, len(staging), rank, slice_pixels, band_begin, band_end,
                                                         int(keep_stats), stream))

    def flags_signal(self, targets, value, stream=None):
        arr = (C.c_void_p * len(targets))(*targets)
        _check(lib().drt_cuda_flags_signal(self._h, arr, len(targets), value & 0xffffffff, stream))

    def flags_wait(self, flags_ptr, count, value, stream=None):
        _check(lib().drt_cuda_flags_wait(self._h, flags_ptr, count, value & 0xffffffff, stream))

    def flags_timeouts(self):
        v = C.c_uint32()
        _check(lib().drt_cuda_flags_timeouts(self._h, C.byref(v)))
        return v.value

    def measure_fp32_peak(self, packed=False):
        v = C.c_double()
        _check(lib().drt_cuda_measure_fp32_peak(self._h, int(packed), C.byref(v)))
        return v.value


def render_host_multi(contexts, params):
    npix, n = params.width * params.height, contexts[0].n
    out = {"sum": np.empty((npix, n), np.float32), "filter": np.empty(npix, np.float32),
           "mean": np.empty((npix, n), np.float32), "m2": np.empty((npix, n), np.float32)}
    film = Film(out["sum"].ctypes.data, out["filter"].ctypes.data, out["mean"].ctypes.data, out["m2"].ctypes.data)
    handles = (C.c_void_p * len(contexts))(*[c._h for c in contexts])
    _check(lib().drt_cuda_render_host_multi(handles, len(contexts), C.byref(params), C.byref(film)))
    return out


def validate_scene(scene):
    _check(lib().drt_cuda_validate_scene(C.byref(scene)))


def plan_scene(scene, camera):
    mode = C.c_int32()
    classes = (C.c_int32 * scene.num_materials)()
    consts = (C.c_float * (scene.num_materials * 6))()
    _check(lib().drt_cuda_plan_scene(C.byref(scene), C.byref(camera), C.byref(mode), classes, consts))
    return mode.value, list(classes), np.array(consts, dtype=np.float32).reshape(scene.num_materials, 3, 2)


def analyse_scene(scene, camera, width, height):
    rect = (C.c_uint32 * 4)()
    flags = (C.c_int32 * max(scene.num_surfaces, 1))()
    _check(lib().drt_cuda_analyse_scene(C.byref(scene), C.byref(camera), width, height, C.byref(rect), flags))
    return tuple(rect), [bool(flags[i]) for i in range(scene.num_surfaces)]


def film_from_tensors(total, filt, mean, m2):
    for t in (total, filt, mean, m2):
        assert t.is_cuda and t.is_contiguous() and t.dtype.is_floating_point and t.element_size() == 4
    return Film(total.data_ptr(), filt.data_ptr(), mean.data_ptr(), m2.data_ptr())
```

### include/drt_cuda.h

```cpp
#ifndef DRT_CUDA_H
#define DRT_CUDA_H

#include <stddef.h>
#include <stdint.h>
#include "drt_scene.h"

#ifdef __cplusplus
extern "C" {
#endif

enum
{
    DRT_CUDA_OK = 0,
    DRT_CUDA_E_NO_DEVICE = -101,
    DRT_CUDA_E_CUDA = -102,
    DRT_CUDA_E_ARG = -103,
    DRT_CUDA_E_UNSUPPORTED = -104,
    DRT_CUDA_E_STATE = -105
};

typedef struct drt_cuda_context drt_cuda_context;

enum { DRT_GEOMETRY_F32 = 0, DRT_GEOMETRY_F64 = 1 };

typedef struct
{
    float *sum, *filter, *mean, *m2;
} drt_film;

typedef struct
{
    uint64_t paths, closest_rays, shadow_rays, shaded_bounces, rng_draws;
    uint64_t terminated_at_depth[8];
    uint64_t reached_depth_cap;
    uint64_t kernel_launches;
} drt_cuda_stats;

const char *drt_cuda_last_error(void);
int  drt_cuda_device_count(void);

int  drt_cuda_create(int device, drt_cuda_context **out);
void drt_cuda_destroy(drt_cuda_context *ctx);

int  drt_cuda_upload_scene(drt_cuda_context *ctx, const drt_scene *scene, const drt_camera *camera, const drt_tables *tables);

int  drt_cuda_validate_scene(const drt_scene *scene);

int  drt_cuda_scene_upload_bytes(const drt_cuda_context *ctx, size_t *bytes);

int  drt_cuda_set_geometry_precision(drt_cuda_context *ctx, int precision);

int  drt_cuda_film_sizes(const drt_cuda_context *ctx, uint32_t width, uint32_t height, size_t *spectral_plane_bytes, size_t *filter_plane_bytes);

int  drt_cuda_render_device(drt_cuda_context *ctx, const drt_render_params *params, const drt_film *film_device,
                            int accumulate, void *stream);

int  drt_cuda_render_device_scatter(drt_cuda_context *ctx, const drt_render_params *params, const drt_film *staging_device, int count, int rank,
                                    uint64_t slice_pixels, void *stream);

int  drt_cuda_render_host(drt_cuda_context *ctx, const drt_render_params *params, const drt_film *film_host);

typedef struct
{
    float    rel_error;
    uint32_t min_samples;
} drt_adaptive;

int  drt_cuda_render_device_adaptive(drt_cuda_context *ctx, const drt_render_params *params, const drt_adaptive *adaptive,
                                     const drt_film *film_device, int accumulate, void *stream);
int  drt_cuda_render_host_adaptive(drt_cuda_context *ctx, const drt_render_params *params, const drt_adaptive *adaptive,
                                   const drt_film *film_host);

int  drt_cuda_render_host_multi(drt_cuda_context **contexts, int count, const drt_render_params *params, const drt_film *film_host);

int  drt_cuda_render_host_multi_images(drt_cuda_context **contexts, int count, const drt_render_params *params, const drt_film *film_host,
                                       uint32_t *bgra_sum_host, uint32_t *bgra_mean_host, uint32_t *bgra_var_host);

int  drt_cuda_render_kernel_info(drt_cuda_context *ctx, const drt_render_params *params, char *name, size_t name_len, int *warps_per_cta, int *ctas_per_sm);

int  drt_cuda_analyse_scene(const drt_scene *scene, const drt_camera *camera, uint32_t width, uint32_t height,
                            uint32_t hit_rect[4], int32_t *boundary );

int  drt_cuda_plan_scene(const drt_scene *scene, const drt_camera *camera, int32_t *kernel_mode,
                         int32_t *material_class , float *specular_constants );

int  drt_cuda_get_stats(drt_cuda_context *ctx, drt_cuda_stats *out);

int  drt_cuda_sample_paths(drt_cuda_context *ctx, const drt_render_params *params,
                           uint32_t x0, uint32_t y0, uint32_t x1, uint32_t y1, float *out_host);

int  drt_cuda_debug_records(drt_cuda_context *ctx, const drt_render_params *params, uint32_t x0, uint32_t y0, uint32_t x1, uint32_t y1,
                            float *out_host, size_t out_capacity_words, uint32_t *words_per_path);

int  drt_cuda_film_to_rgb(drt_cuda_context *ctx, const drt_film *film_device, uint32_t width, uint32_t height, int which,
                          float *rgb_device, uint32_t *bgra_device, void *stream);

int  drt_cuda_film_merge(drt_cuda_context *ctx, const drt_film *dst_device, const drt_film *src_device,
                         uint32_t width, uint32_t height, void *stream);


int  drt_cuda_film_alloc(drt_cuda_context *ctx, uint32_t width, uint32_t height, drt_film *out_device);
int  drt_cuda_film_free(drt_cuda_context *ctx, drt_film *film_device);

int  drt_cuda_film_ipc_export(drt_cuda_context *ctx, const drt_film *film_device, unsigned char handles[4][64]);
int  drt_cuda_film_ipc_open(drt_cuda_context *ctx, const unsigned char handles[4][64], drt_film *out_mapped);
int  drt_cuda_film_ipc_close(drt_cuda_context *ctx, drt_film *mapped);

int  drt_cuda_buffer_alloc(drt_cuda_context *ctx, size_t bytes, void **out_device);
int  drt_cuda_buffer_free(drt_cuda_context *ctx, void *device_ptr);
int  drt_cuda_buffer_ipc_export(drt_cuda_context *ctx, const void *device_ptr, unsigned char handle[64]);
int  drt_cuda_buffer_ipc_open(drt_cuda_context *ctx, const unsigned char handle[64], void **out_mapped);
int  drt_cuda_buffer_ipc_close(drt_cuda_context *ctx, void *mapped);

int  drt_cuda_film_merge_many(drt_cuda_context *ctx, const drt_film *dst_device, const drt_film *srcs_device, int count,
                              uint32_t width, uint32_t height, uint64_t pixel_begin, uint64_t pixel_end,
                              uint32_t *bgra_sum, uint32_t *bgra_mean, uint32_t *bgra_var, void *stream);

int  drt_cuda_film_merge_slices(drt_cuda_context *ctx, const drt_film *dst_device, const drt_film *staging_device, int count, uint64_t slice_pixels,
                                uint32_t width, uint32_t height, uint64_t pixel_begin, uint64_t pixel_end,
                                uint32_t *bgra_sum, uint32_t *bgra_mean, uint32_t *bgra_var, void *stream);

int  drt_cuda_film_merge_slices_local(drt_cuda_context *ctx, const drt_film *slice_device, const drt_film *staging_device, int count, uint64_t slice_pixels,
                                      uint32_t width, uint32_t height, uint64_t pixel_begin, uint64_t pixel_end,
                                      uint32_t *bgra_sum, uint32_t *bgra_mean, uint32_t *bgra_var, void *stream);

int  drt_cuda_film_read_slice(drt_cuda_context *ctx, const drt_film *slice_device, uint64_t slice_begin, uint64_t pixel_begin, uint64_t pixel_end,
                              const drt_film *film_host, void *stream);

int  drt_cuda_render_device_scatter_band(drt_cuda_context *ctx, const drt_render_params *params, const drt_film *staging_device, int count, int rank,
                                         uint64_t slice_pixels, uint64_t band_begin, uint64_t band_end, int keep_stats, void *stream);

int  drt_cuda_flags_signal(drt_cuda_context *ctx, uint32_t *const *targets, int count, uint32_t value, void *stream);
int  drt_cuda_flags_wait(drt_cuda_context *ctx, const uint32_t *flags_device, int count, uint32_t value, void *stream);
int  drt_cuda_flags_timeouts(drt_cuda_context *ctx, uint32_t *timeouts);

int  drt_cuda_host_alloc(size_t bytes, void **out_host);
int  drt_cuda_host_free(void *host_ptr);

int  drt_cuda_measure_fp32_peak(drt_cuda_context *ctx, int packed, double *tflops);

#ifdef __cplusplus
}
#endif
#endif
```

Before: 14.99 billion.

## Add quarter-warp spectral replay mode with 8 lanes per path for 65-72 wavelengths

Adds a quarter-warp mode in which each path's spectrum is spread over 8 lanes with 9 slots instead of 16 lanes with 5 slots. It applies when the wavelength count is in a narrow range, the scene runs the all-fast kernel and spp is at least 32. The plastic and emission tables are duplicated in an 8-lane interleaved layout, and the replay, film batching and merging code is generalised to a group width. Four paths now replay per warp in parallel instead of two, at the cost of more registers per lane and extra pool memory. The paired film now restores parked state inside add_batch instead of unparking it first.

```diff
diff --git a/daily-ray-trace_b200/csrc/drt_capi.cu b/daily-ray-trace_b200/csrc/drt_capi.cu
--- a/daily-ray-trace_b200/csrc/drt_capi.cu
+++ b/daily-ray-trace_b200/csrc/drt_capi.cu
@@ -496,43 +496,54 @@
                 }
             }
         }
+        const bool quarter = n >= DRT_QUARTER_MIN_N && n <= DRT_QUARTER_MAX_N && scene_kernel_mode(scene) == 1
+                             && (half_slots + 1) / 2 * 64 == DRT_QUARTER_BLOCK_OFF;
+        const int qchunks = (DRT_QUARTER_SLOTS + 1) / 2;
         for(int m = 0; m < scene->num_materials; m += 1)
         {
             const drt_material *mm = &scene->materials[m];
             int nd = 0, ng = 0;
             if(mm->is_black_body || classify_material(scene, m, &nd, &ng, nullptr) != DRT_CLASS_PLASTIC) continue;
-            auto val = [&](int k, int mult, int slot, int lane) -> float {
-                int wl = lane + slot * 16;
+            auto val = [&](int k, int mult, int slot, int gw, int lane) -> float {
+                int wl = lane + slot * gw;
                 return (wl < n && (mm->spd_mask & (1 << k))) ? (float)((double)mult * mm->spd[k][wl]) : 0.f;
             };
             const int nchunks = (half_slots + 1) / 2;
             size_t at2 = (pool.size() + 3) & ~(size_t)3;
-            pool.resize(at2 + (size_t)nchunks * 64, 0.f);
+            pool.resize(at2 + (size_t)nchunks * 64 + (quarter ? (size_t)qchunks * 32 : 0), 0.f);
             index.plastic2[m] = (int)at2;
-            for(int lane = 0; lane < 16; lane += 1)
+            auto fill = [&](size_t at, int gw, int slots) {
+                for(int lane = 0; lane < gw; lane += 1)
+                    for(int ch = 0; ch < (slots + 1) / 2; ch += 1)
+                    {
+                        float *c = &pool[at + ((size_t)ch * gw + lane) * 4];
+                        if(2 * ch + 1 < slots)
+                        {
+                            c[0] = val(DRT_SPD_DIFFUSE, nd, 2 * ch, gw, lane); c[1] = val(DRT_SPD_DIFFUSE, nd, 2 * ch + 1, gw, lane);
+                            c[2] = val(DRT_SPD_GLOSSY, ng, 2 * ch, gw, lane);  c[3] = val(DRT_SPD_GLOSSY, ng, 2 * ch + 1, gw, lane);
+                        }
+                        else { c[0] = val(DRT_SPD_DIFFUSE, nd, 2 * ch, gw, lane); c[1] = val(DRT_SPD_GLOSSY, ng, 2 * ch, gw, lane); }
+                    }
+            };
+            fill(at2, 16, half_slots);
+            if(quarter) fill(at2 + DRT_QUARTER_BLOCK_OFF, 8, DRT_QUARTER_SLOTS);
+        }
+        auto fill_e = [&](int gw, int slots) -> int {
+            const int nchunks = (slots + 1) / 2;
+            size_t ate = (pool.size() + 3) & ~(size_t)3;
+            pool.resize(ate + (size_t)nchunks * gw * 2, 0.f);
+            for(int lane = 0; lane < gw; lane += 1)
                 for(int ch = 0; ch < nchunks; ch += 1)
                 {
-                    float *c = &pool[at2 + ((size_t)ch * 16 + lane) * 4];
-                    if(2 * ch + 1 < half_slots)
-                    {
-                        c[0] = val(DRT_SPD_DIFFUSE, nd, 2 * ch, lane); c[1] = val(DRT_SPD_DIFFUSE, nd, 2 * ch + 1, lane);
-                        c[2] = val(DRT_SPD_GLOSSY, ng, 2 * ch, lane);  c[3] = val(DRT_SPD_GLOSSY, ng, 2 * ch + 1, lane);
-                    }
-                    else { c[0] = val(DRT_SPD_DIFFUSE, nd, 2 * ch, lane); c[1] = val(DRT_SPD_GLOSSY, ng, 2 * ch, lane); }
+                    float *c = &pool[ate + ((size_t)ch * gw + lane) * 2];
+                    int w0 = lane + (2 * ch) * gw, w1 = lane + (2 * ch + 1) * gw;
+                    c[0] = (w0 < n && have_e) ? (float)emission[w0] : 0.f;
+                    c[1] = (2 * ch + 1 < slots && w1 < n && have_e) ? (float)emission[w1] : 0.f;
                 }
-        }
-        const int nchunks = (half_slots + 1) / 2;
-        size_t ate = (pool.size() + 3) & ~(size_t)3;
-        pool.resize(ate + (size_t)nchunks * 32, 0.f);
-        index.light_pairs = (int)ate;
-        for(int lane = 0; lane < 16; lane += 1)
-            for(int ch = 0; ch < nchunks; ch += 1)
-            {
-                float *c = &pool[ate + ((size_t)ch * 16 + lane) * 2];
-                int w0 = lane + (2 * ch) * 16, w1 = lane + (2 * ch + 1) * 16;
-                c[0] = (w0 < n && have_e) ? (float)emission[w0] : 0.f;
-                c[1] = (2 * ch + 1 < half_slots && w1 < n && have_e) ? (float)emission[w1] : 0.f;
-            }
+            return (int)ate;
+        };
+        index.light_pairs = fill_e(16, half_slots);
+        if(quarter) index.light_pairs_q = fill_e(8, DRT_QUARTER_SLOTS);
     }
 
     if(scene->materials[scene->base_material].spd_mask & (1 << DRT_SPD_REFRACT))
@@ -590,6 +601,7 @@
     delete g32; delete g64;
     if(e != cudaSuccess) return fail(DRT_CUDA_E_CUDA, "scene upload: %s", cudaGetErrorString(e));
     ctx->n = n; ctx->nslots = index.nslots; ctx->nlights = nlights; ctx->eval_words = eval_words; ctx->all_fast = all_fast; ctx->classed = classed && !all_fast; ctx->pool_words = (uint32_t)pool.size();
+    ctx->quarter = all_fast && index.light_pairs_q != 0;
     ctx->upload_bytes = sizeof(GeomT<float>) + sizeof(GeomT<double>) + sizeof(SpdIndex) + pool.size() * 4 + rgbt.size();
     ctx->have_scene = true;
     return DRT_CUDA_OK;
@@ -618,6 +630,8 @@
 }
 
 static int kernel_mode(const drt_cuda_context *ctx) { return ctx->f64_geometry ? 0 : ctx->all_fast ? 1 : ctx->classed ? 2 : 0; }
+
+static int kernel_slots(const drt_cuda_context *ctx, uint32_t spp) { return (kernel_mode(ctx) == 1 && ctx->quarter && spp >= 32) ? DRT_QUARTER_SLOTS : ctx->nslots; }
 
 static void record_layout(const drt_cuda_context *ctx, uint32_t max_depth, uint32_t smem_depth, RenderLaunch &L)
 {
@@ -636,11 +650,11 @@
     L.deep_stride = over ? ((L.deep_hdr_off + (compact ? (over + 1) / 2 : 0u) + 4u + 3u) & ~3u) : 0u;
 }
 
-static bool launch_shape(const drt_cuda_context *ctx, uint32_t max_depth, bool whole, RenderLaunch &L, int *warps_out, int *ctas_out, size_t *smem_out)
+static bool launch_shape(const drt_cuda_context *ctx, uint32_t max_depth, int nslots, bool whole, RenderLaunch &L, int *warps_out, int *ctas_out, size_t *smem_out)
 {
     const int mode = kernel_mode(ctx);
     const int full_warps = drt_render_cta_warps(ctx->f64_geometry, mode), want_ctas = drt_render_min_ctas(ctx->f64_geometry, mode);
-    auto bytes = [&](uint32_t depth, int warps) { record_layout(ctx, max_depth, depth, L); return drt_render_smem_bytes(L, ctx->f64_geometry, warps, ctx->nslots); };
+    auto bytes = [&](uint32_t depth, int warps) { record_layout(ctx, max_depth, depth, L); return drt_render_smem_bytes(L, ctx->f64_geometry, warps, nslots); };
     int warps = full_warps;
     uint32_t depth = max_depth;
     const size_t per_cta = (size_t)(227 * 1024) / (size_t)want_ctas - 1024;
@@ -672,12 +686,21 @@
     L.pool_words = ctx->pool_words;
     int warps = 0, ctas = 0;
     size_t smem = 0;
-    if(!launch_shape(ctx, max_depth, false, L, &warps, &ctas, &smem)) return fail(DRT_CUDA_E_UNSUPPORTED, "one bounce record of this scene does not fit in shared memory");
+    const uint32_t spp = params->sample_end - params->sample_begin;
+    if(!launch_shape(ctx, max_depth, kernel_slots(ctx, spp), false, L, &warps, &ctas, &smem)) return fail(DRT_CUDA_E_UNSUPPORTED, "one bounce record of this scene does not fit in shared memory");
     if(name && name_len)
         snprintf(name, name_len, "drt::render_kernel<%s,%d,%d,%s,%s>", ctx->f64_geometry ? "double" : "float", ctx->nslots,
                  kernel_mode(ctx), (params->sample_end - params->sample_begin >= 32) ? "true" : "false", L.deep_stride ? "true" : "false");
     if(warps_per_cta) *warps_per_cta = warps;
     if(ctas_per_sm) *ctas_per_sm = ctas;
+    return DRT_CUDA_OK;
+}
+
+extern "C" int drt_cuda_render_group_width(drt_cuda_context *ctx, const drt_render_params *params, int *lanes_per_path)
+{
+    if(!ctx || !params || !lanes_per_path || params->sample_end <= params->sample_begin) return fail(DRT_CUDA_E_ARG, "bad argument");
+    if(!ctx->have_scene) return fail(DRT_CUDA_E_STATE, "upload a scene first");
+    *lanes_per_path = kernel_slots(ctx, params->sample_end - params->sample_begin) == DRT_QUARTER_SLOTS ? 8 : 16;
     return DRT_CUDA_OK;
 }
 
@@ -732,7 +755,8 @@
     const bool whole = record_dump != nullptr || (path_words_out != nullptr && !dump && !film.sum);
     int warps, ctas_per_sm;
     size_t smem;
-    if(!launch_shape(ctx, p->max_depth, whole, L, &warps, &ctas_per_sm, &smem))
+    const int nslots = kernel_slots(ctx, spp);
+    if(!launch_shape(ctx, p->max_depth, nslots, whole, L, &warps, &ctas_per_sm, &smem))
         return fail(DRT_CUDA_E_UNSUPPORTED, "%s: max_cast_depth %u with %d lights needs %zu bytes of shared memory per warp (limit %zu)",
                     whole ? "record dump" : "render", p->max_depth, ctx->nlights, smem, ctx->smem_optin);
     if(path_words_out) { *path_words_out = L.path_words; if(!record_dump && !dump && !film.sum) return DRT_CUDA_OK; }
@@ -766,7 +790,7 @@
     L.stats = ctx->d_stats;
     L.task_counter = ctx->d_counter_ring + (ctx->counter_launches++ % DRT_RING);
     CU(cudaMemsetAsync(L.task_counter, 0, sizeof(unsigned int), stream));
-    cudaError_t e = drt_launch_render(L, ctx->f64_geometry, kernel_mode(ctx), ctx->nslots, (int)grid, warps, smem, stream);
+    cudaError_t e = drt_launch_render(L, ctx->f64_geometry, kernel_mode(ctx), nslots, (int)grid, warps, smem, stream);
     if(e != cudaSuccess) return fail(DRT_CUDA_E_CUDA, "render kernel launch: %s", cudaGetErrorString(e));
     ctx->launches += 1;
     ctx->last_launches = 1;
diff --git a/daily-ray-trace_b200/csrc/drt_context.cuh b/daily-ray-trace_b200/csrc/drt_context.cuh
--- a/daily-ray-trace_b200/csrc/drt_context.cuh
+++ b/daily-ray-trace_b200/csrc/drt_context.cuh
@@ -38,6 +38,7 @@
     bool   hit_bound = false;
     double hit_u0 = 0, hit_u1 = 0, hit_v0 = 0, hit_v1 = 0;
     bool   classed = false;
+    bool   quarter = false;
     bool   all_fast = false;
     void  *d_geom32 = nullptr, *d_geom64 = nullptr;
     SpdIndex *d_index = nullptr;
diff --git a/daily-ray-trace_b200/csrc/drt_device.cuh b/daily-ray-trace_b200/csrc/drt_device.cuh
--- a/daily-ray-trace_b200/csrc/drt_device.cuh
+++ b/daily-ray-trace_b200/csrc/drt_device.cuh
@@ -6,6 +6,13 @@
 #define DRT_MAX_SLOTS 4
 #define DRT_HALF 16
 #define DRT_MAX_HALF_SLOTS 8
+#define DRT_QUARTER_SLOTS 9
+#define DRT_QUARTER_MIN_N 65
+#define DRT_QUARTER_MAX_N 72
+#define DRT_QUARTER_BLOCK_OFF 192
+static_assert((((DRT_QUARTER_MIN_N + 15) / 16 + 1) / 2) * 64 == DRT_QUARTER_BLOCK_OFF &&
+              (((DRT_QUARTER_MAX_N + 15) / 16 + 1) / 2) * 64 == DRT_QUARTER_BLOCK_OFF,
+              "every N of the quarter range has a 5-slot half-warp block of DRT_QUARTER_BLOCK_OFF words");
 #ifndef DRT_CTA_WARPS
 #define DRT_CTA_WARPS 8
 #endif
@@ -85,7 +92,7 @@
     int row[DRT_MAX_MATERIALS][DRT_SPD_COUNT];
     int plastic[DRT_MAX_MATERIALS];
     int plastic2[DRT_MAX_MATERIALS];
-    int light_pairs, pad[3];
+    int light_pairs, light_pairs_q, pad[2];
     int fres[DRT_MAX_MATERIALS][2][3];
 };
 
diff --git a/daily-ray-trace_b200/csrc/drt_render.cuh b/daily-ray-trace_b200/csrc/drt_render.cuh
--- a/daily-ray-trace_b200/csrc/drt_render.cuh
+++ b/daily-ray-trace_b200/csrc/drt_render.cuh
@@ -561,7 +561,7 @@
 #define HDR_FAST 4u
 
 
-template <typename R, int MODE, bool DEEP>
+template <typename R, int MODE, bool DEEP, bool QUARTER>
 __device__ __forceinline__ uint32_t trace_path(const GeomT<R> &g, const SpdIndex &ix, const RenderLaunch &L, float *rec, float *deep,
                                                uint32_t x, uint32_t y, uint32_t sample, uint32_t (&tally)[4])
 {
@@ -703,7 +703,7 @@
             if(plastic)
             {
                 *reinterpret_cast<float4 *>(recw) = make_float4(wd_n, wg_n, wd_s, wg_s);
-                hdr16 = (uint32_t)ix.plastic2[sm];
+                hdr16 = (uint32_t)ix.plastic2[sm] + (QUARTER ? DRT_QUARTER_BLOCK_OFF : 0u);
             }
             else
             {
@@ -1017,6 +1017,8 @@
     }
 }
 
+template <int NS> __host__ __device__ constexpr uint32_t group_width() { return NS == DRT_QUARTER_SLOTS ? 8u : (uint32_t)DRT_HALF; }
+
 template <bool DEEP> __device__ __forceinline__ uint32_t load_hdr16(const uint16_t *p)
 {
     if constexpr(DEEP) return *p;
@@ -1027,10 +1029,11 @@
 
 template <int NS, int MODE, bool DEEP>
 __device__ __forceinline__ void replay_compact(const float *col, const float *deep, uint32_t nb, const SpdIndex &ix, const float *pool, const float *pool_lane,
-                                               uint32_t lane16, const RenderLaunch &L, unsigned long long (&r2)[NS / 2 > 0 ? NS / 2 : 1], float &r1)
+                                               uint32_t gl, const RenderLaunch &L, unsigned long long (&r2)[NS / 2 > 0 ? NS / 2 : 1], float &r1)
 {
     constexpr bool CLASSED = MODE == 2;
     constexpr int NP = NS / 2;
+    constexpr uint32_t GW = group_width<NS>();
     const uint32_t nshade = nb & 0xffffu;
     if(nshade == 0u)
     {
@@ -1057,7 +1060,7 @@
     if(!CLASSED || (hdr & 3u) == 0u)
     {
         const float4 w = *wp;
-        const float4 *blk = reinterpret_cast<const float4 *>(pool + hdr) + lane16;
+        const float4 *blk = reinterpret_cast<const float4 *>(pool + hdr) + gl;
         const float wd = fmaf(w.z, e, w.x), wg = fmaf(w.w, e, w.y);
         const unsigned long long wd2 = pk2(wd, wd), wg2 = pk2(wg, wg);
         step_back();
@@ -1066,12 +1069,12 @@
 #pragma unroll
         for(int k = 0; k < NP; k += 1)
         {
-            const float4 dg = blk[k * DRT_HALF];
+            const float4 dg = blk[k * GW];
             r2[k] = fma2(wg2, pk2(dg.z, dg.w), mul2(wd2, pk2(dg.x, dg.y)));
         }
         if(NS & 1)
         {
-            const float2 q = *reinterpret_cast<const float2 *>(blk + NP * DRT_HALF);
+            const float2 q = *reinterpret_cast<const float2 *>(blk + NP * GW);
             r1 = fmaf(wg, q.y, wd * q.x);
         }
     }
@@ -1098,19 +1101,19 @@
                     continue;
                 }
             }
-            const float4 *blk = reinterpret_cast<const float4 *>(pool + hdr) + lane16;
+            const float4 *blk = reinterpret_cast<const float4 *>(pool + hdr) + gl;
             const unsigned long long wdn = pk2(w.x, w.x), wgn = pk2(w.y, w.y), wds = pk2(w.z, w.z), wgs = pk2(w.w, w.w);
             step_back();
             hdr = load_hdr16<DEEP>(hp);
 #pragma unroll
             for(int k = 0; k < NP; k += 1)
             {
-                const float4 dg = blk[k * DRT_HALF];
+                const float4 dg = blk[k * GW];
                 r2[k] = fma2(pk2(dg.z, dg.w), fma2(wgs, r2[k], wgn), mul2(pk2(dg.x, dg.y), fma2(wds, r2[k], wdn)));
             }
             if(NS & 1)
             {
-                const float2 q = *reinterpret_cast<const float2 *>(blk + NP * DRT_HALF);
+                const float2 q = *reinterpret_cast<const float2 *>(blk + NP * GW);
                 r1 = fmaf(q.y, fmaf(w.w, r1, w.y), q.x * fmaf(w.z, r1, w.x));
             }
         }
@@ -1228,6 +1231,7 @@
 
 template <int NS> struct PixelFilm
 {
+    static constexpr uint32_t GW = group_width<NS>();
     float sum[NS], mean[NS], m2[NS], cnt;
     bool  lit;
     __device__ __forceinline__ void clear()
@@ -1273,9 +1277,11 @@
             mean[j] = fmaf(-mean[j], w, mean[j]);
         }
     }
-    __device__ __forceinline__ void add_batch(uint32_t nz, const BatchStats<NS> &bs, const float *e, uint32_t lane16)
-    {
-        if(bs.cnt == 0u) { add_zeros(nz); return; }
+    template <bool FROM_PARK = false>
+    __device__ __forceinline__ void add_batch(uint32_t nz, const BatchStats<NS> &bs, const float *e, uint32_t gl, const float *parked = nullptr)
+    {
+        if(FROM_PARK) { cnt = parked[0]; lit = parked[DRT_WARP] != 0.f; }
+        if(bs.cnt == 0u) { if(FROM_PARK) unpark(parked); add_zeros(nz); return; }
         const float nb = (float)(bs.cnt + nz), n0 = cnt, zf = (float)nz;
         cnt += nb; lit = true;
         const float inv_nb = r_rcp_fast(nb);
@@ -1291,7 +1297,8 @@
                 else      { upk2(bs.s2[j >> 1], S, t); upk2(bs.q2[j >> 1], Q, t); upk2(bs.k2[j >> 1], K, t); }
             }
             else { S = bs.s1; Q = bs.q1; K = bs.k1; }
-            const float E = e[2 * ((j >> 1) * DRT_HALF + lane16) + (j & 1)];
+            if(FROM_PARK) { sum[j] = parked[(2 + j) * DRT_WARP]; mean[j] = parked[(2 + NS + j) * DRT_WARP]; m2[j] = parked[(2 + 2 * NS + j) * DRT_WARP]; }
+            const float E = e[2 * ((j >> 1) * GW + gl) + (j & 1)];
             const float m = S * inv_nb, dk = m - K;
             const float m2b = fmaxf(fmaf(-nb * dk, dk, fmaf(zf * K, K, Q)), 0.f);
             const float delta = fmaf(E, m, -mean[j]);
@@ -1300,18 +1307,18 @@
             mean[j] = fmaf(delta, w, mean[j]);
         }
     }
-    __device__ __forceinline__ void merge_halves()
-    {
-        float nb = __shfl_xor_sync(0xffffffffu, cnt, DRT_HALF);
-        bool  lb = __shfl_xor_sync(0xffffffffu, (int)lit, DRT_HALF) != 0;
+    __device__ __forceinline__ void merge_with(uint32_t o)
+    {
+        float nb = __shfl_xor_sync(0xffffffffu, cnt, o);
+        bool  lb = __shfl_xor_sync(0xffffffffu, (int)lit, o) != 0;
         float nab = cnt + nb;
         float wb = (nab > 0.f) ? nb / nab : 0.f;
 #pragma unroll
         for(int k = 0; k < NS; k += 1)
         {
-            float mb = __shfl_xor_sync(0xffffffffu, mean[k], DRT_HALF);
-            float vb = __shfl_xor_sync(0xffffffffu, m2[k], DRT_HALF);
-            float sb = __shfl_xor_sync(0xffffffffu, sum[k], DRT_HALF);
+            float mb = __shfl_xor_sync(0xffffffffu, mean[k], o);
+            float vb = __shfl_xor_sync(0xffffffffu, m2[k], o);
+            float sb = __shfl_xor_sync(0xffffffffu, sum[k], o);
             float delta = mb - mean[k];
             m2[k] = m2[k] + vb + delta * delta * cnt * wb;
             mean[k] = fmaf(delta, wb, mean[k]);
@@ -1319,11 +1326,19 @@
         }
         cnt = nab; lit = lit || lb;
     }
+    __device__ __forceinline__ void merge_groups()
+    {
+#pragma unroll
+        for(uint32_t o = GW; o < DRT_WARP; o <<= 1) merge_with(o);
+    }
 };
 
 template <int NS>
-static __device__ __forceinline__ bool pixel_converged(const PixelFilm<NS> &f, const RenderLaunch &L, uint32_t n, uint32_t lane16)
-{
+static __device__ __forceinline__ bool pixel_converged(const PixelFilm<NS> &film, const RenderLaunch &L, uint32_t n, uint32_t gl)
+{
+    constexpr uint32_t GW = group_width<NS>();
+    PixelFilm<NS> f = film;
+    if constexpr(GW < DRT_HALF) f.merge_with(GW);
     const float nb = __shfl_xor_sync(0xffffffffu, f.cnt, DRT_HALF);
     const float nab = f.cnt + nb;
     const float wb = (nab > 0.f) ? nb / nab : 0.f;
@@ -1337,7 +1352,7 @@
         const float delta = mb - f.mean[k];
         const float m2 = f.m2[k] + vb + delta * delta * f.cnt * wb;
         const float mean = fmaf(delta, wb, f.mean[k]);
-        const uint32_t wl = lane16 + k * DRT_HALF;
+        const uint32_t wl = gl + k * GW;
         if(wl < n)
         {
             const float w = __ldg(L.luminance_w + wl);
@@ -1346,7 +1361,7 @@
         }
     }
 #pragma unroll
-    for(int o = DRT_HALF / 2; o > 0; o >>= 1) { y += __shfl_xor_sync(0xffffffffu, y, o); e += __shfl_xor_sync(0xffffffffu, e, o); }
+    for(int o = GW / 2; o > 0; o >>= 1) { y += __shfl_xor_sync(0xffffffffu, y, o); e += __shfl_xor_sync(0xffffffffu, e, o); }
     const bool stop = nab >= (float)L.min_samples && e <= L.rel_error * y;
     return __shfl_sync(0xffffffffu, stop ? 1 : 0, 0) != 0;
 }
@@ -1354,14 +1369,15 @@
 template <int NS>
 static __device__ __noinline__ PixelFilm<NS> film_load(FilmPtrs film, uint32_t gpix, uint32_t n, uint32_t lane)
 {
+    constexpr uint32_t GW = group_width<NS>();
     PixelFilm<NS> f;
     f.clear();
-    if(lane >= DRT_HALF) return f;
+    if(lane >= GW) return f;
     f.cnt = film.filter[gpix]; f.lit = true;
 #pragma unroll
     for(int k = 0; k < NS; k += 1)
     {
-        uint32_t wl = lane + k * DRT_HALF;
+        uint32_t wl = lane + k * GW;
         size_t at = (size_t)gpix * n + wl;
         f.sum[k] = (wl < n) ? film.sum[at] : 0.f; f.mean[k] = (wl < n) ? film.mean[at] : 0.f; f.m2[k] = (wl < n) ? film.m2[at] : 0.f;
     }
@@ -1371,11 +1387,12 @@
 template <int NS>
 static __device__ __noinline__ void film_store(FilmPtrs film, uint32_t gpix, uint32_t n, uint32_t lane, PixelFilm<NS> f)
 {
-    if(lane >= DRT_HALF) return;
+    constexpr uint32_t GW = group_width<NS>();
+    if(lane >= GW) return;
 #pragma unroll
     for(int k = 0; k < NS; k += 1)
     {
-        uint32_t wl = lane + k * DRT_HALF;
+        uint32_t wl = lane + k * GW;
         if(wl < n)
         {
             size_t at = (size_t)gpix * n + wl;
@@ -1388,16 +1405,17 @@
 
 template <int NS>
 static __device__ __noinline__ void dump_path(float *record_dump, float *path_dump, uint32_t path_words, const float *rec_slot, const float *c,
-                                       const float *e, size_t path_index, uint32_t n, uint32_t lane16)
-{
+                                       const float *e, size_t path_index, uint32_t n, uint32_t gl)
+{
+    constexpr uint32_t GW = group_width<NS>();
     if(record_dump)
-        for(uint32_t wd = lane16; wd < path_words; wd += DRT_HALF) record_dump[path_index * path_words + wd] = rec_slot[wd];
+        for(uint32_t wd = gl; wd < path_words; wd += GW) record_dump[path_index * path_words + wd] = rec_slot[wd];
     if(path_dump)
 #pragma unroll
         for(int k = 0; k < NS; k += 1)
         {
-            uint32_t wl = lane16 + k * DRT_HALF;
-            const float ek = e ? e[2 * ((k >> 1) * DRT_HALF + lane16) + (k & 1)] : 1.f;
+            uint32_t wl = gl + k * GW;
+            const float ek = e ? e[2 * ((k >> 1) * GW + gl) + (k & 1)] : 1.f;
             if(wl < n) path_dump[path_index * n + wl] = c ? ek * c[k] : 0.f;
         }
 }
@@ -1448,6 +1466,8 @@
 template <typename R, int MODE, bool PAIRED, bool DEEP>
 static cudaError_t drt_launch_render_ns(const RenderLaunch &L, int nslots, int grid, int warps, size_t smem, cudaStream_t stream)
 {
+    if constexpr(MODE == 1 && PAIRED)
+        if(nslots == DRT_QUARTER_SLOTS) return drt_launch_one(drt::render_kernel<R, DRT_QUARTER_SLOTS, MODE, PAIRED, DEEP>, L, grid, warps, smem, stream);
     switch(nslots)
     {
         case 2: return drt_launch_one(drt::render_kernel<R, 2, MODE, PAIRED, DEEP>, L, grid, warps, smem, stream);
@@ -1460,6 +1480,8 @@
 template <int MODE, bool DEEP>
 static cudaError_t drt_launch_adaptive_ns(const RenderLaunch &L, int nslots, int grid, int warps, size_t smem, cudaStream_t stream)
 {
+    if constexpr(MODE == 1)
+        if(nslots == DRT_QUARTER_SLOTS) return drt_launch_one(drt::render_kernel_adaptive<float, DRT_QUARTER_SLOTS, MODE, DEEP>, L, grid, warps, smem, stream);
     switch(nslots)
     {
         case 2: return drt_launch_one(drt::render_kernel_adaptive<float, 2, MODE, DEEP>, L, grid, warps, smem, stream);
diff --git a/daily-ray-trace_b200/csrc/drt_render_body.cuh b/daily-ray-trace_b200/csrc/drt_render_body.cuh
--- a/daily-ray-trace_b200/csrc/drt_render_body.cuh
+++ b/daily-ray-trace_b200/csrc/drt_render_body.cuh
@@ -43,8 +43,10 @@
     const GeomT<R> &g = *sg;
     const SpdIndex &ix = *six;
 
+    constexpr bool QUARTER = NS == DRT_QUARTER_SLOTS;
+    constexpr uint32_t GW = group_width<NS>(), NG = DRT_WARP / GW;
     const uint32_t lane = threadIdx.x & 31u, warp = threadIdx.x >> 5;
-    const uint32_t lane16 = lane & (DRT_HALF - 1), half = lane >> 4;
+    const uint32_t gl = lane & (GW - 1), grp = lane / GW;
 #ifdef DRT_PHASE_CLOCKS
     asm volatile("mov.u32 %0, %%clock;" : "=r"(phase_t) :: "memory");
 #endif
@@ -52,7 +54,7 @@
     const uint32_t stride = L.path_stride;
     float *park = spark + (size_t)warp * (3 * NS + 2) * DRT_WARP + lane;
     float *deep_w = DEEP ? L.deep + (size_t)(blockIdx.x * (blockDim.x >> 5) + warp) * DRT_WARP * L.deep_stride : nullptr;
-    const float *pool_lane = spool + lane16;
+    const float *pool_lane = spool + gl;
     const uint32_t rw = L.x1 - L.x0, npix = rw * (L.y1 - L.y0);
     const uint32_t spp = L.sample_end - L.sample_begin;
     const uint32_t n = (uint32_t)ix.n;
@@ -133,19 +135,19 @@
                 for(uint32_t q0 = 0; q0 < total; q0 += DRT_WARP)
                 {
                     const uint32_t count = min((uint32_t)DRT_WARP, total - q0);
-                    if(half == 0) film.add_zeros(count);
-                    if(pixel_converged<NS>(film, L, n, lane16)) { taken = q0 + count; break; }
+                    if(grp == 0) film.add_zeros(count);
+                    if(pixel_converged<NS>(film, L, n, gl)) { taken = q0 + count; break; }
                 }
                 traced -= total - taken;
             }
-            else if(half == 0) film.add_zeros(total);
+            else if(grp == 0) film.add_zeros(total);
             if(lane == 0)
             {
                 atomicAdd(&s_stats[1], (unsigned long long)taken);
                 atomicAdd(&s_stats[4], (unsigned long long)((L.pixel_scheme == DRT_PIXEL_RANDOM) ? 2u * taken : 0u));
                 atomicAdd(&s_stats[5], (unsigned long long)taken);
             }
-            film.merge_halves();
+            film.merge_groups();
             if(have_film) store_pixel(task_y * L.width + task_x, film);
             continue;
         }
@@ -170,7 +172,7 @@
                 }
                 else
                 {
-                    uint32_t r = trace_path<R, MODE, DEEP>(g, ix, L, rec + lane * stride, deep_w + (size_t)lane * L.deep_stride, x, y, L.sample_begin + my_s, tally);
+                    uint32_t r = trace_path<R, MODE, DEEP, QUARTER>(g, ix, L, rec + lane * stride, deep_w + (size_t)lane * L.deep_stride, x, y, L.sample_begin + my_s, tally);
                     bin = r & 255u; general = r >> 8;
                 }
             }
@@ -187,11 +189,11 @@
             if(paired && !dumping && !__any_sync(0xffffffffu, lane < count && my_nb != 0u))
             {
                 if(ALLFAST) film.unpark(park);
-                if(half == 0) film.add_zeros(count);
+                if(grp == 0) film.add_zeros(count);
                 __syncwarp();
                 DRT_PHASE_CUT(DRT_PHASE_BOOK);
                 if constexpr(ADAPTIVE)
-                    if(pixel_converged<NS>(film, L, n, lane16)) { traced -= total - (q0 + count); break; }
+                    if(pixel_converged<NS>(film, L, n, gl)) { traced -= total - (q0 + count); break; }
                 continue;
             }
             const uint32_t cls = (my_nb == 0u) ? 0u : min((my_nb & 0xffffu) + (my_nb >> 16 ? 1u : 0u), 15u) + (general ? 16u : 0u);
@@ -224,20 +226,20 @@
                 if(!ALLFAST) start_film();
                 const uint32_t lo = px * per_px;
                 const uint32_t nzero = __popc(__ballot_sync(0xffffffffu, lane < count && my_px == px && my_nb == 0u));
-                if(!ALLFAST && half == 0) film.add_zeros(nzero);
+                if(!ALLFAST && grp == 0) film.add_zeros(nzero);
                 if(dumping)
                     for(uint32_t i = lo; i < lo + nzero; i += 1)
                     {
                         const uint32_t slot = __shfl_sync(0xffffffffu, v, i) & 31u;
                         const uint32_t s_in = paired ? q0 + slot : slot - px * spp;
-                        if(half == 0) dump_path<NS>(L.record_dump, L.path_dump, L.path_words, rec + slot * stride, nullptr, nullptr, (size_t)lp * spp + s_in, n, lane16);
+                        if(grp == 0) dump_path<NS>(L.record_dump, L.path_dump, L.path_words, rec + slot * stride, nullptr, nullptr, (size_t)lp * spp + s_in, n, gl);
                     }
                 BatchStats<NS> bs;
                 if(ALLFAST) bs.clear();
                 DRT_PHASE_CUT(DRT_PHASE_BOOK);
-                for(uint32_t i = lo + nzero; i < lo + per_px; i += 2)
-                {
-                    const uint32_t pos = i + half;
+                for(uint32_t i = lo + nzero; i < lo + per_px; i += NG)
+                {
+                    const uint32_t pos = i + grp;
                     const uint32_t slot = __shfl_sync(0xffffffffu, v, pos & 31u) & 31u;
                     const uint32_t nb = __shfl_sync(0xffffffffu, my_nb, slot);
                     if(pos < lo + per_px)
@@ -247,7 +249,7 @@
                         {
                             unsigned long long r2[BatchStats<NS>::NP1];
                             float r1;
-                            replay_compact<NS, MODE, DEEP>(rec + slot * stride, deep_w + (size_t)slot * L.deep_stride, nb, ix, spool, pool_lane, lane16, L, r2, r1);
+                            replay_compact<NS, MODE, DEEP>(rec + slot * stride, deep_w + (size_t)slot * L.deep_stride, nb, ix, spool, pool_lane, gl, L, r2, r1);
                             bs.add(r2, r1, i == lo + nzero);
                             if(dumping)
                             {
@@ -258,7 +260,7 @@
                         }
                         else
                         {
-                            replay_path<NS, DEEP>(rec + slot * stride, deep_w + (size_t)slot * L.deep_stride, nb, g, ix, spool, pool_lane, lane16, L, c);
+                            replay_path<NS, DEEP>(rec + slot * stride, deep_w + (size_t)slot * L.deep_stride, nb, g, ix, spool, pool_lane, gl, L, c);
                             film.add(c);
                         }
                         if(dumping)
@@ -266,32 +268,33 @@
                             float cc[NS];
 #pragma unroll
                             for(int k = 0; k < NS; k += 1) cc[k] = c[k];
-                            dump_path<NS>(L.record_dump, L.path_dump, L.path_words, rec + slot * stride, cc, ALLFAST ? spool + ix.light_pairs : nullptr,
-                                          (size_t)lp * spp + (paired ? q0 + slot : slot - px * spp), n, lane16);
+                            dump_path<NS>(L.record_dump, L.path_dump, L.path_words, rec + slot * stride, cc, ALLFAST ? spool + (QUARTER ? ix.light_pairs_q : ix.light_pairs) : nullptr,
+                                          (size_t)lp * spp + (paired ? q0 + slot : slot - px * spp), n, gl);
                         }
                     }
                 }
                 DRT_PHASE_CUT(DRT_PHASE_REPLAY);
                 if constexpr(ALLFAST)
                 {
-                    if(paired) film.unpark(park);
+                    if(paired) { if(!QUARTER) film.unpark(park); }
                     else start_film();
-                    film.add_batch(half == 0 ? nzero : 0u, bs, spool + ix.light_pairs, lane16);
+                    if constexpr(QUARTER && PAIRED) film.template add_batch<true>(grp == 0 ? nzero : 0u, bs, spool + ix.light_pairs_q, gl, park);
+                    else film.add_batch(grp == 0 ? nzero : 0u, bs, spool + ix.light_pairs, gl);
                 }
                 if(!paired)
                 {
-                    film.merge_halves();
+                    film.merge_groups();
                     if(have_film) store_pixel(gpix, film);
                 }
             }
             __syncwarp();
             DRT_PHASE_CUT(DRT_PHASE_BOOK);
             if constexpr(ADAPTIVE)
-                if(pixel_converged<NS>(film, L, n, lane16)) { traced -= total - (q0 + count); break; }
+                if(pixel_converged<NS>(film, L, n, gl)) { traced -= total - (q0 + count); break; }
         }
         if(paired)
         {
-            film.merge_halves();
+            film.merge_groups();
             if(have_film) store_pixel(task_y * L.width + task_x, film);
         }
     }
diff --git a/daily-ray-trace_b200/cuda.py b/daily-ray-trace_b200/cuda.py
--- a/daily-ray-trace_b200/cuda.py
+++ b/daily-ray-trace_b200/cuda.py
@@ -10,7 +10,7 @@
 
 EXPORTS = ["drt_cuda_last_error", "drt_cuda_device_count", "drt_cuda_create", "drt_cuda_destroy", "drt_cuda_upload_scene",
            "drt_cuda_scene_upload_bytes", "drt_cuda_set_geometry_precision", "drt_cuda_film_sizes", "drt_cuda_render_device", "drt_cuda_render_host", "drt_cuda_render_host_multi",
-           "drt_cuda_get_stats", "drt_cuda_analyse_scene", "drt_cuda_validate_scene", "drt_cuda_render_kernel_info", "drt_cuda_sample_paths", "drt_cuda_film_to_rgb", "drt_cuda_film_merge",
+           "drt_cuda_get_stats", "drt_cuda_analyse_scene", "drt_cuda_validate_scene", "drt_cuda_render_kernel_info", "drt_cuda_render_group_width", "drt_cuda_sample_paths", "drt_cuda_film_to_rgb", "drt_cuda_film_merge",
            "drt_cuda_measure_fp32_peak", "drt_cuda_film_alloc", "drt_cuda_film_free", "drt_cuda_film_ipc_export",
            "drt_cuda_film_ipc_open", "drt_cuda_film_ipc_close", "drt_cuda_film_merge_many", "drt_cuda_film_merge_slices", "drt_cuda_render_device_scatter", "drt_cuda_debug_records", "drt_cuda_buffer_alloc", "drt_cuda_buffer_free",
            "drt_cuda_buffer_ipc_export", "drt_cuda_buffer_ipc_open", "drt_cuda_buffer_ipc_close",
@@ -60,6 +60,7 @@
         L.drt_cuda_plan_scene.argtypes = [C.POINTER(Scene), C.POINTER(Camera), C.POINTER(C.c_int32), C.POINTER(C.c_int32), C.POINTER(C.c_float)]
         L.drt_cuda_analyse_scene.argtypes = [C.POINTER(Scene), C.POINTER(Camera), C.c_uint32, C.c_uint32, C.POINTER(C.c_uint32 * 4), C.POINTER(C.c_int32)]
         L.drt_cuda_render_kernel_info.argtypes = [C.c_void_p, C.POINTER(RenderParams), C.c_char_p, C.c_size_t, C.POINTER(C.c_int), C.POINTER(C.c_int)]
+        L.drt_cuda_render_group_width.argtypes = [C.c_void_p, C.POINTER(RenderParams), C.POINTER(C.c_int)]
         L.drt_cuda_set_geometry_precision.argtypes = [C.c_void_p, C.c_int]
         L.drt_cuda_film_sizes.argtypes = [C.c_void_p, C.c_uint32, C.c_uint32, C.POINTER(C.c_size_t), C.POINTER(C.c_size_t)]
         L.drt_cuda_render_device.argtypes = [C.c_void_p, C.POINTER(RenderParams), C.POINTER(Film), C.c_int, C.c_void_p]
@@ -145,6 +146,11 @@
         _check(lib().drt_cuda_render_kernel_info(self._h, C.byref(params), name, len(name), C.byref(warps), C.byref(ctas)))
         return name.value.decode(), warps.value, ctas.value
 
+    def render_group_width(self, params):
+        lanes = C.c_int()
+        _check(lib().drt_cuda_render_group_width(self._h, C.byref(params), C.byref(lanes)))
+        return lanes.value
+
     def set_geometry_precision(self, precision):
         _check(lib().drt_cuda_set_geometry_precision(self._h, precision))
 
diff --git a/include/drt_cuda.h b/include/drt_cuda.h
--- a/include/drt_cuda.h
+++ b/include/drt_cuda.h
@@ -77,6 +77,7 @@
                                        uint32_t *bgra_sum_host, uint32_t *bgra_mean_host, uint32_t *bgra_var_host);
 
 int  drt_cuda_render_kernel_info(drt_cuda_context *ctx, const drt_render_params *params, char *name, size_t name_len, int *warps_per_cta, int *ctas_per_sm);
+int  drt_cuda_render_group_width(drt_cuda_context *ctx, const drt_render_params *params, int *lanes_per_path);
 
 int  drt_cuda_analyse_scene(const drt_scene *scene, const drt_camera *camera, uint32_t width, uint32_t height,
                             uint32_t hit_rect[4], int32_t *boundary );
```

Measured after the change: 16.06 billion (median of 6 runs). +7.2%, better.
